# KyleHuang9/YOLO-LP

Measured on AMD Instinct MI355X. Metric: images/sec (640×640) end-to-end detect+NMS, yololps, 1/2/4/8 MI355X, higher is better.
Workload: dtype f16; 1 GPU; yololps 640x640 bs=32/GPU f16, synthetic frames resident in HBM, seeded random-init weights (sigma 0.25), conf 0.40 iou 0.45 max_det 1000; global_batch=32, parallelism=dp1: images sharded, all-gather of detections

## Files before the change

### include/lp_hip.h

```cpp
#ifndef LP_HIP_H
#define LP_HIP_H

#include <stddef.h>
#include <stdint.h>

#ifdef __cplusplus
extern "C" {
#endif

typedef enum { LP_OK = 0, LP_ERR_ARG = -1, LP_ERR_STATE = -2, LP_ERR_HIP = -3, LP_ERR_UNSUPPORTED = -4 } lp_status;
typedef enum { LP_F16 = 0, LP_BF16 = 1, LP_F32 = 2 } lp_dtype;
typedef enum { LP_ACT_NONE = 0, LP_ACT_RELU = 1, LP_ACT_SILU = 2 } lp_act;

#define LP_PRED_COLS 290
#define LP_DET_COLS 28
#define LP_MAX_SRC 4

typedef struct lp_engine lp_engine;

const char* lp_version(void);
const char* lp_last_error(void);

int lp_engine_create(lp_engine** out, int act_dtype );
void lp_engine_destroy(lp_engine* e);

int lp_engine_tensor(lp_engine* e, int channels, int stride_log2);

int lp_engine_set_lane(lp_engine* e, int lane);

int lp_engine_add_input(lp_engine* e, int dst);

typedef struct lp_conv_desc {
    int n_src;
    int src[LP_MAX_SRC];
    int dst;
    int ksize;
    int stride;
    int act;
    int res;
    float res_alpha;
    const float* weight;
    const float* bias;
    int dst2;
} lp_conv_desc;

int lp_engine_add_conv(lp_engine* e, const lp_conv_desc* d);

int lp_engine_add_deconv2x2(lp_engine* e, int src, int dst, const float* weight, const float* bias);

int lp_engine_add_pool5_chain(lp_engine* e, int src, int dst1, int dst2, int dst3);

int lp_engine_add_head_cls(lp_engine* e, int src, int level, int n_cls, const float* weight, const float* bias);

int lp_engine_add_head_box(lp_engine* e, int src, int level, int reg_bins, const float* weight, const float* bias,
                           const float* proj);

int lp_engine_finalize(lp_engine* e, int n_levels);
size_t lp_engine_weight_bytes(const lp_engine* e);
int lp_engine_upload(lp_engine* e, void* dev_weights, void* stream);

size_t lp_engine_arena_bytes(const lp_engine* e, int B, int H, int W);
int lp_engine_bind(lp_engine* e, void* dev_arena, size_t bytes, int B, int H, int W);
int lp_engine_tensor_info(const lp_engine* e, int id, size_t* offset, int* c, int* c_stored, int* h, int* w);
int lp_engine_num_anchors(const lp_engine* e);

int lp_engine_forward(lp_engine* e, const void* x, int x_dtype, float* pred, void* stream);

int lp_engine_forward_det(lp_engine* e, const void* x, int x_dtype, double conf_thres, void* workspace, size_t workspace_bytes,
                          void* stream);

int lp_engine_set_graph(lp_engine* e, int enable);

int lp_engine_set_single_lane(lp_engine* e, int enable);

int lp_engine_set_mfma16(lp_engine* e, int enable);

int lp_engine_num_ops(const lp_engine* e);
int lp_engine_op_info(const lp_engine* e, int op, int* kind, int* ksize, int* cin, int* cout, double* flops,
                      double* bytes);
int lp_engine_profile(lp_engine* e, const void* x, int x_dtype, float* pred, void* stream, float* op_ms, int reps);
int lp_engine_profile_ops(lp_engine* e, const void* x, int x_dtype, float* pred, void* stream, float* op_ms, int reps, int inner);

enum { LP_VARIANT_STREAM64 = 16, LP_VARIANT_STREAM128 = 17, LP_VARIANT_ROWS = 18,
       LP_VARIANT_PIPE_D = 32, LP_VARIANT_PIPE_B = 33, LP_VARIANT_PIPE_F = 34, LP_VARIANT_PIPE_C = 35,
       LP_VARIANT_PIPE_P = 36 ,
       LP_VARIANT_PIPE16_D = 39, LP_VARIANT_PIPE16_F = 41 ,
       LP_VARIANT_PIPE16_V0 = 42, LP_VARIANT_PIPE16_V1 = 43 ,
       LP_VARIANT_FUSED_STEM2 = 37 ,
       LP_VARIANT_FUSED_PW_S2 = 38  };
enum { LP_VARIANT_FUSED_BIFUSION = 45 };
enum { LP_VARIANT_BOX_SPARSE = 46, LP_VARIANT_BOX_DENSE = 47 };
enum { LP_VARIANT_PIPE16_S2A = 48, LP_VARIANT_PIPE16_S2B = 49 };
int lp_engine_op_carrier(const lp_engine* e, int op, int frame_direct);
int lp_engine_autotune(lp_engine* e, const void* x, int x_dtype, float* pred, void* stream, int reps);
int lp_engine_op_variant(const lp_engine* e, int op, int* cfg, int* nbuf);
int lp_engine_set_op_variant(lp_engine* e, int op, int cfg, int nbuf);
int lp_engine_set_op_tile(lp_engine* e, int op, int choice);
int lp_engine_op_tile(const lp_engine* e, int op, int* choice, int* TH, int* TW);
int lp_engine_copy_tuning(lp_engine* dst, const lp_engine* src);

size_t lp_nms_workspace_bytes(int B, int N);
int lp_nms(float* pred, int B, int N, double conf_thres, double iou_thres, int max_det, float* det, int32_t* count,
           int32_t* keep, void* workspace, size_t workspace_bytes, void* stream);

int lp_nms_candidates(int B, int N, double iou_thres, int max_det, float* det, int32_t* count, int32_t* keep, void* workspace,
                      size_t workspace_bytes, void* stream);

const int32_t* lp_nms_candidate_counts(const void* workspace, int B, int N);

int lp_preprocess_letterbox(const unsigned char* img, int h0, int w0, void* out, int out_dtype, int H, int W, int rh, int rw,
                            int top, int left, void* stream);
int lp_rescale_round(float* det, int n, double ratio, double padx, double pady, int img_w, int img_h, void* stream);

#define LP_FRAMES_PER_LAUNCH 64
typedef struct lp_frame_desc {
    const unsigned char* img;
    int h0, w0, rh, rw, top, left;
} lp_frame_desc;
typedef struct lp_rescale_desc { double ratio, padx, pady; int img_w, img_h; } lp_rescale_desc;
int lp_preprocess_letterbox_batch(const lp_frame_desc* desc, int n_frames, int B, void* out, int out_dtype, int H, int W,
                                  void* stream);
int lp_rescale_round_batch(float* det, const int32_t* count, int B, int max_det, const lp_rescale_desc* desc, void* stream);

typedef struct lp_tile_desc {
    const unsigned char* img;
    int h0, w0;
    int y0, x0, th, tw;
    int rh, rw, top, left;
} lp_tile_desc;
int lp_preprocess_tiles_batch(const lp_tile_desc* desc, int n_tiles, int B, void* out, int out_dtype, int H, int W, void* stream);

#define LP_NV12_PER_LAUNCH 32
typedef struct lp_nv12_desc {
    const unsigned char* y;
    const unsigned char* uv;
    int pitch_y, pitch_uv;
    int h0, w0;
    int y0, x0, th, tw;
    int rh, rw, top, left;
    int matrix;
} lp_nv12_desc;
typedef struct lp_nv12_bgr_desc {
    const unsigned char* y;
    const unsigned char* uv;
    int pitch_y, pitch_uv;
    int h0, w0;
    int matrix;
    unsigned char* out;
} lp_nv12_bgr_desc;
int lp_preprocess_nv12_batch(const lp_nv12_desc* desc, int n, int B, void* out, int out_dtype, int H, int W, void* stream);
int lp_nv12_to_bgr_batch(const lp_nv12_bgr_desc* desc, int n, void* stream);

typedef struct lp_tile_ref { int frame, y0, x0, th, tw; } lp_tile_ref;
size_t lp_merge_tiles_workspace_bytes(int n_frames, int max_det);
int lp_merge_tiles(const float* det_t, const int32_t* count_t, const lp_tile_ref* tiles, int n_tiles, int max_det_t,
                   const int* frame_hw, int n_frames, double thres, int metric , int border, int max_det,
                   float* det, int32_t* count, int32_t* src, void* workspace, size_t workspace_bytes, void* stream);

#define LP_TRACK_MAX_TRACKS 128
#define LP_TRACK_MAX_DETS 128
#define LP_TRACK_MAX_CLS 64
typedef struct lp_track_params { double match_thres, new_thres, expand; int max_age; int ncls[8]; } lp_track_params;
size_t lp_track_state_bytes(int n_streams, int max_tracks);
size_t lp_track_dropped_offset(int max_tracks, int stream_index);
int lp_track_update(void* state, int n_streams, int max_tracks, const lp_track_params* p,
                    const float* det, const int32_t* count, int B, int max_det,
                    const int* stream_of , const unsigned char* flush ,
                    float* det_out, int32_t* tid, int32_t* ended_i, float* ended_f, int32_t* ended_count,
                    int max_ended, void* stream);
int lp_track_update_slots(void* state, int n_streams, int max_tracks, const lp_track_params* p,
                          const float* det, const int32_t* count, int B, int max_det,
                          const int* stream_of , const unsigned char* flush ,
                          float* det_out, int32_t* tid, int32_t* slot, int32_t* ended_i, float* ended_f, int32_t* ended_count,
                          int max_ended, void* stream);
typedef struct lp_track_hold_params { int min_hits, max_misses; } lp_track_hold_params;
int lp_track_update_hold(void* state, int n_streams, int max_tracks, const lp_track_params* p,
                         const float* det, const int32_t* count, int B, int max_det,
                         const int* stream_of , const unsigned char* flush ,
                         float* det_out, int32_t* tid, int32_t* slot, int32_t* ended_i, float* ended_f, int32_t* ended_count,
                         int max_ended, const lp_track_hold_params* hp, float* det_hold, int32_t* count_hold, int32_t* tid_hold,
                         void* stream);

typedef struct lp_crop_desc {
    const unsigned char* img;
    int h0, w0;
    int max_crops;
    int out_slot;
} lp_crop_desc;
int lp_plate_crops_batch(const lp_crop_desc* desc, int n_frames, const float* det, const int32_t* count, int max_det,
                         unsigned char* out, int32_t* status, int n_slots, int crop_h, int crop_w, void* stream);

int lp_crop_sharpness(const unsigned char* crops, const int32_t* status, int n_slots, int crop_h, int crop_w,
                      unsigned long long* sharp, void* stream);

size_t lp_best_shot_state_bytes(int n_streams, int max_tracks, int crop_h, int crop_w);
int lp_best_shot_update(void* state, int n_streams, int max_tracks, int crop_h, int crop_w,
                        const float* det, const int32_t* count, int B, int max_det, const int32_t* tid, const int32_t* slot,
                        const unsigned char* crops, const int32_t* status, const unsigned long long* sharp, int max_crops,
                        const int* stream_of , const int32_t* ended_i, const int32_t* ended_count, int max_ended,
                        double min_score, unsigned char* shot_crops, int32_t* shot_i, unsigned long long* shot_q, float* shot_det,
                        void* stream);

#define LP_REDACT_MAX_CELL 64
typedef struct lp_redact_desc {
    unsigned char* p0;
    unsigned char* p1;
    int pitch0, pitch1;
    int h0, w0;
    int format;
} lp_redact_desc;
typedef struct lp_redact_params {
    int mode;
    int cell;
    double margin;
    unsigned char fill[3];
} lp_redact_params;
size_t lp_redact_workspace_bytes(const lp_redact_desc* desc, int n_frames, const lp_redact_params* p);
int lp_redact_plates_batch(const lp_redact_desc* desc, int n_frames, const float* det, const int32_t* count, int max_det,
                           const lp_redact_params* p, int32_t* status ,
                           void* workspace, size_t workspace_bytes, void* stream);

#define LP_REDACT_MAX_RADIUS 48
typedef struct lp_redact_gauss_params {
    double margin;
    int radius, radius_c;
    uint16_t taps[LP_REDACT_MAX_RADIUS + 1];
    uint16_t taps_c[LP_REDACT_MAX_RADIUS + 1];
} lp_redact_gauss_params;
size_t lp_redact_gauss_workspace_bytes(const lp_redact_desc* desc, int n_frames, const lp_redact_gauss_params* p);
int lp_redact_gauss_batch(const lp_redact_desc* desc, int n_frames, const float* det, const int32_t* count, int max_det,
                          const lp_redact_gauss_params* p, int32_t* status ,
                          void* workspace, size_t workspace_bytes, void* stream);

#define LP_LOOKBACK_MAX_DEPTH 32
size_t lp_lookback_state_bytes(int n_streams, int max_tracks, int depth, int rows);
int lp_lookback_update(void* state, int n_streams, int max_tracks, int depth, int max_back, int back_cap,
                       const float* det_hold, const int32_t* count_hold, const int32_t* tid, const int32_t* slot,
                       int B, int max_det, int hold_rows,
                       const int* stream_of , const unsigned char* flush ,
                       float* rel_det, int32_t* rel_count, int32_t* rel_frame,
                       float* tail_det, int32_t* tail_count, int32_t* tail_frame, void* stream);

#define LP_WATCH_MAX_ENTRIES (1 << 24)
#define LP_WATCH_MAX_COST 32768
#define LP_WATCH_BLOCK_ENTRIES 2048
// ... 40 lines not shown
```

### yolo-lp_amd/csrc/lp_conv.hip

```cpp
#include "lp_internal.h"

#include <cstdlib>

namespace lp {

int conv_launch_f16(int cfg, int mode, int ksize, int stride, int nbuf, const ConvArgs& a, hipStream_t st);
int conv_launch_bf16(int cfg, int mode, int ksize, int stride, int nbuf, const ConvArgs& a, hipStream_t st);
int conv_launch_f32(int cfg, int mode, int ksize, int stride, int nbuf, const ConvArgs& a, hipStream_t st);

int conv_stream_launch_f16(int wc, const ConvArgs& a, int cb_pack, int lds, hipStream_t st);
int conv_stream_launch_bf16(int wc, const ConvArgs& a, int cb_pack, int lds, hipStream_t st);
int conv_stream_launch_f32(int wc, const ConvArgs& a, int cb_pack, int lds, hipStream_t st);

int conv_pipe_launch_f16(int pcfg, const ConvArgs& a, int ncu, hipStream_t st);
int conv_pipe_launch_bf16(int pcfg, const ConvArgs& a, int ncu, hipStream_t st);

int head_rows_launch_f16(const ConvArgs& a, int cb_pack, hipStream_t st);
int head_rows_launch_bf16(const ConvArgs& a, int cb_pack, hipStream_t st);
int head_rows_launch_f32(const ConvArgs& a, int cb_pack, hipStream_t st);
int head_box_det_launch_f16(const ConvArgs& a, int cb_pack, hipStream_t st);
int head_box_det_launch_bf16(const ConvArgs& a, int cb_pack, hipStream_t st);
int head_box_det_launch_f32(const ConvArgs& a, int cb_pack, hipStream_t st);

ConvShape conv_shape(int dtype, int cfg, int ksize, int stride) {
    const int sz = (int)dtype_size(dtype);
    ConvShape s;
    int wc = 2, wp = 2, wgc = 1, wgp = 4;
    switch (cfg) {
        case CFG_A: wgc = 2; wgp = 2; break;
        case CFG_B: break;
        case CFG_C: wc = 1; break;
        case CFG_D: wgc = 2; wgp = 4; break;
        case CFG_E: wc = 1; wgc = 2; wgp = 2; break;
        case CFG_F: wc = 1; wgc = 4; wgp = 2; break;
    }
    s.WP = wp;
    s.WGC = wgc;
    s.WGP = wgp;
    s.CB = 32 * wc * wgc;
    s.PB = 32 * wp * wgp;
    s.NT = 64 * wgc * wgp;
    s.KC = ksize == 1 ? 128 / sz : 32 / sz;
    s.HPMAX = ksize == 1 ? s.PB : (stride == 1 ? 2 * s.PB + 128 : 5 * s.PB + 128);
    return s;
}

static inline int swz_host(int row, int g, int gpr) { return gpr == 2 ? (g ^ ((row >> 3) & 1)) : (g ^ ((row >> 1) & 7)); }

int conv_pick_pitch(const ConvShape& s, int dtype, int ksize, int stride, int TH, int TW) {
    const int hw = (TW - 1) * stride + ksize, hh = (TH - 1) * stride + ksize;
    if (ksize == 1) return hw;
    (void)dtype;
    const int rowb = 32, gpr = 2, npix = TH * TW;
    static const int G0[16] = {0, 1, 2, 3, 12, 13, 14, 15, 20, 21, 22, 23, 24, 25, 26, 27};
    static const int G1[16] = {4, 5, 6, 7, 8, 9, 10, 11, 16, 17, 18, 19, 28, 29, 30, 31};
    long best_cost = -1;
    int best = hw;
    for (int pitch = hw; pitch < hw + 16; ++pitch) {
        if (hh * pitch > s.HPMAX) break;
        long cost = 0;
        for (int blk = 0; blk * 32 < s.PB; ++blk)
            for (int t = 0; t < ksize * ksize; ++t)
                for (int half = 0; half < 2; ++half)
                    for (int g = 0; g < 2; ++g) {
                        const int* lanes = g ? G1 : G0;
                        int addr[16], n = 0, slot_cnt[16] = {0};
                        for (int k = 0; k < 16; ++k) {
                            int pl = blk * 32 + lanes[k];
                            if (pl >= npix) pl = 0;
                            const int ty = pl / TW, tx = pl - ty * TW;
                            const int kx = t % ksize, hwe = (hw + 1) >> 1;
                            const int col = stride == 2 ? (kx & 1) * hwe + tx + (kx >> 1) : tx * stride + kx;
                            const int hp = (ty * stride + t / ksize) * pitch + col;
                            const int a = hp * rowb + swz_host(hp, half, gpr) * 16;
                            bool dup = false;
                            for (int m = 0; m < n; ++m) dup |= addr[m] == a;
                            if (!dup) { addr[n++] = a; ++slot_cnt[(a >> 4) & 15]; }
                        }
                        int mx = 1;
                        for (int k = 0; k < 16; ++k) mx = slot_cnt[k] > mx ? slot_cnt[k] : mx;
                        cost += mx;
                    }
        cost = cost * 64 + (pitch - hw);
        if (best_cost < 0 || cost < best_cost) { best_cost = cost; best = pitch; }
    }
    return best;
}

int conv_pick_pitch16(const ConvShape& s, int TH, int TW) {
    const int hw = TW + 2, hh = TH + 2, rowb = 32, npix = TH * TW;
    static const int GRP[4][16] = {{0, 1, 2, 3, 12, 13, 14, 15, 20, 21, 22, 23, 24, 25, 26, 27}, {4, 5, 6, 7, 8, 9, 10, 11, 16, 17, 18, 19, 28, 29, 30, 31},
                                   {32, 33, 34, 35, 44, 45, 46, 47, 52, 53, 54, 55, 56, 57, 58, 59}, {36, 37, 38, 39, 40, 41, 42, 43, 48, 49, 50, 51, 60, 61, 62, 63}};
    auto qo = [](int i) { return ((i >> 2) == 2 ? 12 : (i >> 2) == 3 ? 8 : (i & 12)) + (i & 3); };
    long best_cost = -1;
    int best = hw;
    for (int pitch = hw; pitch < hw + 16; ++pitch) {
        if (hh * pitch > s.HPMAX) break;
        long cost = 0;
        for (int blk = 0; blk * 16 < s.PB; ++blk)
            for (int st = 0; st < 9; ++st) {
                const int ta = st < 4 ? 2 * st : (st == 4 ? 8 : 2 * st - 9), tb = st == 4 ? 0 : ta + 1;
                for (int gq = 0; gq < 4; ++gq) {
                    int addr[16], n = 0, slot_cnt[16] = {0};
                    for (int k = 0; k < 16; ++k) {
                        const int l = GRP[gq][k], i = l & 15, g = l >> 4;
                        int pl = blk * 16 + qo(i);
                        if (pl >= npix) pl = 0;
                        const int ty = pl / TW, tx = pl - ty * TW, t = g < 2 ? ta : tb;
                        const int hp = (ty + t / 3) * pitch + tx + t % 3;
                        const int a = hp * rowb + swz_host(hp, g & 1, 2) * 16 + (g >> 1) * (1 << 20);
                        bool dup = false;
                        for (int m = 0; m < n; ++m) dup |= addr[m] == a;
                        if (!dup) { addr[n++] = a; ++slot_cnt[(a >> 4) & 15]; }
                    }
                    int mx = 1;
                    for (int k = 0; k < 16; ++k) mx = slot_cnt[k] > mx ? slot_cnt[k] : mx;
                    cost += mx;
                }
            }
        cost = cost * 64 + (pitch - hw);
        if (best_cost < 0 || cost < best_cost) { best_cost = cost; best = pitch; }
    }
    return best;
}

void conv_pick_tile16v(const ConvShape& s, int Ho, int Wo, int B, int nct, int choice, int* TH, int* TW, int stride) {
    struct Cand { double cost; int th, tw; };
    Cand best[4];
    int n = 0;
    const int ncu = device_cus();
    for (int th = 1; th <= Ho; ++th)
        for (int tw = 1; tw <= Wo; ++tw) {
            const int hh = (th - 1) * stride + 3, hw = (tw - 1) * stride + 3;
            if (th * tw > s.PB || hh * hw > s.HPMAX) continue;
            const long tiles = (long)B * ceil_div(Ho, th) * ceil_div(Wo, tw) * nct;
            const int nb = ceil_div(th * tw, 16), per_wave = ceil_div(nb, s.WGP);
            const double cost = (double)ceil_div((int)tiles, ncu) * (per_wave + 0.75) + 1e-4 * hh * hw + 1e-7 * tiles;
            int pos = n < 4 ? n : 4;
            for (int k = 0; k < (n < 4 ? n : 4); ++k)
                if (cost < best[k].cost) { pos = k; break; }
            if (pos >= 4) continue;
            for (int k = (n < 4 ? n : 3); k > pos; --k) best[k] = best[k - 1];
            best[pos] = {cost, th, tw};
            if (n < 4) ++n;
        }
    if (n == 0) { *TH = 1; *TW = 1; return; }
    if (choice < 0) choice = 0;
    if (choice >= n) choice = n - 1;
    *TH = best[choice].th;
    *TW = best[choice].tw;
}

void conv_pick_tile(const ConvShape& s, int ksize, int stride, int Ho, int Wo, int choice, int* TH, int* TW) {
    struct Cand { long cost; int th, tw; };
    Cand best[4];
    int n = 0;
    for (int th = 1; th <= s.PB && th <= Ho; ++th) {
        int tw = s.PB / th;
        if (tw > Wo) tw = Wo;
        if (tw < 1) continue;
        const int hh = (th - 1) * stride + ksize, hw = (tw - 1) * stride + ksize;
        if (hh * hw > s.HPMAX) continue;
        const long tiles = (long)ceil_div(Ho, th) * ceil_div(Wo, tw);
        Cand c = {tiles * 100000 + (long)hh * hw, th, tw};
        int pos = n < 4 ? n : 4;
        for (int k = 0; k < (n < 4 ? n : 4); ++k)
            if (c.cost < best[k].cost) { pos = k; break; }
        if (pos >= 4) continue;
        for (int k = (n < 4 ? n : 3); k > pos; --k) best[k] = best[k - 1];
        best[pos] = c;
        if (n < 4) ++n;
    }
// ... 35 lines not shown
    if (a0.nsrc < 1 || a0.nsrc > LP_MAX_SRC || a0.nphase != 1 || a0.out_scale != 1 || a0.Ho != a0.H || a0.Wo != a0.W ||
        a0.out_img_stride != (long long)a0.Ho * a0.Wo * a0.out_pix_stride)
        return fail(LP_ERR_ARG, "conv1x1 stream: not a dense 1x1 stride-1 layer");
    if (a0.out2 && (a0.out_split % (32 * wc) != 0 || a0.res || a0.out2_img_stride != (long long)a0.Ho * a0.Wo * a0.out2_pix_stride))
        return fail(LP_ERR_ARG, "conv1x1 stream: the second destination must start at a cout tile of the wave");
    const int kc = 128 / (int)dtype_size(dtype);
    for (int i = 0; i < a0.nsrc; ++i)
        if (a0.src[i].cs % (kc / 4) != 0) return fail(LP_ERR_ARG, "conv1x1 stream: source channels are not whole 32-byte K-steps");
    ConvArgs a = a0;
    a.nct = ceil_div(a.out_c, 32 * wc);
    switch (dtype) {
        case LP_F16: return conv_stream_launch_f16(wc, a, cb_pack, lds, st);
        case LP_BF16: return conv_stream_launch_bf16(wc, a, cb_pack, lds, st);
        case LP_F32: return conv_stream_launch_f32(wc, a, cb_pack, lds, st);
    }
    return fail(LP_ERR_ARG, "conv1x1 stream: dtype");
}

ConvShape conv_pipe_shape(int pcfg) {
    ConvShape s;
    s.KC = 16;
    s.NT = 512;
    s.WP = 2;
    switch (pcfg) {
        case PIPE_B: s.CB = 64; s.WGC = 1; s.WGP = 8; s.HPMAX = 704; break;
        case PIPE_F: case PIPE16_F: s.CB = 128; s.WGC = 4; s.WGP = 2; s.HPMAX = 384; break;
        case PIPE_C: s.CB = 32; s.WGC = 1; s.WGP = 8; s.HPMAX = 736; break;
        case PIPE16_V0: s.CB = 128; s.WGC = 2; s.WGP = 4; s.HPMAX = 512; s.PB = 4 * 7 * 16; return s;
        case PIPE16_V1: s.CB = 128; s.WGC = 4; s.WGP = 2; s.HPMAX = 512; s.PB = 2 * 7 * 16; return s;
        case PIPE16_S2A: s.CB = 128; s.WGC = 2; s.WGP = 4; s.HPMAX = 864; s.PB = 4 * 4 * 16; return s;
        case PIPE16_S2B: s.CB = 128; s.WGC = 4; s.WGP = 2; s.HPMAX = 864; s.PB = 2 * 7 * 16; return s;
        default: s.CB = 128; s.WGC = 2; s.WGP = 4; s.HPMAX = 384; break;
    }
    s.PB = 32 * s.WP * s.WGP;
    return s;
}

bool conv_pipe_fits(int dtype, int pcfg, int cb_pack, int ksize, int stride, int mode, int nct, int nphase, int nchunks) {
    if (pcfg == PIPE_P) return false;
    if (pipe_is_16s2(pcfg))
        return dtype != LP_F32 && ksize == 3 && stride == 2 && mode == MODE_ACT && nphase == 1 && cb_pack == 128 && nct * 128 <= 512 && nchunks >= 1 && nchunks <= 64;
    if (pipe_is_16(pcfg) && (nchunks < 4 || nchunks % 4 != 0)) return false;
    if (dtype == LP_F32 || pcfg < 0 || (pcfg >= PIPE_COUNT && !pipe_is_16(pcfg)) || ksize != 3 || stride != 1 || mode != MODE_ACT || nphase != 1) return false;
    const ConvShape s = conv_pipe_shape(pcfg);
    if (pipe_is_16v(pcfg) && (nct * s.CB > 512 || nchunks > 32)) return false;
    return s.CB == cb_pack && nct * s.CB <= 1024 && nchunks <= 64;
}

static int g_ncu[16] = {0};
int device_cus() {
    int dev = 0;
    if (hipGetDevice(&dev) != hipSuccess || dev < 0 || dev >= 16) return 256;
    if (!g_ncu[dev]) {
        int n = 0;
        if (hipDeviceGetAttribute(&n, hipDeviceAttributeMultiprocessorCount, dev) != hipSuccess || n < 8) n = 256;
        g_ncu[dev] = n / 8 * 8;
        if (const char* cap = getenv("LP_PIPE_MAXWG")) { const int c = atoi(cap) / 8 * 8; if (c >= 8 && c < g_ncu[dev]) g_ncu[dev] = c; }
    }
    return g_ncu[dev];
}

bool stem_planar_tile(int Ho, int Wo, int choice, int* TH, int* TW) {
    struct Cand { long long tiles; int th, tw; };
    std::vector<Cand> cands;
    for (int tw = 4; tw <= 512 && tw < Wo + 4; tw += 4) {
        int th = 512 / tw;
        if (th > Ho) th = Ho;
        while (th >= 1 && ((th + 2) * 6 + 2) * (tw / 4 + 2) * 16 > 20 * 1024) --th;
        if (th < 1) continue;
        cands.push_back({(long long)ceil_div(Ho, th) * ceil_div(Wo, tw), th, tw});
    }
    std::sort(cands.begin(), cands.end(), [](const Cand& x, const Cand& y) { return x.tiles != y.tiles ? x.tiles < y.tiles : x.tw > y.tw; });
    if (choice < 0 || choice >= (int)cands.size()) return false;
    *TH = cands[choice].th;
    *TW = cands[choice].tw;
    return true;
}

bool stem2_fused_tile(int Ho, int Wo, int choice, int* TH, int* TW, int* hpitch) {
    struct Cand { long long cost; int th, tw; };
    std::vector<Cand> cands;
    for (int tw = 2; tw <= 128 && tw < Wo + 2; tw += 2)
        for (int th = 1; th <= 128 / tw && th <= Ho; ++th) {
            const int hp4 = tw / 2 + 2, rin = 2 * th + 3, hps = 2 * tw + 1;
            const int ntb = (th * tw + 31) / 32;
            if ((rin * 6 + 2) * hp4 * 16 > 21 * 1024 || (rin * 6 * hp4 + 63) / 64 > 24 || (2 * th + 1) * hps > 640 || ntb * 2 > 16) continue;
            cands.push_back({(long long)ceil_div(Ho, th) * ceil_div(Wo, tw) * (2 * th + 1) * hps, th, tw});
        }
    std::sort(cands.begin(), cands.end(), [](const Cand& x, const Cand& y) { return x.cost != y.cost ? x.cost < y.cost : x.tw > y.tw; });
    if (choice < 0 || choice >= (int)cands.size()) return false;
    *TH = cands[choice].th;
    *TW = cands[choice].tw;
    *hpitch = 2 * cands[choice].tw + 1;
    return true;
}

int conv_pipe_launch(int dtype, int pcfg, const ConvArgs& a, hipStream_t st) {
    if (pcfg == PIPE_P || pcfg == PIPE_FUSED2 || pcfg == PIPE_FUSED_PW || pcfg == PIPE_FUSED_BF) {
        switch (dtype) {
            case LP_F16: return conv_pipe_launch_f16(pcfg, a, device_cus(), st);
            case LP_BF16: return conv_pipe_launch_bf16(pcfg, a, device_cus(), st);
        }
        return fail(LP_ERR_UNSUPPORTED, "planar stem: 16-bit frames only");
    }
    const ConvShape s = conv_pipe_shape(pcfg);
    if (pipe_is_16s2(pcfg)) {
        const int hh2 = 2 * a.TH + 1, hw2 = 2 * a.TW + 1, nchunks = a.chunk_begin[a.nsrc];
        if (a.TH < 1 || a.TW < 1 || a.TH * a.TW > s.PB || a.hpitch != hw2 || hh2 * a.hpitch > s.HPMAX)
            return fail(LP_ERR_ARG, "conv3x3 s2p16: tile does not fit the kernel configuration");
        if (a.tiles_x * a.TW < a.Wo || a.tiles_y * a.TH < a.Ho) return fail(LP_ERR_ARG, "conv3x3 s2p16: tiles do not cover the output");
        if (a.nsrc < 1 || a.nsrc > LP_MAX_SRC || a.nct < 1 || a.nct * s.CB > 512 || nchunks < 1 || nchunks > 64 || a.nphase != 1 || a.out_scale != 1 ||
            a.H != 2 * a.Ho || a.W != 2 * a.Wo || a.out2)
            return fail(LP_ERR_ARG, "conv3x3 s2p16: not a 3x3 stride-2 layer this kernel runs");
        const int stride = a.out_pix_stride > a.res_cs ? a.out_pix_stride : a.res_cs;
        if (((long long)a.TH * a.Wo + a.TW) * stride + 2048 >= (1ll << 31)) return fail(LP_ERR_ARG, "conv3x3 s2p16: a tile's rows span more than 2^31 elements");
        switch (dtype) {
            case LP_F16: return conv_pipe_launch_f16(pcfg, a, device_cus(), st);
            case LP_BF16: return conv_pipe_launch_bf16(pcfg, a, device_cus(), st);
        }
        return fail(LP_ERR_UNSUPPORTED, "conv3x3 s2p16: 16-bit activations only");
    }
    const int hh = a.TH + 2, hw = a.TW + 2;
    if (pcfg < 0 || (pcfg >= PIPE_COUNT && !pipe_is_16(pcfg))) return fail(LP_ERR_ARG, "conv3x3 pipe: configuration");
    if (pipe_is_16(pcfg) && (a.chunk_begin[a.nsrc] < 4 || a.chunk_begin[a.nsrc] % 4 != 0)) return fail(LP_ERR_ARG, "conv3x3 pipe16: K-chunks not a multiple of four");
    if (a.TH < 1 || a.TW < 1 || a.TH * a.TW > s.PB || a.hpitch < hw || hh * a.hpitch > s.HPMAX)
        return fail(LP_ERR_ARG, "conv3x3 pipe: tile does not fit the kernel configuration");
    if (a.tiles_x * a.TW < a.Wo || a.tiles_y * a.TH < a.Ho) return fail(LP_ERR_ARG, "conv3x3 pipe: tiles do not cover the output");
    if (pipe_is_16v(pcfg) && (a.nct * s.CB > 512 || a.chunk_begin[a.nsrc] > 32)) return fail(LP_ERR_ARG, "conv3x3 pipe16v: layer exceeds the kernel's LDS tables");
    if (pipe_is_16v(pcfg)) {
        int stride = a.out_pix_stride > a.res_cs ? a.out_pix_stride : a.res_cs;
        if (a.out2 && a.out2_pix_stride > stride) stride = a.out2_pix_stride;
        if (((long long)a.TH * a.Wo + a.TW) * stride + 2048 >= (1ll << 31)) return fail(LP_ERR_ARG, "conv3x3 pipe16v: a tile's rows span more than 2^31 elements");
    }
    if (a.chunk_begin[a.nsrc] > 64) return fail(LP_ERR_ARG, "conv3x3 pipe: more K-chunks than the kernel's LDS chunk table holds");
    if (a.nsrc < 1 || a.nsrc > LP_MAX_SRC || a.nct < 1 || a.nct * s.CB > 1024 || a.nphase != 1 || a.out_scale != 1 || a.Ho != a.H || a.Wo != a.W)
        return fail(LP_ERR_ARG, "conv3x3 pipe: not a 3x3 stride-1 layer this kernel runs");
    switch (dtype) {
        case LP_F16: return conv_pipe_launch_f16(pcfg, a, device_cus(), st);
        case LP_BF16: return conv_pipe_launch_bf16(pcfg, a, device_cus(), st);
    }
    return fail(LP_ERR_UNSUPPORTED, "conv3x3 pipe: 16-bit activations only");
}

bool head_rows_fits(int dtype, int nchunks, int cb_pack, int out_c) {
    const long lds = (long)nchunks * 9 * 32 * 128 + 9 * 32 * 4 + 32 * 8 + 32 * 1168;
    return nchunks >= 1 && nchunks <= 3 && lds <= 160 * 1024 && (cb_pack == 32 || cb_pack == 64 || cb_pack == 128) && out_c == LP_PRED_COLS - 13;
}
bool head_det_fits(int dtype, int nchunks, int cb_pack, int out_c) {
    const long lds = (long)nchunks * 9 * 32 * 128 + 9 * 32 * 4 + 32 * 8 * 4 + 16 + 6 * 32 * 8 * 4 + 6 * 1168;
    return nchunks >= 1 && nchunks <= (dtype == LP_F32 ? 3 : 4) && lds <= 160 * 1024 && (cb_pack == 32 || cb_pack == 64 || cb_pack == 128) &&
           out_c == LP_PRED_COLS - 13;
}

bool head_box_det_fits(const ConvArgs& a, int cb_pack, int ksize, int stride) {
    const int nchunks = a.chunk_begin[a.nsrc];
    return ksize == 1 && stride == 1 && a.nsrc == 1 && nchunks >= 1 && nchunks <= 4 && a.reg_bins == 1 && a.out_c == 12 && a.nct == 1 &&
           cb_pack >= 32 && a.nphase == 1 && a.out_scale == 1 && a.Ho == a.H && a.Wo == a.W && a.src[0].cs % 8 == 0;
}
int head_box_det_launch(int dtype, const ConvArgs& a, int cb_pack, hipStream_t st) {
    if (!a.det_mode || !a.out || !a.zero || !head_box_det_fits(a, cb_pack, 1, 1)) return fail(LP_ERR_ARG, "head box: op does not fit");
    if (a.out_pix_stride % 4 != 0 || a.out_img_stride % 4 != 0 || ((uintptr_t)a.out & 15)) return fail(LP_ERR_ARG, "head box: candidate rows are not 16-byte aligned");
    switch (dtype) {
        case LP_F16: return head_box_det_launch_f16(a, cb_pack, st);
        case LP_BF16: return head_box_det_launch_bf16(a, cb_pack, st);
        case LP_F32: return head_box_det_launch_f32(a, cb_pack, st);
    }
    return fail(LP_ERR_ARG, "head box: dtype");
}

int head_rows_launch(int dtype, const ConvArgs& a, int cb_pack, hipStream_t st) {
    const int nchunks = a.chunk_begin[a.nsrc];
    if (!(a.det_mode ? head_det_fits(dtype, nchunks, cb_pack, a.out_c) : head_rows_fits(dtype, nchunks, cb_pack, a.out_c)))
        return fail(LP_ERR_ARG, "head rows: op does not fit");
    const int kc = 128 / (int)dtype_size(dtype);
    for (int i = 0; i < a.nsrc; ++i)
        if (a.src[i].cs % (kc / 4) != 0)
            return fail(LP_ERR_ARG, "head rows: source channels are not whole 32-byte K-steps");
    if (a.nphase != 1 || a.out_scale != 1 || a.Ho != a.H || a.Wo != a.W || !a.out) return fail(LP_ERR_ARG, "head rows: bad geometry");
    switch (dtype) {
        case LP_F16: return head_rows_launch_f16(a, cb_pack, st);
        case LP_BF16: return head_rows_launch_bf16(a, cb_pack, st);
        case LP_F32: return head_rows_launch_f32(a, cb_pack, st);
    }
    return fail(LP_ERR_ARG, "head rows: dtype");
}

}

extern "C" int lp_plan_block_tile(int variant, int Ho, int Wo, int B, int nct, int choice, int* TH, int* TW, int* hpitch) {
    const int pcfg = variant - LP_VARIANT_PIPE_D;
    if (!TH || !TW || Ho < 1 || Wo < 1 || B < 1 || nct < 1) return lp::fail(LP_ERR_ARG, "lp_plan_block_tile: bad arguments");
    if (!lp::pipe_is_16v(pcfg) && !lp::pipe_is_16s2(pcfg)) return lp::fail(LP_ERR_UNSUPPORTED, "lp_plan_block_tile: not a block-tiled variant");
    const lp::ConvShape s = lp::conv_pipe_shape(pcfg);
    const int stride = lp::pipe_is_16s2(pcfg) ? 2 : 1;
    lp::conv_pick_tile16v(s, Ho, Wo, B, nct, choice, TH, TW, stride);
    if (hpitch) *hpitch = (*TW - 1) * stride + 3;
    return LP_OK;
}

extern "C" int lp_plan_stem_tile(int fused, int Ho, int Wo, int choice, int* TH, int* TW, int* hpitch) {
    if (!TH || !TW || Ho < 1 || Wo < 1) return lp::fail(LP_ERR_ARG, "lp_plan_stem_tile: bad arguments");
    int hp = 0;
    const bool ok = fused ? lp::stem2_fused_tile(Ho, Wo, choice, TH, TW, &hp) : lp::stem_planar_tile(Ho, Wo, choice, TH, TW);
    if (hpitch) *hpitch = hp;
    return ok ? LP_OK : LP_ERR_UNSUPPORTED;
}
```

### yolo-lp_amd/csrc/lp_conv_bf16.hip

```cpp
#include "lp_conv_kernel.inc"
#include "lp_conv1x1_stream.inc"
#include "lp_head_rows.inc"
#include "lp_head_box.inc"
#include "lp_conv3x3_pipe.inc"
#include "lp_conv3x3_pipe16.inc"
#include "lp_conv3x3_pipe16v.inc"
#include "lp_conv3x3_s2p16.inc"
#include "lp_stem_planar.inc"
#include "lp_stem2_fused.inc"
#include "lp_pw_s2_fused.inc"
#include "lp_bifusion_fused.inc"

namespace lp {
int conv_launch_bf16(int cfg, int mode, int ksize, int stride, int nbuf, const ConvArgs& a, hipStream_t st) {
    return launch_dtype<bf16>(cfg, mode, ksize, stride, nbuf, a, st);
}
int conv_stream_launch_bf16(int wc, const ConvArgs& a, int cb_pack, int lds, hipStream_t st) {
    return stream_launch_dtype<bf16>(wc, a, cb_pack, lds, st);
}
int head_rows_launch_bf16(const ConvArgs& a, int cb_pack, hipStream_t st) { return head_rows_launch_dtype<bf16>(a, cb_pack, st); }
int head_box_det_launch_bf16(const ConvArgs& a, int cb_pack, hipStream_t st) { return head_box_det_launch_dtype<bf16>(a, cb_pack, st); }
int conv_pipe_launch_bf16(int pcfg, const ConvArgs& a, int ncu, hipStream_t st) {
    if (pcfg == PIPE_FUSED2) return stem2_fused_launch<bf16>(a, ncu, st);
    if (pcfg == PIPE_FUSED_PW) return pw_s2_fused_launch<bf16>(a, ncu, st);
    if (pcfg == PIPE_FUSED_BF) return bifusion_launch_dtype<bf16>(a, ncu, st);
    if (pipe_is_16s2(pcfg)) return s2p16_launch_dtype<bf16>(pcfg, a, ncu, st);
    if (pipe_is_16v(pcfg)) return pipe16v_launch_dtype<bf16>(pcfg, a, ncu, st);
    if (pipe_is_16(pcfg)) return pipe16_launch_dtype<bf16>(pcfg, a, ncu, st);
    return pcfg == PIPE_P ? stem_planar_launch<bf16>(a, ncu, st) : pipe_launch_dtype<bf16>(pcfg, a, ncu, st);
}
}
```

### yolo-lp_amd/csrc/lp_conv_f16.hip

```cpp
#include "lp_conv_kernel.inc"
#include "lp_conv1x1_stream.inc"
#include "lp_head_rows.inc"
#include "lp_head_box.inc"
#include "lp_conv3x3_pipe.inc"
#include "lp_conv3x3_pipe16.inc"
#include "lp_conv3x3_pipe16v.inc"
#include "lp_conv3x3_s2p16.inc"
#include "lp_stem_planar.inc"
#include "lp_stem2_fused.inc"
#include "lp_pw_s2_fused.inc"
#include "lp_bifusion_fused.inc"

namespace lp {
int conv_launch_f16(int cfg, int mode, int ksize, int stride, int nbuf, const ConvArgs& a, hipStream_t st) {
    return launch_dtype<f16>(cfg, mode, ksize, stride, nbuf, a, st);
}
int conv_stream_launch_f16(int wc, const ConvArgs& a, int cb_pack, int lds, hipStream_t st) {
    return stream_launch_dtype<f16>(wc, a, cb_pack, lds, st);
}
int head_rows_launch_f16(const ConvArgs& a, int cb_pack, hipStream_t st) { return head_rows_launch_dtype<f16>(a, cb_pack, st); }
int head_box_det_launch_f16(const ConvArgs& a, int cb_pack, hipStream_t st) { return head_box_det_launch_dtype<f16>(a, cb_pack, st); }
int conv_pipe_launch_f16(int pcfg, const ConvArgs& a, int ncu, hipStream_t st) {
    if (pcfg == PIPE_FUSED2) return stem2_fused_launch<f16>(a, ncu, st);
    if (pcfg == PIPE_FUSED_PW) return pw_s2_fused_launch<f16>(a, ncu, st);
    if (pcfg == PIPE_FUSED_BF) return bifusion_launch_dtype<f16>(a, ncu, st);
    if (pipe_is_16s2(pcfg)) return s2p16_launch_dtype<f16>(pcfg, a, ncu, st);
    if (pipe_is_16v(pcfg)) return pipe16v_launch_dtype<f16>(pcfg, a, ncu, st);
    if (pipe_is_16(pcfg)) return pipe16_launch_dtype<f16>(pcfg, a, ncu, st);
    return pcfg == PIPE_P ? stem_planar_launch<f16>(a, ncu, st) : pipe_launch_dtype<f16>(pcfg, a, ncu, st);
}
}
```

### yolo-lp_amd/csrc/lp_engine.hip

```cpp
#include "lp_internal.h"

#include <cmath>
#include <cstdlib>
#include <cstring>
#include <map>
#include <utility>
#include <vector>

namespace lp {

static thread_local std::string g_err;
void set_error(const std::string& msg) { g_err = msg; }
int fail(int code, const std::string& msg) {
    g_err = msg;
    return code;
}

enum OpKind { OP_INPUT = 0, OP_CONV = 1, OP_DECONV = 2, OP_POOL = 3, OP_HEAD_CLS = 4, OP_HEAD_BOX = 5 };

struct Tensor {
    int c, cs, sl;
    bool unused = false;
    size_t offset;
    int h, w;
};

struct Op {
    int kind = OP_CONV;
    int nsrc = 0;
    int src[LP_MAX_SRC] = {-1, -1, -1, -1};
    int dst = -1, dst2 = -1, dst3 = -1;
    int ksize = 1, stride = 1, act = 0;
    int res = -1;
    float alpha = 0.f;
    int cout = 0;
    int cin = 0;
    int level = 0, reg_bins = 1;
    bool s2d = false;
    int alg_kk = 0;
    int lane = 0;
    std::vector<int> deps;
    bool signal = false;
    std::vector<float> weight, bias, proj;
    int cfg = CFG_A, mode = MODE_ACT, nct = 1, nchunks = 0, nphase = 1, nbuf = 1, tile = 0;
    int stream_wc = 0, stream_rd = 2;
    int rows = 0;
    size_t det_scratch = (size_t)-1;
    int box_sparse = 1;
    int pipe = 0;
    int fused_pw = 0;
    int fused_bf = 0;
    int bf_up = -1, bf_cv1 = -1;
    int bf_carrier = -1;
    int fused = 0;
    int planar = 0;
    int chunk_begin[LP_MAX_SRC + 1] = {0, 0, 0, 0, 0};
    size_t w_off = 0, b_off = 0, proj_off = 0;
    long long w_phase_stride = 0;
};

struct Launch {
    ConvArgs a;
    long long pred_off = 0;
    int cfg = 0, mode = 0, ks = 1, st = 1, nbuf = 1;
    int stream_wc = 0, stream_rd = 2, cb_pack = 0, rows = 0, pipe = 0;
    bool is_conv = false;
};

}

using namespace lp;
struct lp_engine;
static bool bifusion_fused_possible(const lp_engine* e, size_t i, int* up, int* cv1);
static bool op_fam16(const lp_engine* e, const lp::Op& op);
static int fam16_default_pipe(const lp_engine* e, const lp::Op& op);

#ifndef LP_MAX_LANES
#define LP_MAX_LANES 5
#endif
struct lp_engine {
    int dtype = LP_F16;
    bool finalized = false;
    int n_levels = 3;
    std::vector<Tensor> tensors;
    std::vector<Op> ops;
    std::vector<unsigned char> blob;
    char* dev_w = nullptr;
    char* arena = nullptr;
    size_t arena_bytes = 0;
    int B = 0, H = 0, W = 0, n_anchors = 0;
    std::vector<int> level_off;
    std::vector<hipEvent_t> events;
    int cur_lane = 0;
    int n_lanes = 1;
    hipStream_t lane_stream[LP_MAX_LANES] = {};
    std::vector<hipEvent_t> op_event;
    hipEvent_t fork_ev = nullptr, join_ev[LP_MAX_LANES] = {};
    bool single_lane = true;
    bool use_graph = false;
    bool s2p16 = getenv("LP_S2P16") != nullptr;
    bool mfma16 = getenv("LP_NO_MFMA16") == nullptr;
    bool box_sparse_ok = false;
    std::vector<int> box_ord;
    struct CachedGraph {
        hipGraphExec_t exec = nullptr;
        const void* x = nullptr;
        float* pred = nullptr;
        void* ws = nullptr;
        float conf = 0.f;
        int x_dtype = -1;
        unsigned long long epoch = 0, last_use = 0;
        hipStream_t stream = nullptr;
    };
    std::vector<CachedGraph> graphs;
    unsigned long long graph_clock = 0;
    hipEvent_t done_ev = nullptr;
    bool done_valid = false;
    hipStream_t cap_stream = nullptr;
    unsigned long long epoch = 1;
    std::vector<Launch> launches;
    Launch stem_planar;
    Launch stem2_fused;
    std::map<int, Launch> pw_fused;
    std::map<int, Launch> bf_fused;
    std::map<std::vector<int>, std::vector<std::vector<int>>> tuned;
};

struct lp_engine;
static int prepare_op(lp_engine* e, size_t idx);
static unsigned long long* g_stamps = nullptr;
extern "C" void lpdbg_set_stamps(void* p) { g_stamps = (unsigned long long*)p; }
static bool valid_tensor(const lp_engine* e, int id) { return id >= 0 && id < (int)e->tensors.size(); }

extern "C" const char* lp_version(void) { return "yololp-hip 0.1 (gfx950)"; }
extern "C" const char* lp_last_error(void) { return g_err.c_str(); }

extern "C" int lp_engine_create(lp_engine** out, int act_dtype) {
    if (!out) return fail(LP_ERR_ARG, "lp_engine_create: null out");
    if (act_dtype != LP_F16 && act_dtype != LP_BF16 && act_dtype != LP_F32) return fail(LP_ERR_ARG, "lp_engine_create: dtype");
    lp_engine* e = new lp_engine();
    e->dtype = act_dtype;
    *out = e;
    return LP_OK;
}

extern "C" void lp_engine_destroy(lp_engine* e) {
    if (!e) return;
    for (int l = 1; l < LP_MAX_LANES; ++l)
        if (e->lane_stream[l]) (void)hipStreamSynchronize(e->lane_stream[l]);
    if (e->done_valid) (void)hipEventSynchronize(e->done_ev);
    if (e->done_ev) (void)hipEventDestroy(e->done_ev);
    for (hipEvent_t ev : e->events) (void)hipEventDestroy(ev);
    for (auto& g : e->graphs) {
        if (g.stream) (void)hipStreamSynchronize(g.stream);
        if (g.exec) (void)hipGraphExecDestroy(g.exec);
    }
    if (e->cap_stream) (void)hipStreamDestroy(e->cap_stream);
    for (hipEvent_t ev : e->op_event) if (ev) (void)hipEventDestroy(ev);
    if (e->fork_ev) (void)hipEventDestroy(e->fork_ev);
    for (int l = 1; l < LP_MAX_LANES; ++l) { if (e->join_ev[l]) (void)hipEventDestroy(e->join_ev[l]); if (e->lane_stream[l]) (void)hipStreamDestroy(e->lane_stream[l]); }
    delete e;
}

extern "C" int lp_engine_tensor(lp_engine* e, int channels, int stride_log2) {
    if (!e || e->finalized) return fail(LP_ERR_STATE, "lp_engine_tensor: engine is null or frozen");
    if (channels < 1 || stride_log2 < 0 || stride_log2 > 6) return fail(LP_ERR_ARG, "lp_engine_tensor: bad shape");
    Tensor t;
    t.c = channels;
    t.cs = round_up(channels, 8);
    t.sl = stride_log2;
    t.offset = 0;
    t.h = t.w = 0;
    e->tensors.push_back(t);
    return (int)e->tensors.size() - 1;
}

extern "C" int lp_engine_set_lane(lp_engine* e, int lane) {
    if (!e || e->finalized) return fail(LP_ERR_STATE, "lp_engine_set_lane: engine is null or frozen");
    if (lane < 0 || lane >= LP_MAX_LANES) return fail(LP_ERR_ARG, "lp_engine_set_lane: lane must be 0..4");
    e->cur_lane = lane;
    return LP_OK;
}

extern "C" int lp_engine_add_input(lp_engine* e, int dst) {
    if (!e || e->finalized) return fail(LP_ERR_STATE, "lp_engine_add_input: engine is null or frozen");
    if (!e->ops.empty()) return fail(LP_ERR_STATE, "lp_engine_add_input: must be the first op");
    if (!valid_tensor(e, dst) || e->tensors[dst].c != 3 || e->tensors[dst].sl != 0)
        return fail(LP_ERR_ARG, "lp_engine_add_input: dst must be a 3-channel full-resolution tensor");
    Op op;
    op.kind = OP_INPUT;
    op.dst = dst;
    op.cout = 3;
    op.cin = 3;
    op.lane = e->cur_lane;
    e->ops.push_back(op);
    return LP_OK;
}

extern "C" int lp_engine_add_conv(lp_engine* e, const lp_conv_desc* d) {
    if (!e || e->finalized) return fail(LP_ERR_STATE, "lp_engine_add_conv: engine is null or frozen");
// ... 253 lines not shown
        blob.resize(blob.size() + per_phase * op.nphase * esz, 0);
        unsigned char* wp = blob.data() + op.w_off;
        for (int ph = 0; ph < op.nphase; ++ph)
            for (int ct = 0; ct < op.nct; ++ct)
                for (int i = 0; i < op.nsrc; ++i) {
                    const Tensor& t = e->tensors[op.src[i]];
                    for (int q = op.chunk_begin[i]; q < op.chunk_begin[i + 1]; ++q) {
                        const int c0 = (q - op.chunk_begin[i]) * s.KC;
                        for (int tp = 0; tp < taps; ++tp)
                            for (int cl = 0; cl < s.CB; ++cl) {
                                const int co = ct * s.CB + cl;
                                if (co >= op.cout) continue;
                                const size_t row = ((((size_t)ph * op.nct + ct) * op.nchunks + q) * taps + tp) * s.CB + cl;
                                const int srow = tp * s.CB + cl;
                                for (int kc = 0; kc < s.KC; ++kc) {
                                    const int c = c0 + kc;
                                    if (c >= t.c) break;
                                    const int ci = cin_off[i] + c;
                                    float v;
                                    if (op.kind == OP_DECONV)
                                        v = op.weight[((size_t)ci * op.cout + co) * 4 + ph];
                                    else
                                        v = op.weight[((size_t)co * op.cin + ci) * taps + tp];
                                    const int epg = 16 / (int)esz, gpr = s.KC / epg;
                                    const int pos = gpr == 2 ? ((kc / epg) ^ ((srow >> 3) & 1)) : ((kc / epg) ^ ((srow >> 1) & 7));
                                    put_elem(wp, row * s.KC + (size_t)pos * epg + kc % epg, v, dt);
                                }
                            }
                    }
                }
        align();
        op.b_off = blob.size();
        blob.resize(blob.size() + (size_t)op.nct * s.CB * 4, 0);
        memcpy(blob.data() + op.b_off, op.bias.data(), (size_t)op.cout * 4);
        if (!op.proj.empty()) {
            align();
            op.proj_off = blob.size();
            blob.resize(blob.size() + op.proj.size() * 4, 0);
            memcpy(blob.data() + op.proj_off, op.proj.data(), op.proj.size() * 4);
        }
        std::vector<float>().swap(op.weight);
    }
    align();
    for (size_t i = 0; i < e->ops.size(); ++i) {
        int up = -1, c1 = -1;
        if (!bifusion_fused_possible(e, i, &up, &c1)) continue;
        e->ops[i].bf_up = up;
        e->ops[i].bf_cv1 = c1;
        e->ops[(size_t)up].bf_carrier = e->ops[(size_t)c1].bf_carrier = (int)i;
    }
    {
        e->box_ord.assign(e->ops.size(), -1);
        bool ok = true;
        int nbox = 0, cls_seen = 0, cls_level = -1;
        for (size_t i = 0; i < e->ops.size(); ++i) {
            const Op& o = e->ops[i];
            if (o.kind == OP_HEAD_CLS) { ++cls_seen; cls_level = o.level; }
            if (o.kind == OP_HEAD_BOX) {
                ok = ok && cls_seen == 1 && cls_level == o.level;
                e->box_ord[i] = nbox++;
                cls_seen = 0;
            }
        }
        e->box_sparse_ok = ok && nbox >= 1 && nbox <= 4 && cls_seen == 0;
    }
    e->finalized = true;
    return LP_OK;
}

extern "C" size_t lp_engine_weight_bytes(const lp_engine* e) { return e && e->finalized ? e->blob.size() : 0; }

extern "C" int lp_engine_upload(lp_engine* e, void* dev_weights, void* stream) {
    if (!e || !e->finalized) return fail(LP_ERR_STATE, "lp_engine_upload: finalize first");
    if (!dev_weights || ((uintptr_t)dev_weights & 255)) return fail(LP_ERR_ARG, "lp_engine_upload: need a 256-byte aligned device pointer");
    LP_HIP_CHECK(hipMemcpyAsync(dev_weights, e->blob.data(), e->blob.size(), hipMemcpyHostToDevice, (hipStream_t)stream));
    LP_HIP_CHECK(hipStreamSynchronize((hipStream_t)stream));
    e->dev_w = (char*)dev_weights;
    return LP_OK;
}

static bool rows_fits(const lp_engine* e, const Op& op);
static bool det_fits(const lp_engine* e, const Op& op);

static size_t place(const lp_engine* e, int B, int H, int W, std::vector<Tensor>* out, std::vector<size_t>* scratch = nullptr) {
    size_t off = 0;
    const size_t esz = dtype_size(e->dtype);
    for (size_t i = 0; i < e->tensors.size(); ++i) {
        Tensor t = e->tensors[i];
        t.h = H >> t.sl;
        t.w = W >> t.sl;
        t.offset = off;
        if (!t.unused) off += ((size_t)B * t.h * t.w * t.cs * esz + 255) / 256 * 256;
        if (out) (*out)[i] = t;
    }
    if (scratch) scratch->assign(e->ops.size(), (size_t)-1);
    for (size_t i = 0; i < e->ops.size(); ++i) {
        const Op& op = e->ops[i];
        if (op.kind != OP_HEAD_CLS || det_fits(e, op)) continue;
        if (scratch) (*scratch)[i] = off;
        off += ((size_t)B * (H >> (3 + op.level)) * (W >> (3 + op.level)) * LP_PRED_COLS * 4 + 255) / 256 * 256;
    }
    return off + 256;
}

static bool pool_fits(const lp_engine* e, int H, int W) {
    for (const Op& op : e->ops) {
        if (op.kind != OP_POOL) continue;
        const Tensor& t = e->tensors[op.src[0]];
        const int h = H >> t.sl, w = W >> t.sl;
        if (pool_min_lds_bytes(e->dtype, h, w) > POOL_MAX_LDS || h * w >= 65536) return false;
    }
    return true;
}

static int size_granule(const lp_engine* e) {
    int sl = 5;
    for (const Tensor& t : e->tensors) sl = t.sl > sl ? t.sl : sl;
    return 1 << sl;
}

extern "C" size_t lp_engine_arena_bytes(const lp_engine* e, int B, int H, int W) {
    if (!e || B < 1) return 0;
    const int g = size_granule(e);
    if (H < g || W < g || H % g || W % g || !pool_fits(e, H, W)) return 0;
    return place(e, B, H, W, nullptr);
}

extern "C" int lp_engine_bind(lp_engine* e, void* dev_arena, size_t bytes, int B, int H, int W) {
    if (!e || !e->finalized) return fail(LP_ERR_STATE, "lp_engine_bind: finalize first");
    const int gran = size_granule(e);
    if (B < 1 || H < gran || W < gran || H % gran || W % gran)
        return fail(LP_ERR_ARG, "lp_engine_bind: H and W must be positive multiples of " + std::to_string(gran) + " (the coarsest stride of the graph)");
    if (!dev_arena || ((uintptr_t)dev_arena & 255)) return fail(LP_ERR_ARG, "lp_engine_bind: need a 256-byte aligned device pointer");
    if (!pool_fits(e, H, W))
        return fail(LP_ERR_UNSUPPORTED, "lp_engine_bind: the SPPF pool chain keeps a whole stride-32 map in LDS: input too large (limit ~2048x2048 px in "
                                        "f16 / bf16, ~1440x1440 in f32)");
    const size_t need = place(e, B, H, W, nullptr);
    if (bytes < need) return fail(LP_ERR_ARG, "lp_engine_bind: arena too small");
    if ((long long)B * H * W >= (1LL << 31)) return fail(LP_ERR_UNSUPPORTED, "lp_engine_bind: batch too large for 32-bit pixel indices");
    std::vector<size_t> scratch;
    place(e, B, H, W, &e->tensors, &scratch);
    for (size_t i = 0; i < e->ops.size(); ++i) e->ops[i].det_scratch = scratch[i];
    e->arena = (char*)dev_arena;
    e->arena_bytes = bytes;
    e->B = B;
    e->H = H;
    e->W = W;
    e->level_off.assign(e->n_levels + 1, 0);
    for (int l = 0; l < e->n_levels; ++l) e->level_off[l + 1] = e->level_off[l] + (H >> (3 + l)) * (W >> (3 + l));
    e->n_anchors = e->level_off[e->n_levels];
    if (!e->dev_w) return fail(LP_ERR_STATE, "lp_engine_bind: upload the weights first");
    auto it = e->tuned.find({B, H, W});
    if (it != e->tuned.end())
        for (size_t i = 0; i < e->ops.size(); ++i) { e->ops[i].cfg = it->second[i][0]; e->ops[i].nbuf = it->second[i][1]; e->ops[i].tile = it->second[i][2]; e->ops[i].stream_wc = it->second[i][3]; e->ops[i].stream_rd = it->second[i][4]; e->ops[i].rows = it->second[i][5]; e->ops[i].pipe = it->second[i][6]; e->ops[i].planar = it->second[i][7]; e->ops[i].fused = it->second[i][8]; e->ops[i].fused_pw = it->second[i][9]; e->ops[i].fused_bf = it->second[i].size() > 10 ? it->second[i][10] : 0; }
    e->launches.assign(e->ops.size(), Launch());
    for (size_t i = 0; i < e->ops.size(); ++i) {
        int rc = prepare_op(e, i);
        if (rc) return rc;
    }
    return LP_OK;
}

extern "C" int lp_engine_tensor_info(const lp_engine* e, int id, size_t* offset, int* c, int* c_stored, int* h, int* w) {
    if (!e || !valid_tensor(e, id)) return fail(LP_ERR_ARG, "lp_engine_tensor_info: tensor id");
    const Tensor& t = e->tensors[id];
    if (offset) *offset = t.offset;
    if (c) *c = t.c;
    if (c_stored) *c_stored = t.cs;
    if (h) *h = t.h;
    if (w) *w = t.w;
    return LP_OK;
}

extern "C" int lp_engine_num_anchors(const lp_engine* e) { return e ? e->n_anchors : 0; }
extern "C" int lp_engine_num_ops(const lp_engine* e) { return e ? (int)e->ops.size() : 0; }

extern "C" int lp_engine_op_info(const lp_engine* e, int i, int* kind, int* ksize, int* cin, int* cout, double* flops, double* bytes) {
    if (!e || i < 0 || i >= (int)e->ops.size()) return fail(LP_ERR_ARG, "lp_engine_op_info: op index");
    if (!e->arena) return fail(LP_ERR_STATE, "lp_engine_op_info: bind first");
    const Op& op = e->ops[i];
    const double esz = (double)dtype_size(e->dtype);
    double fl = 0, by = 0;
    auto tbytes = [&](int id) { const Tensor& t = e->tensors[id]; return (double)e->B * t.h * t.w * t.c * esz; };
    const Tensor& s0 = e->tensors[op.kind == OP_INPUT ? op.dst : op.src[0]];
    const double in_px = (double)e->B * s0.h * s0.w;
    switch (op.kind) {
        case OP_INPUT: by = (double)e->B * e->H * e->W * 3 * esz + tbytes(op.dst); break;
        case OP_CONV: {
            const Tensor& d = e->tensors[op.dst];
            fl = 2.0 * e->B * d.h * d.w * op.cout * (op.alg_kk ? op.alg_kk : op.cin * op.ksize * op.ksize);
            for (int k = 0; k < op.nsrc; ++k) by += tbytes(op.src[k]);
            by += tbytes(op.dst) + (op.dst2 >= 0 ? tbytes(op.dst2) : 0) + (op.res >= 0 ? tbytes(op.res) : 0) + (double)op.cout * op.cin * op.ksize * op.ksize * esz;
            break;
        }
        case OP_DECONV: fl = 2.0 * in_px * op.cin * op.cout * 4; by = tbytes(op.src[0]) + tbytes(op.dst) + 4.0 * op.cin * op.cout * esz; break;
        case OP_POOL: by = 4 * tbytes(op.src[0]); break;
        case OP_HEAD_CLS:
        case OP_HEAD_BOX:
            fl = 2.0 * in_px * op.cin * op.cout;
            by = tbytes(op.src[0]) + in_px * (op.kind == OP_HEAD_CLS ? op.cout : 13) * 4 + (double)op.cin * op.cout * esz;
            break;
    }
    if (kind) *kind = op.kind;
    if (ksize) *ksize = op.ksize;
    if (cin) *cin = op.cin;
    if (cout) *cout = op.cout;
    if (flops) *flops = fl;
    if (bytes) *bytes = by;
    return LP_OK;
}

static bool stream_fits(const lp_engine* e, const Op& op, int wc) {
    if (op.kind != OP_CONV || op.ksize != 1 || op.stride != 1 || op.mode != MODE_ACT) return false;
    if (op.dst2 >= 0 && e->tensors[op.dst].cs % (32 * wc) != 0) return false;
    const int kc = 128 / (int)dtype_size(e->dtype);
    for (int i = 0; i < op.nsrc; ++i)
        if (e->tensors[op.src[i]].cs % (kc / 4) != 0) return false;
    return conv_stream_lds(e->dtype, wc, op.nchunks, conv_shape(e->dtype, op.cfg, 1, 1).CB) >= 0;
}

static bool rows_fits(const lp_engine* e, const Op& op) {
    if (op.kind != OP_HEAD_CLS) return false;
    const int kc = 128 / (int)dtype_size(e->dtype);
    for (int i = 0; i < op.nsrc; ++i) {
        const int cs = e->tensors[op.src[i]].cs;
        if (cs % (kc / 4) != 0) return false;
    }
    return head_rows_fits(e->dtype, op.nchunks, conv_shape(e->dtype, op.cfg, 1, 1).CB, op.cout);
}

static bool det_fits(const lp_engine* e, const Op& op) {
    if (op.kind != OP_HEAD_CLS || getenv("LP_NO_HEAD_DET")) return false;
    const int kc = 128 / (int)dtype_size(e->dtype);
    for (int i = 0; i < op.nsrc; ++i) {
        const int cs = e->tensors[op.src[i]].cs;
        if (cs % (kc / 4) != 0) return false;
    }
    return head_det_fits(e->dtype, op.nchunks, conv_shape(e->dtype, op.cfg, 1, 1).CB, op.cout);
}

static bool op_fam16(const lp_engine* e, const Op& op) {
    if (!e->mfma16 || e->dtype == LP_F32 || op.kind != OP_CONV || op.ksize != 3 || op.mode != MODE_ACT) return false;
    if (op.stride == 2)
        return e->s2p16 && op.dst2 < 0 && conv_pipe_fits(e->dtype, PIPE16_S2A, conv_shape(e->dtype, op.cfg, 3, 2).CB, 3, 2, op.mode, op.nct, op.nphase, op.nchunks);
    if (op.stride != 1) return false;
    return conv_pipe_fits(e->dtype, PIPE16_D, conv_shape(e->dtype, op.cfg, 1, 1).CB, 3, 1, op.mode, op.nct, op.nphase, op.nchunks);
}
static int fam16_default_pipe(const lp_engine*, const Op& op) { return (op.stride == 2 ? PIPE16_S2A : PIPE16_D) + 1; }

static int prepare_op(lp_engine* e, size_t idx) {
    ++e->epoch;
    const Op& op = e->ops[idx];
    Launch& L = e->launches[idx];
    L.is_conv = !(op.kind == OP_INPUT || op.kind == OP_POOL);
    if (!L.is_conv) return LP_OK;
    const int dt = e->dtype;
    auto tptr = [&](int id) { return (void*)(e->arena + e->tensors[id].offset); };
    const int ks = op.kind == OP_CONV ? op.ksize : 1, stv = op.kind == OP_CONV ? op.stride : 1;
    const int cb_pack = conv_shape(dt, op.cfg, ks, stv).CB;
    const ConvShape s = op.pipe ? conv_pipe_shape(op.pipe - 1) : conv_shape(dt, op.cfg, ks, stv);
    ConvArgs& a = L.a;
    memset(&a, 0, sizeof(a));
    a.nsrc = op.nsrc;
    for (int i = 0; i < op.nsrc; ++i) { a.src[i].ptr = tptr(op.src[i]); a.src[i].cs = e->tensors[op.src[i]].cs; }
    for (int i = 0; i <= LP_MAX_SRC; ++i) a.chunk_begin[i] = op.chunk_begin[i];
    a.zero = e->dev_w;
    a.trash = e->dev_w + 128;
    a.w = e->dev_w + op.w_off;
    a.bias = (const float*)(e->dev_w + op.b_off);
    const Tensor& s0 = e->tensors[op.src[0]];
    a.B = e->B;
    a.H = s0.h;
    a.W = s0.w;
    a.Ho = stv == 2 ? s0.h / 2 : s0.h;
    a.Wo = stv == 2 ? s0.w / 2 : s0.w;
    if (op.pipe && pipe_is_16s2(op.pipe - 1)) {
        conv_pick_tile16v(s, a.Ho, a.Wo, e->B, op.nct, op.tile, &a.TH, &a.TW, 2);
        a.hpitch = 2 * a.TW + 1;
    } else if (op.pipe && pipe_is_16v(op.pipe - 1)) {
        conv_pick_tile16v(s, a.Ho, a.Wo, e->B, op.nct, op.tile, &a.TH, &a.TW);
        a.hpitch = a.TW + 2;
    } else {
        conv_pick_tile(s, ks, stv, a.Ho, a.Wo, op.tile, &a.TH, &a.TW);
        a.hpitch = (op.pipe && pipe_is_16(op.pipe - 1)) ? conv_pick_pitch16(s, a.TH, a.TW) : conv_pick_pitch(s, dt, ks, stv, a.TH, a.TW);
    }
    a.tw_magic = (unsigned)(((1u << 22) + a.TW - 1) / a.TW);
    a.hp_magic = (unsigned)(((1u << 22) + a.hpitch - 1) / a.hpitch);
    a.tiles_x = ceil_div(a.Wo, a.TW);
    a.tiles_y = ceil_div(a.Ho, a.TH);
    a.nct = op.nct;
    a.nphase = op.nphase;
    a.w_phase_stride = op.w_phase_stride;
    a.out_scale = op.kind == OP_DECONV ? 2 : 1;
    a.act = op.act;
    a.alpha = op.alpha;
    if (op.mode == MODE_ACT) {
        const Tensor& d = e->tensors[op.dst];
        a.out = tptr(op.dst);
        a.out_c = d.cs;
        a.out_pix_stride = d.cs;
        a.out_img_stride = (long long)d.h * d.w * d.cs;
        if (op.kind == OP_CONV && op.dst2 >= 0) {
            const Tensor& d2 = e->tensors[op.dst2];
            a.out2 = tptr(op.dst2);
            a.out_split = d.cs;
            a.out_c = d.cs + d2.cs;
            a.out2_pix_stride = d2.cs;
            a.out2_img_stride = (long long)d2.h * d2.w * d2.cs;
        }
        if (op.res >= 0) { a.res = tptr(op.res); a.res_cs = e->tensors[op.res].cs; }
    } else {
        a.out = nullptr;
        L.pred_off = (long long)e->level_off[op.level] * LP_PRED_COLS + (op.mode == MODE_PRED ? 13 : 0);
        a.out_pix_stride = LP_PRED_COLS;
        a.out_img_stride = (long long)e->n_anchors * LP_PRED_COLS;
        a.out_c = op.cout;
        if (op.mode == MODE_DECODE) {
            a.reg_bins = op.reg_bins;
            a.proj = op.proj.empty() ? nullptr : (const float*)(e->dev_w + op.proj_off);
            a.stride_px = (float)(8 << op.level);
        }
    }
    a.stamps = g_stamps;
    L.cfg = op.cfg;
    L.mode = op.mode;
    L.ks = ks;
    L.st = stv;
    L.nbuf = op.nbuf;
    L.stream_wc = op.stream_wc;
    L.stream_rd = op.stream_rd;
    L.rows = op.rows;
    L.pipe = op.pipe;
    L.cb_pack = cb_pack;
    if (op.planar) {
        Launch& P = e->stem_planar;
        P = L;
        ConvArgs& pa = P.a;
        if (pa.W % 4 != 0 || !stem_planar_tile(pa.Ho, pa.Wo, op.planar - 1, &pa.TH, &pa.TW))
            return fail(LP_ERR_UNSUPPORTED, "planar stem: no tile for this frame size");
        pa.tw_magic = (unsigned)(((1u << 22) + pa.TW - 1) / pa.TW);
        pa.tiles_x = ceil_div(pa.Wo, pa.TW);
        pa.tiles_y = ceil_div(pa.Ho, pa.TH);
        pa.src[0].ptr = nullptr;
        P.pipe = PIPE_P + 1;
    }
    if (op.fused) {
        const Op& stem = e->ops[1];
        Launch& F = e->stem2_fused;
        F = L;
        ConvArgs& fa = F.a;
        if (!stem2_fused_tile(fa.Ho, fa.Wo, op.fused - 1, &fa.TH, &fa.TW, &fa.hpitch))
            return fail(LP_ERR_UNSUPPORTED, "fused stem: no tile for this frame size");
        fa.tw_magic = (unsigned)(((1u << 22) + fa.TW - 1) / fa.TW);
        fa.hp_magic = (unsigned)(((1u << 22) + fa.hpitch - 1) / fa.hpitch);
        fa.tiles_x = ceil_div(fa.Wo, fa.TW);
        fa.tiles_y = ceil_div(fa.Ho, fa.TH);
        fa.src[0].ptr = nullptr;
        fa.fz_w1 = e->dev_w + stem.w_off;
        fa.fz_b1 = (const float*)(e->dev_w + stem.b_off);
        fa.fz_act1 = stem.act;
        fa.fz_c1 = e->tensors[stem.dst].cs;
        F.pipe = PIPE_FUSED2 + 1;
    }
    if (op.fused_bf) {
        const Op& up = e->ops[op.bf_up];
        const Op& c1 = e->ops[op.bf_cv1];
        Launch& F = e->bf_fused[(int)idx];
        F = L;
        ConvArgs& fa = F.a;
        fa.src[0].ptr = tptr(up.src[0]); fa.src[0].cs = e->tensors[up.src[0]].cs;
        fa.src[1].ptr = tptr(c1.src[0]); fa.src[1].cs = e->tensors[c1.src[0]].cs;
        fa.fz_w1 = e->dev_w + c1.w_off;
        fa.fz_b1 = (const float*)(e->dev_w + c1.b_off);
        fa.fz_act1 = c1.act;
        fa.bf_wd = e->dev_w + up.w_off;
        fa.bf_bd = (const float*)(e->dev_w + up.b_off);
        fa.bf_wd_phase_stride = up.w_phase_stride;
        F.pipe = PIPE_FUSED_BF + 1;
    }
    if (op.fused_pw) {
        const Op& pw = e->ops[idx - 1];
        Launch& F = e->pw_fused[(int)idx];
        F = L;
        ConvArgs& fa = F.a;
        int hp = 0;
        if (!stem2_fused_tile(fa.Ho, fa.Wo, op.fused_pw - 1, &fa.TH, &fa.TW, &hp))
            return fail(LP_ERR_UNSUPPORTED, "fused 1x1 + 3x3 s2: no tile for this map size");
        fa.hpitch = hp;
        fa.tw_magic = (unsigned)(((1u << 22) + fa.TW - 1) / fa.TW);
        fa.hp_magic = (unsigned)(((1u << 22) + fa.hpitch - 1) / fa.hpitch);
        fa.tiles_x = ceil_div(fa.Wo, fa.TW);
        fa.tiles_y = ceil_div(fa.Ho, fa.TH);
        fa.src[0].ptr = tptr(pw.src[0]);
        fa.src[0].cs = e->tensors[pw.src[0]].cs;
        fa.fz_w1 = e->dev_w + pw.w_off;
        fa.fz_b1 = (const float*)(e->dev_w + pw.b_off);
        fa.fz_act1 = pw.act;
        fa.fz_c1 = e->tensors[pw.dst].cs;
        F.pipe = PIPE_FUSED_PW + 1;
    }
    return LP_OK;
}

static bool stem_planar_possible(const lp_engine* e) {
    return e->dtype != LP_F32 && e->ops.size() > 1 && e->ops[0].kind == OP_INPUT && e->ops[0].s2d && e->ops[1].kind == OP_CONV &&
           e->ops[1].ksize == 3 && e->ops[1].stride == 1 && e->ops[1].mode == MODE_ACT && e->ops[1].nct == 1 && e->ops[1].nchunks == 1 &&
           (conv_shape(e->dtype, e->ops[1].cfg, 3, 1).CB == 32 || conv_shape(e->dtype, e->ops[1].cfg, 3, 1).CB == 64) && e->ops[1].res < 0 &&
           e->ops[1].dst2 < 0;
}
static bool frame_direct(const lp_engine* e, const void* x, int x_dtype) { return x_dtype == e->dtype && ((uintptr_t)x & 15) == 0; }
static bool stem_planar_now(const lp_engine* e, const void* x, int x_dtype) { return e->ops.size() > 1 && e->ops[1].planar && frame_direct(e, x, x_dtype); }
static bool stem2_fused_possible(const lp_engine* e) {
    if (!stem_planar_possible(e) || e->ops.size() < 3) return false;
    const Op& s = e->ops[1];
    const Op& c = e->ops[2];
    if (c.kind != OP_CONV || c.ksize != 3 || c.stride != 2 || c.nsrc != 1 || c.src[0] != s.dst || c.res >= 0 || c.dst2 >= 0 || c.mode != MODE_ACT ||
        c.nct != 1 || c.nphase != 1 || c.nchunks < 1 || c.nchunks > 2 || s.act != LP_ACT_RELU || c.act != LP_ACT_RELU) return false;
    const int cb = conv_shape(e->dtype, c.cfg, 3, 2).CB, cs2 = e->tensors[c.dst].cs;
    if ((cb != 32 && cb != 64) || cb != 32 * ((cs2 + 31) / 32) || e->tensors[s.dst].cs > 16 * c.nchunks) return false;
    for (size_t i = 3; i < e->ops.size(); ++i) {
        const Op& o = e->ops[i];
        for (int k = 0; k < o.nsrc; ++k) if (o.src[k] == s.dst) return false;
        if (o.res == s.dst) return false;
    }
    return true;
}
static bool pw_fused_possible(const lp_engine* e, size_t i) {
    if (e->dtype == LP_F32 || i < 2 || i >= e->ops.size()) return false;
    const Op& p = e->ops[i - 1];
    const Op& c = e->ops[i];
    if (c.kind != OP_CONV || c.ksize != 3 || c.stride != 2 || c.nsrc != 1 || c.res >= 0 || c.dst2 >= 0 || c.mode != MODE_ACT || c.nct != 1 || c.nphase != 1) return false;
    if (p.kind != OP_CONV || p.ksize != 1 || p.stride != 1 || p.nsrc != 1 || p.res >= 0 || p.dst2 >= 0 || p.mode != MODE_ACT || p.nct != 1 || p.nphase != 1 ||
        p.nchunks != 1 || p.dst != c.src[0] || p.lane != c.lane || p.signal) return false;
    const int cs0 = e->tensors[p.src[0]].cs, cs1 = e->tensors[p.dst].cs, cs2 = e->tensors[c.dst].cs;
    if (cs0 != 64 || (cs1 != 32 && cs1 != 64) || (cs2 != 32 && cs2 != 64)) return false;
    if (conv_shape(e->dtype, p.cfg, 1, 1).CB != cs1 || conv_shape(e->dtype, c.cfg, 3, 2).CB != cs2 || c.nchunks != cs1 / 16) return false;
    for (size_t k = 0; k < e->ops.size(); ++k) {
        if (k == i) continue;
        const Op& o = e->ops[k];
        for (int q = 0; q < o.nsrc; ++q) if (o.src[q] == p.dst) return false;
        if (o.res == p.dst) return false;
    }
    return true;
}
static bool bifusion_fused_possible(const lp_engine* e, size_t i, int* up, int* cv1) {
    if (e->dtype == LP_F32 || i >= e->ops.size()) return false;
    const Op& c = e->ops[i];
    if (c.kind != OP_CONV || c.ksize != 1 || c.stride != 1 || c.nsrc != 3 || c.res >= 0 || c.dst2 >= 0 || c.mode != MODE_ACT || c.nct != 1 || c.nphase != 1 ||
        c.nchunks != 3 || c.act != LP_ACT_RELU || conv_shape(e->dtype, c.cfg, 1, 1).CB != 64 || e->tensors[c.dst].cs != 64) return false;
    int ju = -1, ja = -1;
    for (size_t k = 0; k < i; ++k) {
        if (e->ops[k].kind == OP_DECONV && e->ops[k].dst == c.src[0]) ju = (int)k;
        if (e->ops[k].kind == OP_CONV && e->ops[k].dst == c.src[1]) ja = (int)k;
    }
    if (ju < 0 || ja < 0) return false;
    const Op& u = e->ops[ju];
    const Op& p = e->ops[ja];
    if (u.nsrc != 1 || u.nct != 1 || u.nphase != 4 || u.nchunks != 1 || u.act != LP_ACT_NONE ||
        conv_shape(e->dtype, u.cfg, 1, 1).CB != 64 || e->tensors[u.src[0]].cs != 64 || e->tensors[u.dst].cs != 64) return false;
    if (p.ksize != 1 || p.stride != 1 || p.nsrc != 1 || p.res >= 0 || p.dst2 >= 0 || p.mode != MODE_ACT || p.nct != 1 || p.nphase != 1 || p.nchunks != 2 ||
        p.act != LP_ACT_RELU || conv_shape(e->dtype, p.cfg, 1, 1).CB != 64 || e->tensors[p.src[0]].cs != 128 ||
        e->tensors[p.dst].cs != 64 || e->tensors[c.src[2]].cs != 64) return false;
    const Tensor& tf = e->tensors[c.dst];
    const Tensor& tc = e->tensors[u.src[0]];
    if (tf.h != 2 * tc.h || tf.w != 2 * tc.w) return false;
    for (size_t k = 0; k < e->ops.size(); ++k) {
        if (k == i) continue;
        const Op& o = e->ops[k];
        for (int q = 0; q < o.nsrc; ++q) if (o.src[q] == u.dst || o.src[q] == p.dst) return false;
        if (o.res == u.dst || o.res == p.dst) return false;
    }
    if (up) *up = ju;
    if (cv1) *cv1 = ja;
    return true;
}
static bool stem2_fused_now(const lp_engine* e, const void* x, int x_dtype) { return e->ops.size() > 2 && e->ops[2].fused && frame_direct(e, x, x_dtype); }

struct DetCtx {
    NmsWs w;
    float conf;
};

static int run_head_det(lp_engine* e, size_t idx, const DetCtx& dc, hipStream_t st) {
    const Op& op = e->ops[idx];
    const Launch& L = e->launches[idx];
    const int dt = e->dtype;
    ConvArgs a = L.a;
    const int anchor0 = e->level_off[op.level], N = e->n_anchors;
    if (L.mode == MODE_DECODE) {
        a.det_mode = 1;
        a.out = dc.w.rows + (long long)anchor0 * LP_DET_COLS;
        a.out_pix_stride = LP_DET_COLS;
        a.out_img_stride = (long long)N * LP_DET_COLS;
        static const bool no_box_stream = getenv("LP_NO_BOX_STREAM") != nullptr;
        static const bool no_box_sparse = getenv("LP_NO_BOX_SPARSE") != nullptr;
        const bool snap_ok = !no_box_sparse && e->box_sparse_ok && (e->n_lanes <= 1 || e->single_lane) && e->box_ord[idx] >= 0 && N >= 8;
        auto streams = [&](size_t j) { const Launch& Lj = e->launches[j]; return !no_box_stream && head_box_det_fits(Lj.a, Lj.cb_pack, Lj.ks, Lj.st); };
        if (streams(idx)) {
            if (snap_ok) {
                const int k = e->box_ord[idx];
                int* const snaps = dc.w.kept;
                a.det_cnt = dc.w.cnt;
                a.det_np = dc.w.NP;
                a.det_snap = snaps + (size_t)k * e->B;
                bool prev_snap = k == 0;
                for (size_t j = 0; j < idx && !prev_snap; ++j) prev_snap = e->box_ord[j] == k - 1 && streams(j);
                if (op.box_sparse && prev_snap) {
                    a.det_keys = dc.w.keys;
                    a.det_n = N;
                    a.det_anchor0 = anchor0;
                    a.det_prev = k > 0 ? snaps + (size_t)(k - 1) * e->B : nullptr;
                }
            }
            return head_box_det_launch(dt, a, L.cb_pack, st);
        }
        return conv_launch(dt, L.cfg, L.mode, L.ks, L.st, L.nbuf, a, st);
    }
    if (op.det_scratch == (size_t)-1) {
        a.det_mode = 1;
        a.out = dc.w.rows;
        a.det_keys = dc.w.keys;
        a.det_cnt = dc.w.cnt;
        a.det_np = dc.w.NP;
        a.det_n = N;
        a.det_anchor0 = anchor0;
        a.det_conf = dc.conf;
        return head_rows_launch(dt, a, L.cb_pack, st);
    }
    float* const scratch = (float*)(e->arena + op.det_scratch);
    const int rpi = a.Ho * a.Wo;
    a.out = scratch + 13;
    a.out_img_stride = (long long)rpi * LP_PRED_COLS;
    int rc = conv_launch(dt, L.cfg, L.mode, L.ks, L.st, L.nbuf, a, st);
    if (rc) return rc;
    return nms_score_launch(scratch, e->B, rpi, anchor0, N, dc.conf, dc.w, false, st);
}

static int run_op(lp_engine* e, size_t idx, const void* x, int x_dtype, float* pred, hipStream_t st, const DetCtx* det = nullptr) {
    const Op& op = e->ops[idx];
    const int dt = e->dtype;
    auto tptr = [&](int id) { return (void*)(e->arena + e->tensors[id].offset); };
    if (op.kind == OP_INPUT) {
        if (op.s2d && (stem_planar_now(e, x, x_dtype) || stem2_fused_now(e, x, x_dtype))) return LP_OK;
        return op.s2d ? input_s2d_launch(x, x_dtype, tptr(op.dst), dt, e->B, e->H, e->W, st)
                      : input_launch(x, x_dtype, tptr(op.dst), dt, e->B, e->H, e->W, st);
    }
    if (op.kind == OP_POOL) {
        const Tensor& t = e->tensors[op.src[0]];
        return pool_launch(tptr(op.src[0]), tptr(op.dst), tptr(op.dst2), tptr(op.dst3), dt, e->B, t.h, t.w, t.cs, st);
    }
    const Launch& L = e->launches[idx];
    if (idx + 1 < e->ops.size() && e->ops[idx + 1].fused_pw) return LP_OK;
    if (op.bf_carrier >= 0 && e->ops[op.bf_carrier].fused_bf) return LP_OK;
    if (op.fused_bf) return conv_pipe_launch(dt, PIPE_FUSED_BF, e->bf_fused[(int)idx].a, st);
    if (op.fused_pw) return conv_pipe_launch(dt, PIPE_FUSED_PW, e->pw_fused[(int)idx].a, st);
    if (idx == 1 && stem2_fused_now(e, x, x_dtype)) return LP_OK;
    if (idx == 2 && stem2_fused_now(e, x, x_dtype)) {
        ConvArgs a = e->stem2_fused.a;
        a.src[0].ptr = x;
        return conv_pipe_launch(dt, PIPE_FUSED2, a, st);
    }
    if (idx == 1 && op.planar && stem_planar_now(e, x, x_dtype)) {
        ConvArgs a = e->stem_planar.a;
        a.src[0].ptr = x;
        return conv_pipe_launch(dt, PIPE_P, a, st);
    }
    if (L.mode == MODE_ACT && L.pipe) return conv_pipe_launch(dt, L.pipe - 1, L.a, st);
    if (L.mode == MODE_ACT && L.stream_wc) return conv_stream_launch(dt, L.stream_wc, L.a, L.cb_pack, st);
    if (L.mode == MODE_ACT) return conv_launch(dt, L.cfg, L.mode, L.ks, L.st, L.nbuf, L.a, st);
    if (det) return run_head_det(e, idx, *det, st);
    if (!pred) return fail(LP_ERR_ARG, "forward: pred is null");
    ConvArgs a = L.a;
    a.out = pred + L.pred_off;
    if (L.mode == MODE_PRED && L.rows) return head_rows_launch(dt, a, L.cb_pack, st);
    return conv_launch(dt, L.cfg, L.mode, L.ks, L.st, L.nbuf, a, st);
}

static int check_ready(const lp_engine* e, const void* x, int x_dtype) {
    if (!e || !e->finalized) return fail(LP_ERR_STATE, "forward: engine not finalized");
    if (!e->dev_w) return fail(LP_ERR_STATE, "forward: weights not uploaded");
    if (!e->arena) return fail(LP_ERR_STATE, "forward: arena not bound");
    if (!x) return fail(LP_ERR_ARG, "forward: x is null");
    if (x_dtype != LP_F16 && x_dtype != LP_BF16 && x_dtype != LP_F32) return fail(LP_ERR_ARG, "forward: x dtype");
    return LP_OK;
}

static int ensure_lanes(lp_engine* e) {
    for (int l = 1; l < e->n_lanes; ++l)
        if (!e->lane_stream[l]) LP_HIP_CHECK(hipStreamCreateWithFlags(&e->lane_stream[l], hipStreamNonBlocking));
    if (!e->fork_ev) LP_HIP_CHECK(hipEventCreateWithFlags(&e->fork_ev, hipEventDisableTiming));
    for (int l = 1; l < e->n_lanes; ++l)
        if (!e->join_ev[l]) LP_HIP_CHECK(hipEventCreateWithFlags(&e->join_ev[l], hipEventDisableTiming));
    if (e->op_event.size() != e->ops.size()) e->op_event.assign(e->ops.size(), nullptr);
    for (size_t i = 0; i < e->ops.size(); ++i)
        if (e->ops[i].signal && !e->op_event[i]) LP_HIP_CHECK(hipEventCreateWithFlags(&e->op_event[i], hipEventDisableTiming));
    return LP_OK;
}

static int issue_forward(lp_engine* e, const void* x, int x_dtype, float* pred, hipStream_t main_st, const DetCtx* det = nullptr) {
    int rc;
    if (e->n_lanes <= 1 || e->single_lane) {
        for (size_t i = 0; i < e->ops.size(); ++i) {
            rc = run_op(e, i, x, x_dtype, pred, main_st, det);
            if (rc) return rc;
        }
        return LP_OK;
    }
    rc = ensure_lanes(e);
    if (rc) return rc;
    e->lane_stream[0] = main_st;
    LP_HIP_CHECK(hipEventRecord(e->fork_ev, main_st));
    for (int l = 1; l < e->n_lanes; ++l) LP_HIP_CHECK(hipStreamWaitEvent(e->lane_stream[l], e->fork_ev, 0));
    for (size_t i = 0; i < e->ops.size(); ++i) {
        const Op& op = e->ops[i];
        hipStream_t st = e->lane_stream[op.lane];
        for (int d : op.deps) LP_HIP_CHECK(hipStreamWaitEvent(st, e->op_event[d], 0));
        rc = run_op(e, i, x, x_dtype, pred, st, det);
        if (rc) return rc;
        if (op.signal) LP_HIP_CHECK(hipEventRecord(e->op_event[i], st));
    }
    for (int l = 1; l < e->n_lanes; ++l) {
        LP_HIP_CHECK(hipEventRecord(e->join_ev[l], e->lane_stream[l]));
        LP_HIP_CHECK(hipStreamWaitEvent(main_st, e->join_ev[l], 0));
    }
    return LP_OK;
}

extern "C" int lp_engine_set_single_lane(lp_engine* e, int enable) {
    if (!e) return fail(LP_ERR_ARG, "lp_engine_set_single_lane: null engine");
    if (e->single_lane != (enable != 0)) ++e->epoch;
    e->single_lane = enable != 0;
    return LP_OK;
}

extern "C" int lp_engine_set_mfma16(lp_engine* e, int enable) {
    if (!e) return fail(LP_ERR_ARG, "lp_engine_set_mfma16: null engine");
    if (e->finalized) return fail(LP_ERR_STATE, "lp_engine_set_mfma16: the families are fixed by lp_engine_finalize");
    e->mfma16 = enable != 0;
    return LP_OK;
}

extern "C" int lp_engine_set_graph(lp_engine* e, int enable) {
    if (!e) return fail(LP_ERR_ARG, "lp_engine_set_graph: null engine");
    e->use_graph = enable != 0;
    return LP_OK;
}

static int mark_done(lp_engine* e, hipStream_t st) {
    if (!e->done_ev) LP_HIP_CHECK(hipEventCreateWithFlags(&e->done_ev, hipEventDisableTiming | hipEventDisableSystemFence));
    LP_HIP_CHECK(hipEventRecord(e->done_ev, st));
    e->done_valid = true;
    return LP_OK;
}

static int run_forward(lp_engine* e, const void* x, int x_dtype, float* pred, const DetCtx* det, void* ws, hipStream_t main_st) {
    int rc;
    auto issue = [&](hipStream_t st) -> int {
        if (det) { if (int zr = zero_counts_launch(det->w.cnt, e->B, st)) return zr; }
        return issue_forward(e, x, x_dtype, pred, st, det);
    };
    if (!e->use_graph) {
        rc = issue(main_st);
        return rc ? rc : mark_done(e, main_st);
    }
    constexpr size_t kMaxGraphs = 8;
    const float conf = det ? det->conf : 0.f;
    lp_engine::CachedGraph* hit = nullptr;
    for (auto& g : e->graphs)
        if (g.exec && g.x == x && g.pred == pred && g.ws == ws && g.conf == conf && g.x_dtype == x_dtype && g.epoch == e->epoch) hit = &g;
    if (!hit) {
        for (size_t i = 0; i < e->graphs.size();) {
            auto& g = e->graphs[i];
            bool drop = g.epoch != e->epoch;
            if (!drop && e->graphs.size() >= kMaxGraphs) {
                drop = true;
                for (const auto& o : e->graphs) drop = drop && o.last_use >= g.last_use;
            }
            if (!drop) { ++i; continue; }
            if (g.stream) (void)hipStreamSynchronize(g.stream);
            if (g.exec) (void)hipGraphExecDestroy(g.exec);
            e->graphs.erase(e->graphs.begin() + (long)i);
        }
        rc = ensure_lanes(e);
        if (rc) return rc;
        hipGraph_t g = nullptr;
        if (!e->cap_stream) LP_HIP_CHECK(hipStreamCreateWithFlags(&e->cap_stream, hipStreamNonBlocking));
        LP_HIP_CHECK(hipStreamBeginCapture(e->cap_stream, hipStreamCaptureModeThreadLocal));
        rc = issue(e->cap_stream);
        hipError_t ce = hipStreamEndCapture(e->cap_stream, &g);
        if (rc) { if (g) (void)hipGraphDestroy(g); return rc; }
        if (ce != hipSuccess) return fail(LP_ERR_HIP, std::string("hipStreamEndCapture: ") + hipGetErrorString(ce));
        lp_engine::CachedGraph cg;
        ce = hipGraphInstantiate(&cg.exec, g, nullptr, nullptr, 0);
        (void)hipGraphDestroy(g);
        if (ce != hipSuccess) return fail(LP_ERR_HIP, std::string("hipGraphInstantiate: ") + hipGetErrorString(ce));
        cg.x = x;
        cg.pred = pred;
        cg.ws = ws;
        cg.conf = conf;
        cg.x_dtype = x_dtype;
        cg.epoch = e->epoch;
        e->graphs.push_back(cg);
        hit = &e->graphs.back();
    }
    LP_HIP_CHECK(hipGraphLaunch(hit->exec, main_st));
    hit->stream = main_st;
    hit->last_use = ++e->graph_clock;
    return mark_done(e, main_st);
}

extern "C" int lp_engine_forward(lp_engine* e, const void* x, int x_dtype, float* pred, void* stream) {
    int rc = check_ready(e, x, x_dtype);
    if (rc) return rc;
    if (!pred) return fail(LP_ERR_ARG, "forward: pred is null");
    return run_forward(e, x, x_dtype, pred, nullptr, nullptr, (hipStream_t)stream);
}

extern "C" int lp_engine_forward_det(lp_engine* e, const void* x, int x_dtype, double conf_thres, void* workspace, size_t workspace_bytes,
                                     void* stream) {
    int rc = check_ready(e, x, x_dtype);
    if (rc) return rc;
    if (!workspace || ((uintptr_t)workspace & 255)) return fail(LP_ERR_ARG, "lp_engine_forward_det: need a 256-byte aligned workspace");
    if (!(conf_thres >= 0.0 && conf_thres <= 1.0)) return fail(LP_ERR_ARG, "lp_engine_forward_det: conf_thres must be in [0, 1]");
    DetCtx dc;
    dc.w = nms_carve(workspace, e->B, e->n_anchors);
    dc.conf = (float)conf_thres;
    if (workspace_bytes < dc.w.bytes) return fail(LP_ERR_ARG, "lp_engine_forward_det: workspace too small (lp_nms_workspace_bytes)");
    return run_forward(e, x, x_dtype, nullptr, &dc, workspace, (hipStream_t)stream);
}

static int forward_single_lane(lp_engine* e, const void* x, int x_dtype, float* pred, hipStream_t st) {
    for (size_t i = 0; i < e->ops.size(); ++i) {
        int rc = run_op(e, i, x, x_dtype, pred, st);
        if (rc) return rc;
    }
    return LP_OK;
}

extern "C" int lp_engine_profile_ops(lp_engine* e, const void* x, int x_dtype, float* pred, void* stream, float* op_ms, int reps,
                                     int inner) {
    int rc = check_ready(e, x, x_dtype);
    if (rc) return rc;
    if (!op_ms || reps < 1 || inner < 1) return fail(LP_ERR_ARG, "profile: op_ms / reps / inner");
    hipStream_t st = (hipStream_t)stream;
    const size_t n = e->ops.size();
    while (e->events.size() < n + 1) {
        hipEvent_t ev;
        LP_HIP_CHECK(hipEventCreate(&ev));
        e->events.push_back(ev);
    }
    rc = forward_single_lane(e, x, x_dtype, pred, (hipStream_t)stream);
    if (rc) return rc;
    for (size_t i = 0; i < n; ++i) op_ms[i] = 0.f;
    for (int r = 0; r < reps; ++r) {
        LP_HIP_CHECK(hipEventRecord(e->events[0], st));
        for (size_t i = 0; i < n; ++i) {
            for (int k = 0; k < inner; ++k) {
                rc = run_op(e, i, x, x_dtype, pred, st);
                if (rc) return rc;
            }
            LP_HIP_CHECK(hipEventRecord(e->events[i + 1], st));
        }
        LP_HIP_CHECK(hipEventSynchronize(e->events[n]));
        for (size_t i = 0; i < n; ++i) {
            float ms = 0.f;
            LP_HIP_CHECK(hipEventElapsedTime(&ms, e->events[i], e->events[i + 1]));
            op_ms[i] += ms / reps / inner;
        }
    }
    return LP_OK;
}

extern "C" int lp_engine_profile(lp_engine* e, const void* x, int x_dtype, float* pred, void* stream, float* op_ms, int reps) {
    return lp_engine_profile_ops(e, x, x_dtype, pred, stream, op_ms, reps, 1);
}

extern "C" int lp_engine_autotune(lp_engine* e, const void* x, int x_dtype, float* pred, void* stream, int reps) {
    int rc = check_ready(e, x, x_dtype);
    if (rc) return rc;
    if (reps < 1) reps = 3;
    hipStream_t st = (hipStream_t)stream;
    for (Op& op : e->ops) { op.planar = 0; op.fused = 0; op.fused_pw = 0; op.fused_bf = 0; }
    rc = forward_single_lane(e, x, x_dtype, pred, st);
    if (rc) return rc;
    struct EventPair {
        hipEvent_t a = nullptr, b = nullptr;
        ~EventPair() { if (a) (void)hipEventDestroy(a); if (b) (void)hipEventDestroy(b); }
    } evp;
    LP_HIP_CHECK(hipEventCreate(&evp.a));
    LP_HIP_CHECK(hipEventCreate(&evp.b));
    const hipEvent_t e0 = evp.a, e1 = evp.b;
    for (size_t i = 0; i < e->ops.size(); ++i) {
        Op& op = e->ops[i];
        if (e->launches[i].is_conv && op.kind == OP_HEAD_CLS && rows_fits(e, op) && !getenv("LP_NO_HEAD_ROWS")) {
            float best = -1.f;
            int best_rows = 0;
            for (int rows = 0; rows <= 1; ++rows) {
                op.rows = rows;
                if (prepare_op(e, i) != LP_OK || run_op(e, i, x, x_dtype, pred, st) != LP_OK) continue;
                float ms_min = -1.f;
                for (int round = 0; round < 3; ++round) {
                    LP_HIP_CHECK(hipEventRecord(e0, st));
                    for (int r = 0; r < reps; ++r) run_op(e, i, x, x_dtype, pred, st);
                    LP_HIP_CHECK(hipEventRecord(e1, st));
                    LP_HIP_CHECK(hipEventSynchronize(e1));
                    float ms = 0.f;
                    LP_HIP_CHECK(hipEventElapsedTime(&ms, e0, e1));
                    if (ms_min < 0.f || ms < ms_min) ms_min = ms;
                }
                if (best < 0.f || ms_min < best) { best = ms_min; best_rows = rows; }
            }
            op.rows = best_rows;
            rc = prepare_op(e, i);
            if (rc) return rc;
            continue;
        }
        if (!e->launches[i].is_conv || op.mode != MODE_ACT) continue;
        const int cb = conv_shape(e->dtype, op.cfg, 1, 1).CB;
        int best_cfg = op.cfg, best_nb = op.nbuf, best_tile = op.tile, best_wc = 0, best_rd = 2, best_pipe = 0;
        float best_ms = -1.f;
        int trc = LP_OK;
        auto time_current = [&]() -> float {
            if (run_op(e, i, x, x_dtype, pred, st) != LP_OK) return -1.f;
            float ms_min = -1.f;
            for (int round = 0; round < 3; ++round) {
                if (hipEventRecord(e0, st) != hipSuccess) { trc = LP_ERR_HIP; return -1.f; }
                for (int r = 0; r < reps; ++r) run_op(e, i, x, x_dtype, pred, st);
                float ms = 0.f;
                if (hipEventRecord(e1, st) != hipSuccess || hipEventSynchronize(e1) != hipSuccess ||
                    hipEventElapsedTime(&ms, e0, e1) != hipSuccess) { trc = LP_ERR_HIP; return -1.f; }
                if (ms_min < 0.f || ms < ms_min) ms_min = ms;
            }
            return ms_min;
        };
        op.stream_wc = 0;
        op.pipe = 0;
        const bool fam16 = op_fam16(e, op);
        for (int cfg = 0; cfg < CFG_COUNT && !fam16; ++cfg) {
            if (conv_shape(e->dtype, cfg, 1, 1).CB != cb) continue;
            for (int nb = 1; nb <= (cfg == CFG_C ? 1 : 2); ++nb) {
                int last_th = -1, last_tw = -1;
                for (int tile = 0; tile < 3; ++tile) {
                    op.cfg = cfg;
                    op.nbuf = nb;
                    op.tile = tile;
                    if (prepare_op(e, i) != LP_OK) continue;
                    if (e->launches[i].a.TH == last_th && e->launches[i].a.TW == last_tw) break;
                    last_th = e->launches[i].a.TH;
                    last_tw = e->launches[i].a.TW;
                    const float ms = time_current();
                    if (ms >= 0.f && (best_ms < 0.f || ms < best_ms)) { best_ms = ms; best_cfg = cfg; best_nb = nb; best_tile = tile; }
                }
            }
        }
        if (!getenv("LP_NO_STREAM") && !fam16) {
            op.cfg = best_cfg; op.nbuf = best_nb; op.tile = best_tile;
            for (int wc = 2; wc <= 4; wc += 2) {
                if (!stream_fits(e, op, wc)) continue;
                for (int rd = 2; rd <= 2; ++rd) {
                    op.stream_wc = wc;
                    op.stream_rd = rd;
                    if (prepare_op(e, i) != LP_OK) continue;
                    const float ms = time_current();
                    if (ms >= 0.f && (best_ms < 0.f || ms < best_ms)) { best_ms = ms; best_wc = wc; best_rd = rd; }
                }
            }
        }
        int pipe_tile = 0;
        if ((!getenv("LP_NO_PIPE") || fam16) && op.kind == OP_CONV) {
            op.cfg = best_cfg; op.nbuf = best_nb; op.stream_wc = 0;
            for (int pc = fam16 ? PIPE16_D : 0; pc < (fam16 ? PIPE_S2_END : PIPE_COUNT); ++pc) {
                if (fam16 && !pipe_is_16(pc)) continue;
                if (!conv_pipe_fits(e->dtype, pc, cb, op.ksize, op.stride, op.mode, op.nct, op.nphase, op.nchunks)) continue;
                int last_th = -1, last_tw = -1;
                for (int tile = 0; tile < 3; ++tile) {
                    op.pipe = pc + 1;
                    op.tile = tile;
                    if (prepare_op(e, i) != LP_OK) continue;
                    if (e->launches[i].a.TH == last_th && e->launches[i].a.TW == last_tw) break;
                    last_th = e->launches[i].a.TH;
                    last_tw = e->launches[i].a.TW;
                    const float ms = time_current();
                    if (ms >= 0.f && (best_ms < 0.f || ms < best_ms)) { best_ms = ms; best_pipe = pc + 1; pipe_tile = tile; }
                }
            }
            op.pipe = 0;
            if (fam16 && !best_pipe) best_pipe = fam16_default_pipe(e, op);
        }
        if (trc) return fail(trc, "autotune: event timing failed");
        op.cfg = best_cfg;
        op.nbuf = best_nb;
        op.tile = best_pipe ? pipe_tile : best_tile;
        op.stream_wc = best_pipe ? 0 : best_wc;
        op.stream_rd = best_rd;
        op.pipe = best_pipe;
        op.planar = 0;
        op.fused = 0;
        op.fused_pw = 0;
        rc = prepare_op(e, i);
        if (rc) return rc;
        if (i == 1 && stem_planar_possible(e) && frame_direct(e, x, x_dtype) && !getenv("LP_NO_PLANAR")) {
            float t_in = -1.f;
            for (int round = 0; round < 3 && trc == LP_OK; ++round) {
                float ms = 0.f;
                if (hipEventRecord(e0, st) != hipSuccess) { trc = LP_ERR_HIP; break; }
                for (int r = 0; r < reps; ++r) run_op(e, 0, x, x_dtype, pred, st);
                if (hipEventRecord(e1, st) != hipSuccess || hipEventSynchronize(e1) != hipSuccess || hipEventElapsedTime(&ms, e0, e1) != hipSuccess) { trc = LP_ERR_HIP; break; }
                if (t_in < 0.f || ms < t_in) t_in = ms;
            }
            int best_planar = 0, last_th = -1, last_tw = -1;
            float best_pl = -1.f;
            for (int tile = 0; tile < 3 && trc == LP_OK && t_in >= 0.f; ++tile) {
                op.planar = tile + 1;
                if (prepare_op(e, i) != LP_OK) continue;
                if (e->stem_planar.a.TH == last_th && e->stem_planar.a.TW == last_tw) break;
                last_th = e->stem_planar.a.TH;
                last_tw = e->stem_planar.a.TW;
                const float ms = time_current();
                if (ms >= 0.f && (best_pl < 0.f || ms < best_pl)) { best_pl = ms; best_planar = tile + 1; }
            }
            if (trc) return fail(trc, "autotune: event timing failed");
            op.planar = (best_planar && best_pl < best_ms + t_in) ? best_planar : 0;
            rc = prepare_op(e, i);
            if (rc) return rc;
        }
        if (i == 2 && stem2_fused_possible(e) && frame_direct(e, x, x_dtype) && !getenv("LP_NO_PLANAR") && !getenv("LP_NO_FUSED_STEM")) {
            auto time_ops = [&](size_t first, size_t last) -> float {
                float ms_min = -1.f;
                for (int round = 0; round < 3 && trc == LP_OK; ++round) {
                    float ms = 0.f;
                    if (hipEventRecord(e0, st) != hipSuccess) { trc = LP_ERR_HIP; break; }
                    for (int r = 0; r < reps; ++r)
                        for (size_t k = first; k <= last; ++k) run_op(e, k, x, x_dtype, pred, st);
                    if (hipEventRecord(e1, st) != hipSuccess || hipEventSynchronize(e1) != hipSuccess || hipEventElapsedTime(&ms, e0, e1) != hipSuccess) { trc = LP_ERR_HIP; break; }
                    if (ms_min < 0.f || ms < ms_min) ms_min = ms;
                }
                return ms_min;
            };
            op.fused = 0;
            const float t_sep = time_ops(0, 2);
            int best_f = 0, last_th = -1, last_tw = -1;
            float best_fms = -1.f;
            for (int tile = 0; tile < 3 && trc == LP_OK && t_sep >= 0.f; ++tile) {
                op.fused = tile + 1;
                if (prepare_op(e, i) != LP_OK) continue;
                if (e->stem2_fused.a.TH == last_th && e->stem2_fused.a.TW == last_tw) break;
                last_th = e->stem2_fused.a.TH;
                last_tw = e->stem2_fused.a.TW;
                if (run_op(e, 2, x, x_dtype, pred, st) != LP_OK) continue;
                const float ms = time_ops(2, 2);
                if (ms >= 0.f && (best_fms < 0.f || ms < best_fms)) { best_fms = ms; best_f = tile + 1; }
            }
            if (trc) return fail(trc, "autotune: event timing failed");
            op.fused = (best_f && best_fms < t_sep) ? best_f : 0;
            rc = prepare_op(e, i);
            if (rc) return rc;
        }
        if (pw_fused_possible(e, i) && !getenv("LP_NO_FUSED_PW")) {
            auto time_pair = [&](size_t first) -> float {
                float ms_min = -1.f;
                for (int round = 0; round < 3 && trc == LP_OK; ++round) {
                    float ms = 0.f;
                    if (hipEventRecord(e0, st) != hipSuccess) { trc = LP_ERR_HIP; break; }
                    for (int r = 0; r < reps; ++r)
                        for (size_t k = first; k <= i; ++k) run_op(e, k, x, x_dtype, pred, st);
                    if (hipEventRecord(e1, st) != hipSuccess || hipEventSynchronize(e1) != hipSuccess || hipEventElapsedTime(&ms, e0, e1) != hipSuccess) { trc = LP_ERR_HIP; break; }
                    if (ms_min < 0.f || ms < ms_min) ms_min = ms;
                }
                return ms_min;
            };
            op.fused_pw = 0;
            const float t_sep = time_pair(i - 1);
            int best_f = 0, last_th = -1, last_tw = -1;
            float best_fms = -1.f;
            for (int tile = 0; tile < 3 && trc == LP_OK && t_sep >= 0.f; ++tile) {
                op.fused_pw = tile + 1;
                if (prepare_op(e, i) != LP_OK) continue;
                const ConvArgs& fa = e->pw_fused[(int)i].a;
                if (fa.TH == last_th && fa.TW == last_tw) break;
                last_th = fa.TH;
                last_tw = fa.TW;
                if (run_op(e, i, x, x_dtype, pred, st) != LP_OK) continue;
                const float ms = time_pair(i);
                if (ms >= 0.f && (best_fms < 0.f || ms < best_fms)) { best_fms = ms; best_f = tile + 1; }
            }
            if (trc) return fail(trc, "autotune: event timing failed");
            op.fused_pw = (best_f && best_fms < t_sep) ? best_f : 0;
            rc = prepare_op(e, i);
            if (rc) return rc;
        }
        if (op.bf_up >= 0 && !getenv("LP_NO_FUSED_BF")) {
            auto time_set = [&](bool fused_form) -> float {
                float ms_min = -1.f;
                for (int round = 0; round < 3 && trc == LP_OK; ++round) {
                    float ms = 0.f;
                    if (hipEventRecord(e0, st) != hipSuccess) { trc = LP_ERR_HIP; break; }
                    for (int r = 0; r < reps; ++r) {
                        if (!fused_form) { run_op(e, (size_t)op.bf_up, x, x_dtype, pred, st); run_op(e, (size_t)op.bf_cv1, x, x_dtype, pred, st); }
                        run_op(e, i, x, x_dtype, pred, st);
                    }
                    if (hipEventRecord(e1, st) != hipSuccess || hipEventSynchronize(e1) != hipSuccess || hipEventElapsedTime(&ms, e0, e1) != hipSuccess) { trc = LP_ERR_HIP; break; }
                    if (ms_min < 0.f || ms < ms_min) ms_min = ms;
                }
                return ms_min;
            };
            op.fused_bf = 0;
            const float t_sep = time_set(false);
            op.fused_bf = 1;
            float t_fused = -1.f;
            if (prepare_op(e, i) == LP_OK && run_op(e, i, x, x_dtype, pred, st) == LP_OK) t_fused = time_set(true);
            if (trc) return fail(trc, "autotune: event timing failed");
            op.fused_bf = (t_sep >= 0.f && t_fused >= 0.f && t_fused < t_sep) ? 1 : 0;
            rc = prepare_op(e, i);
            if (rc) return rc;
        }
    }
    std::vector<std::vector<int>> choice;
    for (const Op& op : e->ops) choice.push_back({op.cfg, op.nbuf, op.tile, op.stream_wc, op.stream_rd, op.rows, op.pipe, op.planar, op.fused, op.fused_pw, op.fused_bf});
    e->tuned[{e->B, e->H, e->W}] = choice;
    return LP_OK;
}

extern "C" int lp_engine_copy_tuning(lp_engine* dst, const lp_engine* src) {
    if (!dst || !src || !dst->finalized || !src->finalized) return fail(LP_ERR_STATE, "lp_engine_copy_tuning: finalize both engines first");
    if (dst->dtype != src->dtype || dst->ops.size() != src->ops.size()) return fail(LP_ERR_ARG, "lp_engine_copy_tuning: engines differ");
    for (size_t i = 0; i < src->ops.size(); ++i) {
        const Op &a = src->ops[i], &b = dst->ops[i];
        if (a.kind != b.kind || a.ksize != b.ksize || a.stride != b.stride || a.cout != b.cout || a.nchunks != b.nchunks || a.nct != b.nct)
            return fail(LP_ERR_ARG, "lp_engine_copy_tuning: engines were built from different graphs");
    }
    dst->tuned = src->tuned;
    if (dst->arena) {
        auto it = dst->tuned.find({dst->B, dst->H, dst->W});
        if (it != dst->tuned.end())
            for (size_t i = 0; i < dst->ops.size(); ++i) {
                Op& op = dst->ops[i];
                op.cfg = it->second[i][0]; op.nbuf = it->second[i][1]; op.tile = it->second[i][2];
                op.stream_wc = it->second[i][3]; op.stream_rd = it->second[i][4]; op.rows = it->second[i][5]; op.pipe = it->second[i][6]; op.planar = it->second[i][7]; op.fused = it->second[i][8]; op.fused_pw = it->second[i][9]; op.fused_bf = it->second[i].size() > 10 ? it->second[i][10] : 0;
                int rc = prepare_op(dst, i);
                if (rc) return rc;
            }
    }
    return LP_OK;
}

extern "C" int lp_engine_set_op_variant(lp_engine* e, int op_idx, int cfg, int nbuf) {
    if (!e || !e->finalized || op_idx < 0 || op_idx >= (int)e->ops.size()) return fail(LP_ERR_ARG, "lp_engine_set_op_variant: op index");
    Op& op = e->ops[op_idx];
    if (op.kind == OP_HEAD_CLS) {
        if (cfg == LP_VARIANT_ROWS && !rows_fits(e, op)) return fail(LP_ERR_UNSUPPORTED, "lp_engine_set_op_variant: the row-writer kernel does not fit this op");
        if (cfg != LP_VARIANT_ROWS && cfg != op.cfg) return fail(LP_ERR_UNSUPPORTED, "lp_engine_set_op_variant: head_cls takes LP_VARIANT_ROWS or its packing tile");
        op.rows = cfg == LP_VARIANT_ROWS;
        e->tuned.erase({e->B, e->H, e->W});
        if (e->arena && op_idx < (int)e->launches.size()) return prepare_op(e, (size_t)op_idx);
        return LP_OK;
    }
    if (op.kind == OP_HEAD_BOX && (cfg == LP_VARIANT_BOX_SPARSE || cfg == LP_VARIANT_BOX_DENSE)) {
        op.box_sparse = cfg == LP_VARIANT_BOX_SPARSE;
        ++e->epoch;
        return LP_OK;
    }
    if (op.kind == OP_INPUT || op.kind == OP_POOL || op.mode != MODE_ACT) return fail(LP_ERR_UNSUPPORTED, "lp_engine_set_op_variant: op has no variants");
    const int ks = op.kind == OP_CONV ? op.ksize : 1, stv = op.kind == OP_CONV ? op.stride : 1;
    const int cb = conv_shape(e->dtype, op.cfg, ks, stv).CB;
    if (cfg == LP_VARIANT_FUSED_BIFUSION) {
        if (op.bf_up < 0 || nbuf != 3) return fail(LP_ERR_UNSUPPORTED, "lp_engine_set_op_variant: not the cv3 of a 64-channel BiFusion level");
        op.fused_bf = 1;
        e->tuned.erase({e->B, e->H, e->W});
        if (e->arena && op_idx < (int)e->launches.size()) return prepare_op(e, (size_t)op_idx);
        return LP_OK;
    }
    op.fused_bf = 0;
    if (cfg == LP_VARIANT_FUSED_PW_S2) {
        if (!pw_fused_possible(e, (size_t)op_idx) || nbuf != 3)
            return fail(LP_ERR_UNSUPPORTED, "lp_engine_set_op_variant: no 1x1 layer of at most 64 channels feeds this 3x3 stride-2 layer alone");
        op.fused_pw = 1;
        e->tuned.erase({e->B, e->H, e->W});
        if (e->arena && op_idx < (int)e->launches.size()) return prepare_op(e, (size_t)op_idx);
        return LP_OK;
    }
    op.fused_pw = 0;
    if (cfg == LP_VARIANT_FUSED_STEM2) {
        if (op_idx != 2 || !stem2_fused_possible(e) || nbuf != 3)
            return fail(LP_ERR_UNSUPPORTED, "lp_engine_set_op_variant: only the layer behind the stem (3x3 stride 2, <= 64 channels) has the fused form");
        op.fused = 1;
        e->tuned.erase({e->B, e->H, e->W});
        if (e->arena && op_idx < (int)e->launches.size()) return prepare_op(e, (size_t)op_idx);
        return LP_OK;
    }
    op.fused = 0;
    if (cfg == LP_VARIANT_PIPE_D + PIPE_P) {
        if (op_idx != 1 || !stem_planar_possible(e) || nbuf != 3)
            return fail(LP_ERR_UNSUPPORTED, "lp_engine_set_op_variant: only the stem over the space-to-depth image has the planar form");
        op.planar = 1;
        e->tuned.erase({e->B, e->H, e->W});
        if (e->arena && op_idx < (int)e->launches.size()) return prepare_op(e, (size_t)op_idx);
        return LP_OK;
    }
    op.planar = 0;
    if ((cfg >= LP_VARIANT_PIPE_D && cfg < LP_VARIANT_PIPE_D + PIPE_COUNT) || pipe_is_16(cfg - LP_VARIANT_PIPE_D)) {
        const int pc = cfg - LP_VARIANT_PIPE_D;
        if (!conv_pipe_fits(e->dtype, pc, cb, ks, stv, op.mode, op.nct, op.nphase, op.nchunks) || op.kind != OP_CONV || nbuf != 3)
            return fail(LP_ERR_UNSUPPORTED, "lp_engine_set_op_variant: the pipelined 3x3 kernel does not fit this op");
        op.stream_wc = 0;
        op.pipe = pc + 1;
    } else if (cfg == LP_VARIANT_STREAM64 || cfg == LP_VARIANT_STREAM128) {
        const int wc = cfg == LP_VARIANT_STREAM64 ? 2 : 4;
        if (!stream_fits(e, op, wc) || nbuf != 2)
            return fail(LP_ERR_UNSUPPORTED, "lp_engine_set_op_variant: the streaming 1x1 kernel does not fit this op");
        op.stream_wc = wc;
        op.stream_rd = nbuf;
        op.pipe = 0;
    } else {
        if (cfg < 0 || cfg >= CFG_COUNT || conv_shape(e->dtype, cfg, ks, stv).CB != cb || nbuf < 1 || nbuf > (cfg == CFG_C ? 1 : 2))
            return fail(LP_ERR_UNSUPPORTED, "lp_engine_set_op_variant: variant does not share the op's weight packing");
        op.stream_wc = 0;
        op.pipe = 0;
        op.cfg = cfg;
        op.nbuf = nbuf;
    }
    e->tuned.erase({e->B, e->H, e->W});
    if (e->arena && op_idx < (int)e->launches.size()) return prepare_op(e, (size_t)op_idx);
    return LP_OK;
}

static int* op_tile_slot(lp_engine* e, int op_idx, int* bias, const Launch** L) {
    Op& op = e->ops[(size_t)op_idx];
    if (op.kind == OP_INPUT || op.kind == OP_POOL || op.mode != MODE_ACT || op.fused_bf) return nullptr;
    const bool bound = e->arena && op_idx < (int)e->launches.size();
    *bias = 1;
    if (op.fused_pw) { *L = bound ? &e->pw_fused[op_idx] : nullptr; return &op.fused_pw; }
    if (op.fused) { *L = bound ? &e->stem2_fused : nullptr; return &op.fused; }
    if (op.planar) { *L = bound ? &e->stem_planar : nullptr; return &op.planar; }
    if (op.stream_wc && !op.pipe) return nullptr;
    *bias = 0;
    *L = bound ? &e->launches[(size_t)op_idx] : nullptr;
    return &op.tile;
}

extern "C" int lp_engine_set_op_tile(lp_engine* e, int op_idx, int choice) {
    if (!e || !e->finalized || op_idx < 0 || op_idx >= (int)e->ops.size() || choice < 0) return fail(LP_ERR_ARG, "lp_engine_set_op_tile: op index or choice");
    int bias = 0;
    const Launch* L = nullptr;
    int* slot = op_tile_slot(e, op_idx, &bias, &L);
    if (!slot) return fail(LP_ERR_UNSUPPORTED, "lp_engine_set_op_tile: the op's kernel has no output tiles");
    const int before = *slot;
    *slot = choice + bias;
    e->tuned.erase({e->B, e->H, e->W});
    if (e->arena && op_idx < (int)e->launches.size()) {
        const int rc = prepare_op(e, (size_t)op_idx);
        if (rc) { *slot = before; prepare_op(e, (size_t)op_idx); }
        return rc;
    }
    return LP_OK;
}

extern "C" int lp_engine_op_tile(const lp_engine* e, int op_idx, int* choice, int* TH, int* TW) {
    if (!e || !e->finalized || op_idx < 0 || op_idx >= (int)e->ops.size()) return fail(LP_ERR_ARG, "lp_engine_op_tile: op index");
    int bias = 0;
    const Launch* L = nullptr;
    const int* slot = op_tile_slot(const_cast<lp_engine*>(e), op_idx, &bias, &L);
    if (!slot) return fail(LP_ERR_UNSUPPORTED, "lp_engine_op_tile: the op's kernel has no output tiles");
    if (!L) return fail(LP_ERR_STATE, "lp_engine_op_tile: no shape bound");
    if (choice) *choice = *slot - bias;
    if (TH) *TH = L->a.TH;
    if (TW) *TW = L->a.TW;
    return LP_OK;
}

extern "C" int lp_engine_op_carrier(const lp_engine* e, int op, int frame_direct_) {
    if (!e || op < 0 || op >= (int)e->ops.size()) return -1;
    const Op& o = e->ops[(size_t)op];
    if (o.bf_carrier >= 0 && e->ops[(size_t)o.bf_carrier].fused_bf) return o.bf_carrier;
    if ((size_t)op + 1 < e->ops.size() && e->ops[(size_t)op + 1].fused_pw) return op + 1;
    if (frame_direct_ && e->ops.size() > 2 && e->ops[0].kind == OP_INPUT && e->ops[0].s2d) {
        if (e->ops[2].fused && op <= 1) return 2;
        if (e->ops[1].planar && op == 0) return 1;
    }
    return -1;
}

extern "C" int lp_engine_op_variant(const lp_engine* e, int op, int* cfg, int* nbuf) {
    if (!e || op < 0 || op >= (int)e->ops.size()) return fail(LP_ERR_ARG, "lp_engine_op_variant: op index");
    const bool stream = e->ops[op].stream_wc != 0;
    if (e->ops[op].fused_bf) {
        if (cfg) *cfg = LP_VARIANT_FUSED_BIFUSION;
        if (nbuf) *nbuf = 3;
        return LP_OK;
    }
    if (e->ops[op].fused_pw) {
        if (cfg) *cfg = LP_VARIANT_FUSED_PW_S2;
        if (nbuf) *nbuf = 3;
        return LP_OK;
    }
    if (e->ops[op].fused) {
        if (cfg) *cfg = LP_VARIANT_FUSED_STEM2;
        if (nbuf) *nbuf = 3;
        return LP_OK;
    }
    if (e->ops[op].planar) {
        if (cfg) *cfg = LP_VARIANT_PIPE_D + PIPE_P;
        if (nbuf) *nbuf = 3;
        return LP_OK;
    }
    if (e->ops[op].pipe) {
        if (cfg) *cfg = LP_VARIANT_PIPE_D + e->ops[op].pipe - 1;
        if (nbuf) *nbuf = 3;
        return LP_OK;
    }
    if (cfg) *cfg = e->ops[op].rows ? LP_VARIANT_ROWS : stream ? (e->ops[op].stream_wc == 2 ? LP_VARIANT_STREAM64 : LP_VARIANT_STREAM128) : e->ops[op].cfg;
    if (nbuf) *nbuf = stream ? e->ops[op].stream_rd : e->ops[op].nbuf;
    return LP_OK;
}
```

### yolo-lp_amd/csrc/lp_internal.h

```cpp
#pragma once
#include <hip/hip_runtime.h>
#include <stdint.h>
#include <stddef.h>
#include <atomic>
#include <string>

#include "../../include/lp_hip.h"

#ifndef LP_PRO_ORDER
#define LP_PRO_ORDER 0
#endif

namespace lp {

typedef _Float16 f16;
typedef __bf16 bf16;

void set_error(const std::string& msg);
int fail(int code, const std::string& msg);
#define LP_HIP_CHECK(expr)                                                                       \
    do {                                                                                         \
        hipError_t _e = (expr);                                                                  \
        if (_e != hipSuccess)                                                                    \
            return ::lp::fail(LP_ERR_HIP, std::string(#expr) + ": " + hipGetErrorString(_e));    \
    } while (0)

template <typename K> inline int set_max_lds_once(K kernel, int bytes, std::atomic<unsigned long long>& done, const char* what) {
    int dev = 0;
    if (hipGetDevice(&dev) != hipSuccess || dev < 0 || dev >= 64) dev = -1;
    if (dev >= 0 && ((done.load(std::memory_order_acquire) >> dev) & 1ull)) return LP_OK;
    hipError_t e = hipFuncSetAttribute((const void*)kernel, hipFuncAttributeMaxDynamicSharedMemorySize, bytes);
    if (e != hipSuccess) return fail(LP_ERR_HIP, std::string(what) + ": LDS attribute: " + hipGetErrorString(e));
    if (dev >= 0) done.fetch_or(1ull << dev, std::memory_order_release);
    return LP_OK;
}

__device__ __forceinline__ void resize_coef(int d, double scale, int src, int* s0, int* a0, int* a1) {
    float f = (float)((d + 0.5) * scale - 0.5);
    int s = (int)floorf(f);
    f -= (float)s;
    if (s < 0) { f = 0.f; s = 0; }
    if (s >= src - 1) { f = 0.f; s = src - 1; }
    *s0 = s;
    const float c0 = (1.f - f) * 2048.f, c1 = f * 2048.f;
    *a0 = (int)rintf(c0);
    *a1 = (int)rintf(c1);
}
__device__ __forceinline__ int resize_blend(int t00, int t01, int t10, int t11, int a0, int a1, int b0, int b1) {
    const int h0v = t00 * a0 + t01 * a1;
    const int h1v = t10 * a0 + t11 * a1;
    return (((b0 * (h0v >> 4)) >> 16) + ((b1 * (h1v >> 4)) >> 16) + 2) >> 2;
}
constexpr int LETTERBOX_PAD = 114;

std::string plane_fault(const unsigned char* y, const unsigned char* uv, int pitch_y, int pitch_uv, int h0, int w0, int matrix);

inline size_t dtype_size(int dt) { return dt == LP_F32 ? 4 : 2; }
inline int round_up(int x, int m) { return (x + m - 1) / m * m; }
inline int ceil_div(int a, int b) { return (a + b - 1) / b; }

enum ConvMode { MODE_ACT = 0, MODE_PRED = 1, MODE_DECODE = 2 };
enum ConvCfg { CFG_A = 0 , CFG_B = 1 , CFG_C = 2 , CFG_D = 3 , CFG_E = 4 , CFG_F = 5 , CFG_COUNT = 6 };

enum PipeCfgId { PIPE_D = 0 , PIPE_B = 1 , PIPE_F = 2 , PIPE_C = 3 , PIPE_P = 4 , PIPE_COUNT = 5,
                 PIPE_FUSED2 = 5 ,
                 PIPE_FUSED_PW = 6 ,
                 PIPE_FUSED_BF = 13 ,
                 PIPE16_D = 7, PIPE16_F = 9 ,
                 PIPE16_V0 = 10, PIPE16_V1 = 11 , PIPE_END = 12,
                 PIPE16_S2A = 16, PIPE16_S2B = 17 , PIPE_S2_END = 18 };
inline bool pipe_is_16s2(int pcfg) { return pcfg == PIPE16_S2A || pcfg == PIPE16_S2B; }
inline bool pipe_is_16(int pcfg) { return pcfg == PIPE16_D || pcfg == PIPE16_F || pcfg == PIPE16_V0 || pcfg == PIPE16_V1 || pipe_is_16s2(pcfg); }
inline bool pipe_is_16v(int pcfg) { return pcfg == PIPE16_V0 || pcfg == PIPE16_V1; }

struct ConvSrc {
    const void* ptr;
    int cs;
};

struct ConvArgs {
    ConvSrc src[LP_MAX_SRC];
    int chunk_begin[LP_MAX_SRC + 1];
    int nsrc;
    const void* w;
    const float* bias;
    unsigned long long* stamps;
    const void* zero;
    void* trash;
    void* out;
    void* out2;
    int out_split;
    int out2_pix_stride;
    long long out2_img_stride;
    const void* res;
    int res_cs;
    float alpha;
    int B, H, W;
    int Ho, Wo;
    int TH, TW, tiles_x, tiles_y;
    unsigned tw_magic, hp_magic;
    int hpitch;
    int nct;
    int out_c;
    long long out_img_stride;
    int out_pix_stride;
    int out_scale;
    int nphase;
    long long w_phase_stride;
    int act;
    int det_mode;
    unsigned long long* det_keys;
    int* det_cnt;
    int det_np, det_n, det_anchor0;
    float det_conf;
    const int* det_prev;
    int* det_snap;
    const void* fz_w1;
    const float* fz_b1;
    int fz_act1, fz_c1;
    const void* bf_wd;
    const float* bf_bd;
    long long bf_wd_phase_stride;
    int reg_bins;
    const float* proj;
    float stride_px;
};

struct ConvShape {
    int CB, PB, KC, HPMAX, NT, WP, WGC, WGP;
};
ConvShape conv_shape(int dtype, int cfg, int ksize, int stride);
void conv_pick_tile(const ConvShape& s, int ksize, int stride, int Ho, int Wo, int choice, int* TH, int* TW);
int conv_pick_pitch(const ConvShape& s, int dtype, int ksize, int stride, int TH, int TW);
int conv_pick_pitch16(const ConvShape& s, int TH, int TW);
void conv_pick_tile16v(const ConvShape& s, int Ho, int Wo, int B, int nct, int choice, int* TH, int* TW, int stride = 1);
int device_cus();
int conv_launch(int dtype, int cfg, int mode, int ksize, int stride, int nbuf, const ConvArgs& a, hipStream_t st);
bool stem_planar_tile(int Ho, int Wo, int choice, int* TH, int* TW);
bool stem2_fused_tile(int Ho, int Wo, int choice, int* TH, int* TW, int* hpitch);

int conv_stream_lds(int dtype, int wc, int nchunks, int cb_pack);
int conv_stream_launch(int dtype, int wc, const ConvArgs& a, int cb_pack, hipStream_t st);

ConvShape conv_pipe_shape(int pcfg);
bool conv_pipe_fits(int dtype, int pcfg, int cb_pack, int ksize, int stride, int mode, int nct, int nphase, int nchunks);
int conv_pipe_launch(int dtype, int pcfg, const ConvArgs& a, hipStream_t st);

bool head_rows_fits(int dtype, int nchunks, int cb_pack, int out_c);
bool head_det_fits(int dtype, int nchunks, int cb_pack, int out_c);
bool head_box_det_fits(const ConvArgs& a, int cb_pack, int ksize, int stride);
int head_box_det_launch(int dtype, const ConvArgs& a, int cb_pack, hipStream_t st);
int head_rows_launch(int dtype, const ConvArgs& a, int cb_pack, hipStream_t st);

struct NmsWs {
    int32_t* cnt;
    unsigned long long* keys;
    float* rows;
    float4* sbox;
    int32_t* kept;
    int NP;
    size_t bytes;
};
NmsWs nms_carve(void* base, int B, int N);
int nms_score_launch(float* pred, int B, int rows_per_img, int anchor0, int N, float conf_f, const NmsWs& w, bool write_box, hipStream_t st);
int zero_counts_launch(int* p, int n, hipStream_t st);

int input_launch(const void* x, int x_dtype, void* dst, int dtype, int B, int H, int W, hipStream_t st);
int input_s2d_launch(const void* x, int x_dtype, void* dst, int dtype, int B, int H, int W, hipStream_t st);
size_t pool_min_lds_bytes(int dtype, int h, int w);
constexpr size_t POOL_MAX_LDS = 128 * 1024;
int pool_launch(const void* src, void* d1, void* d2, void* d3, int dtype, int B, int h, int w, int cs, hipStream_t st);

}
```

### yolo-lp_amd/yolov6/hip/abi.py

```python
import ctypes
import os
from ctypes import POINTER, c_char_p, c_double, c_float, c_int, c_int32, c_size_t, c_void_p

LP_F16, LP_BF16, LP_F32 = 0, 1, 2
LP_ACT_NONE, LP_ACT_RELU, LP_ACT_SILU = 0, 1, 2
LP_PRED_COLS, LP_DET_COLS, LP_MAX_SRC = 290, 28, 4
LP_VARIANT_STREAM64, LP_VARIANT_STREAM128, LP_VARIANT_ROWS = 16, 17, 18
LP_VARIANT_PIPE_D, LP_VARIANT_PIPE_B, LP_VARIANT_PIPE_F, LP_VARIANT_PIPE_C = 32, 33, 34, 35
LP_VARIANT_PIPE16_D, LP_VARIANT_PIPE16_F = 39, 41
LP_VARIANT_PIPE16_V0, LP_VARIANT_PIPE16_V1 = 42, 43
LP_VARIANT_PIPE16_S2A, LP_VARIANT_PIPE16_S2B = 48, 49
LP_VARIANT_FUSED_BIFUSION = 45
LP_VARIANT_BOX_SPARSE, LP_VARIANT_BOX_DENSE = 46, 47
LP_VARIANT_FUSED_PW_S2 = 38
LP_VARIANT_FUSED_STEM2 = 37
LP_VARIANT_PIPE_P = 36
VARIANT_SHORT = {
    LP_VARIANT_STREAM64: 'S', LP_VARIANT_STREAM128: 'W', LP_VARIANT_ROWS: 'R',
    LP_VARIANT_PIPE_D: 'Pd', LP_VARIANT_PIPE_B: 'Pb', LP_VARIANT_PIPE_F: 'Pf', LP_VARIANT_PIPE_C: 'Pc', LP_VARIANT_PIPE_P: 'Pp',
    LP_VARIANT_FUSED_STEM2: 'Fz', LP_VARIANT_FUSED_PW_S2: 'Fp', LP_VARIANT_FUSED_BIFUSION: 'Fb',
    LP_VARIANT_PIPE16_D: 'Md', LP_VARIANT_PIPE16_F: 'Mf', LP_VARIANT_PIPE16_V0: 'V0', LP_VARIANT_PIPE16_V1: 'V1',
    LP_VARIANT_PIPE16_S2A: 'Xa', LP_VARIANT_PIPE16_S2B: 'Xb',
}
LP_FRAMES_PER_LAUNCH = 64
LP_NV12_PER_LAUNCH = 32
LP_MERGE_MAX_TILES, LP_MERGE_MAX_CANDIDATES = 64, 16384
LP_TRACK_MAX_TRACKS, LP_TRACK_MAX_DETS, LP_TRACK_MAX_CLS = 128, 128, 64
LP_REDACT_MAX_CELL = 64
LP_REDACT_MAX_RADIUS = 48
LP_LOOKBACK_MAX_DEPTH = 32
LP_WATCH_MAX_ENTRIES, LP_WATCH_MAX_COST = 1 << 24, 32768
LP_WATCH_BLOCK_ENTRIES, LP_WATCH_QUERY_BLOCK = 2048, 16
LP_TILE_GATE_TILE_WORDS = 8
LP_EVAL_NCOUNTS = 43

_PKG_ROOT = os.path.dirname(os.path.dirname(os.path.dirname(os.path.abspath(__file__))))
LIB_PATH = os.environ.get('LP_HIP_LIB') or os.path.join(_PKG_ROOT, 'libyololp_hip.so')
CSRC_DIR = os.path.join(_PKG_ROOT, 'csrc')


class FrameDesc(ctypes.Structure):
    _fields_ = [('img', c_void_p), ('h0', c_int), ('w0', c_int), ('rh', c_int), ('rw', c_int), ('top', c_int), ('left', c_int)]


class RescaleDesc(ctypes.Structure):
    _fields_ = [('ratio', c_double), ('padx', c_double), ('pady', c_double), ('img_w', c_int), ('img_h', c_int)]


class CropDesc(ctypes.Structure):
    _fields_ = [('img', c_void_p), ('h0', c_int), ('w0', c_int), ('max_crops', c_int), ('out_slot', c_int)]


class TileDesc(ctypes.Structure):
    _fields_ = [('img', c_void_p), ('h0', c_int), ('w0', c_int), ('y0', c_int), ('x0', c_int), ('th', c_int), ('tw', c_int),
                ('rh', c_int), ('rw', c_int), ('top', c_int), ('left', c_int)]


class Nv12Desc(ctypes.Structure):
    _fields_ = [('y', c_void_p), ('uv', c_void_p), ('pitch_y', c_int), ('pitch_uv', c_int), ('h0', c_int), ('w0', c_int),
                ('y0', c_int), ('x0', c_int), ('th', c_int), ('tw', c_int), ('rh', c_int), ('rw', c_int), ('top', c_int),
                ('left', c_int), ('matrix', c_int)]


class Nv12BgrDesc(ctypes.Structure):
    _fields_ = [('y', c_void_p), ('uv', c_void_p), ('pitch_y', c_int), ('pitch_uv', c_int), ('h0', c_int), ('w0', c_int),
                ('matrix', c_int), ('out', c_void_p)]


class RedactDesc(ctypes.Structure):
    _fields_ = [('p0', c_void_p), ('p1', c_void_p), ('pitch0', c_int), ('pitch1', c_int), ('h0', c_int), ('w0', c_int),
                ('format', c_int)]


class RedactParams(ctypes.Structure):
    _fields_ = [('mode', c_int), ('cell', c_int), ('margin', c_double), ('fill', ctypes.c_ubyte * 3)]


class RedactGaussParams(ctypes.Structure):
    _fields_ = [('margin', c_double), ('radius', c_int), ('radius_c', c_int), ('taps', ctypes.c_uint16 * (LP_REDACT_MAX_RADIUS + 1)),
                ('taps_c', ctypes.c_uint16 * (LP_REDACT_MAX_RADIUS + 1))]


class TileGateDesc(ctypes.Structure):
    _fields_ = [('p0', c_void_p), ('pitch0', c_int), ('h0', c_int), ('w0', c_int), ('format', c_int), ('blocks', c_void_p)]


class TileRef(ctypes.Structure):
    _fields_ = [('frame', c_int), ('y0', c_int), ('x0', c_int), ('th', c_int), ('tw', c_int)]


class TrackParams(ctypes.Structure):
    _fields_ = [('match_thres', c_double), ('new_thres', c_double), ('expand', c_double), ('max_age', c_int), ('ncls', c_int * 8)]


class TrackHoldParams(ctypes.Structure):
    _fields_ = [('min_hits', c_int), ('max_misses', c_int)]


class ConvDesc(ctypes.Structure):
    _fields_ = [('n_src', c_int), ('src', c_int * LP_MAX_SRC), ('dst', c_int), ('ksize', c_int), ('stride', c_int),
                ('act', c_int), ('res', c_int), ('res_alpha', c_float), ('weight', c_void_p), ('bias', c_void_p), ('dst2', c_int)]


SYMBOLS = {
    'lp_version': (c_char_p, []),
    'lp_last_error': (c_char_p, []),
    'lp_engine_create': (c_int, [POINTER(c_void_p), c_int]),
    'lp_engine_destroy': (None, [c_void_p]),
    'lp_engine_tensor': (c_int, [c_void_p, c_int, c_int]),
    'lp_engine_set_lane': (c_int, [c_void_p, c_int]),
    'lp_engine_add_input': (c_int, [c_void_p, c_int]),
    'lp_engine_add_conv': (c_int, [c_void_p, POINTER(ConvDesc)]),
    'lp_engine_add_deconv2x2': (c_int, [c_void_p, c_int, c_int, c_void_p, c_void_p]),
    'lp_engine_add_pool5_chain': (c_int, [c_void_p, c_int, c_int, c_int, c_int]),
    'lp_engine_add_head_cls': (c_int, [c_void_p, c_int, c_int, c_int, c_void_p, c_void_p]),
    'lp_engine_add_head_box': (c_int, [c_void_p, c_int, c_int, c_int, c_void_p, c_void_p, c_void_p]),
    'lp_engine_finalize': (c_int, [c_void_p, c_int]),
    'lp_engine_weight_bytes': (c_size_t, [c_void_p]),
    'lp_engine_upload': (c_int, [c_void_p, c_void_p, c_void_p]),
    'lp_engine_arena_bytes': (c_size_t, [c_void_p, c_int, c_int, c_int]),
    'lp_engine_bind': (c_int, [c_void_p, c_void_p, c_size_t, c_int, c_int, c_int]),
    'lp_engine_tensor_info': (c_int, [c_void_p, c_int, POINTER(c_size_t), POINTER(c_int), POINTER(c_int),
                                      POINTER(c_int), POINTER(c_int)]),
    'lp_engine_num_anchors': (c_int, [c_void_p]),
    'lp_engine_forward': (c_int, [c_void_p, c_void_p, c_int, c_void_p, c_void_p]),
    'lp_engine_set_graph': (c_int, [c_void_p, c_int]),
    'lp_engine_set_single_lane': (c_int, [c_void_p, c_int]),
    'lp_engine_set_mfma16': (c_int, [c_void_p, c_int]),
    'lp_engine_op_carrier': (c_int, [c_void_p, c_int, c_int]),
    'lp_engine_num_ops': (c_int, [c_void_p]),
    'lp_engine_op_info': (c_int, [c_void_p, c_int, POINTER(c_int), POINTER(c_int), POINTER(c_int), POINTER(c_int),
                                  POINTER(c_double), POINTER(c_double)]),
    'lp_engine_forward_det': (c_int, [c_void_p, c_void_p, c_int, ctypes.c_double, c_void_p, c_size_t, c_void_p]),
    'lp_nms_candidates': (c_int, [c_int, c_int, ctypes.c_double, c_int, c_void_p, c_void_p, c_void_p, c_void_p, c_size_t, c_void_p]),
    'lp_engine_profile': (c_int, [c_void_p, c_void_p, c_int, c_void_p, c_void_p, POINTER(c_float), c_int]),
    'lp_engine_profile_ops': (c_int, [c_void_p, c_void_p, c_int, c_void_p, c_void_p, POINTER(c_float), c_int, c_int]),
    'lp_engine_autotune': (c_int, [c_void_p, c_void_p, c_int, c_void_p, c_void_p, c_int]),
    'lp_engine_op_variant': (c_int, [c_void_p, c_int, POINTER(c_int), POINTER(c_int)]),
    'lp_engine_set_op_variant': (c_int, [c_void_p, c_int, c_int, c_int]),
    'lp_engine_set_op_tile': (c_int, [c_void_p, c_int, c_int]),
    'lp_engine_op_tile': (c_int, [c_void_p, c_int, POINTER(c_int), POINTER(c_int), POINTER(c_int)]),
    'lp_engine_copy_tuning': (c_int, [c_void_p, c_void_p]),
    'lp_nms_workspace_bytes': (c_size_t, [c_int, c_int]),
    'lp_nms_candidate_counts': (c_void_p, [c_void_p, c_int, c_int]),
    'lp_preprocess_letterbox': (c_int, [c_void_p, c_int, c_int, c_void_p, c_int, c_int, c_int, c_int, c_int, c_int, c_int,
                                        c_void_p]),
    'lp_rescale_round': (c_int, [c_void_p, c_int, c_double, c_double, c_double, c_int, c_int, c_void_p]),
    'lp_preprocess_letterbox_batch': (c_int, [POINTER(FrameDesc), c_int, c_int, c_void_p, c_int, c_int, c_int, c_void_p]),
    'lp_rescale_round_batch': (c_int, [c_void_p, c_void_p, c_int, c_int, POINTER(RescaleDesc), c_void_p]),
    'lp_preprocess_tiles_batch': (c_int, [POINTER(TileDesc), c_int, c_int, c_void_p, c_int, c_int, c_int, c_void_p]),
    'lp_preprocess_nv12_batch': (c_int, [POINTER(Nv12Desc), c_int, c_int, c_void_p, c_int, c_int, c_int, c_void_p]),
    'lp_nv12_to_bgr_batch': (c_int, [POINTER(Nv12BgrDesc), c_int, c_void_p]),
    'lp_merge_tiles_workspace_bytes': (c_size_t, [c_int, c_int]),
    'lp_merge_tiles': (c_int, [c_void_p, c_void_p, POINTER(TileRef), c_int, c_int, POINTER(c_int), c_int, c_double, c_int, c_int, c_int,
                               c_void_p, c_void_p, c_void_p, c_void_p, c_size_t, c_void_p]),
    'lp_track_state_bytes': (c_size_t, [c_int, c_int]),
    'lp_track_dropped_offset': (c_size_t, [c_int, c_int]),
    'lp_track_update': (c_int, [c_void_p, c_int, c_int, POINTER(TrackParams), c_void_p, c_void_p, c_int, c_int, POINTER(c_int),
                                c_void_p, c_void_p, c_void_p, c_void_p, c_void_p, c_void_p, c_int, c_void_p]),
    'lp_track_update_slots': (c_int, [c_void_p, c_int, c_int, POINTER(TrackParams), c_void_p, c_void_p, c_int, c_int, POINTER(c_int),
                                      c_void_p, c_void_p, c_void_p, c_void_p, c_void_p, c_void_p, c_void_p, c_int, c_void_p]),
    'lp_track_update_hold': (c_int, [c_void_p, c_int, c_int, POINTER(TrackParams), c_void_p, c_void_p, c_int, c_int, POINTER(c_int),
                                     c_void_p, c_void_p, c_void_p, c_void_p, c_void_p, c_void_p, c_void_p, c_int,
                                     POINTER(TrackHoldParams), c_void_p, c_void_p, c_void_p, c_void_p]),
    'lp_plate_crops_batch': (c_int, [POINTER(CropDesc), c_int, c_void_p, c_void_p, c_int, c_void_p, c_void_p, c_int, c_int, c_int,
                                     c_void_p]),
    'lp_crop_sharpness': (c_int, [c_void_p, c_void_p, c_int, c_int, c_int, c_void_p, c_void_p]),
    'lp_best_shot_state_bytes': (c_size_t, [c_int, c_int, c_int, c_int]),
    'lp_best_shot_update': (c_int, [c_void_p, c_int, c_int, c_int, c_int, c_void_p, c_void_p, c_int, c_int, c_void_p, c_void_p, c_void_p,
                                    c_void_p, c_void_p, c_int, POINTER(c_int), c_void_p, c_void_p, c_int, c_double, c_void_p, c_void_p,
                                    c_void_p, c_void_p, c_void_p]),
    'lp_redact_workspace_bytes': (c_size_t, [POINTER(RedactDesc), c_int, POINTER(RedactParams)]),
    'lp_redact_plates_batch': (c_int, [POINTER(RedactDesc), c_int, c_void_p, c_void_p, c_int, POINTER(RedactParams), c_void_p, c_void_p,
                                       c_size_t, c_void_p]),
    'lp_redact_gauss_workspace_bytes': (c_size_t, [POINTER(RedactDesc), c_int, POINTER(RedactGaussParams)]),
    'lp_redact_gauss_batch': (c_int, [POINTER(RedactDesc), c_int, c_void_p, c_void_p, c_int, POINTER(RedactGaussParams), c_void_p, c_void_p,
                                      c_size_t, c_void_p]),
    'lp_lookback_state_bytes': (c_size_t, [c_int, c_int, c_int, c_int]),
    'lp_lookback_update': (c_int, [c_void_p, c_int, c_int, c_int, c_int, c_int, c_void_p, c_void_p, c_void_p, c_void_p, c_int, c_int, c_int,
                                   POINTER(c_int), c_void_p, c_void_p, c_void_p, c_void_p, c_void_p, c_void_p, c_void_p, c_void_p]),
    'lp_watch_workspace_bytes': (c_size_t, [c_int, c_int]),
    'lp_watch_match': (c_int, [c_void_p, c_int, c_void_p, c_void_p, c_void_p, c_void_p, c_int, c_int, c_int, c_int, c_void_p, c_void_p,
                               c_size_t, c_void_p]),
    'lp_tile_gate_luma_batch': (c_int, [POINTER(TileGateDesc), c_int, c_void_p]),
    'lp_tile_gate_update': (c_int, [POINTER(TileGateDesc), c_int, POINTER(c_int), c_int, c_void_p, POINTER(c_int), c_int, c_void_p,
                                    ctypes.c_longlong, c_void_p, c_int, c_int, c_int, c_void_p, c_void_p, c_void_p]),
    'lp_eval_counts': (c_int, [c_void_p, c_void_p, c_int, c_void_p, c_void_p, c_int, c_int, c_void_p, c_void_p]),
    'lp_check_sigmoid_monotone': (c_int, [c_void_p, c_void_p]),
    'lp_debug_poison_lds': (c_int, [c_void_p]),
    'lp_check_iou_predicate': (c_int, [c_void_p, ctypes.c_longlong, c_double, c_void_p, c_void_p]),
    'lp_plan_stem_tile': (c_int, [c_int, c_int, c_int, c_int, c_void_p, c_void_p, c_void_p]),
    'lp_plan_block_tile': (c_int, [c_int, c_int, c_int, c_int, c_int, c_int, c_void_p, c_void_p, c_void_p]),
    'lp_nms': (c_int, [c_void_p, c_int, c_int, c_double, c_double, c_int, c_void_p, c_void_p, c_void_p, c_void_p,
                       c_size_t, c_void_p]),
}

_lib = None


def load():
    global _lib
    if _lib is None:
        import torch
        if not os.path.exists(LIB_PATH):
            raise RuntimeError('HIP extension %s is missing: build it with `make -C %s` (or '
                               '`python -c "import __graft_entry__ as g; g.build()"`). The GPU path has no '
                               'eager fallback.' % (LIB_PATH, CSRC_DIR))
        lib = ctypes.CDLL(LIB_PATH)
        for name, (restype, argtypes) in SYMBOLS.items():
            fn = getattr(lib, name)
            fn.restype = restype
            fn.argtypes = argtypes
        _lib = lib
    return _lib


def check(rc, what=''):
    if rc < 0:
        msg = load().lp_last_error()
        raise RuntimeError('%s failed (%d): %s' % (what or 'libyololp_hip', rc, msg.decode() if msg else '?'))
    return rc
```

### yolo-lp_amd/yolov6/hip/runtime.py

```python
import copy
import ctypes
import os
import weakref

import numpy as np
import torch
import torch.nn as nn

from yolov6.core.frames import letterbox_placement
from yolov6.core.tiles import hw_pair, plan_frames, tiles_per_frame
from yolov6.hip import abi
from yolov6.layers import common as L
from yolov6.utils.lookback import LookbackHost
from yolov6.utils.nv12 import Nv12Frame, is_nv12_list

DET_CROSSOVER = 0.5
_DT = {torch.float16: abi.LP_F16, torch.bfloat16: abi.LP_BF16, torch.float32: abi.LP_F32}
_TORCH_DT = {v: k for k, v in _DT.items()}
CLS_HEADS = ('pro', 'alp', 'ad0', 'ad1', 'ad2', 'ad3', 'ad4', 'ad5')
OP_KINDS = ('input', 'conv', 'deconv', 'pool', 'head_cls', 'head_box', 'stem')


def _dptr(t):
    return None if t is None else ctypes.c_void_p(t.data_ptr())
# ... 361 lines not shown

    def tensor_view(self, tid):
        off, c, cs, h, w = ctypes.c_size_t(), ctypes.c_int(), ctypes.c_int(), ctypes.c_int(), ctypes.c_int()
        abi.check(self.lib.lp_engine_tensor_info(self.h, tid, ctypes.byref(off), ctypes.byref(c), ctypes.byref(cs),
                                                 ctypes.byref(h), ctypes.byref(w)), 'lp_engine_tensor_info')
        B = self.bound[0]
        esz = torch.empty(0, dtype=self.dtype).element_size()
        base = _aligned(self.arena) - self.arena.data_ptr() + off.value
        n = B * h.value * w.value * cs.value
        flat = self.arena[base:base + n * esz].view(self.dtype)
        return flat.view(B, h.value, w.value, cs.value)[..., :c.value].permute(0, 3, 1, 2)

    def prepare(self, B, H, W, x_dtype=None):
        if not self._untuned((B, H, W)):
            return
        x = torch.zeros(B, 3, H, W, dtype=x_dtype or self.dtype, device=self.device)
        graph = self.graph
        if graph:
            self.set_graph(False)
        try:
            self.forward(x)
            torch.cuda.current_stream(self.device).synchronize()
        finally:
            if graph:
                self.set_graph(True)

    @staticmethod
    def _check_input(x):
        if x.dim() != 4 or x.shape[1] != 3:
            raise ValueError('expected [B,3,H,W], got %s' % (tuple(x.shape),))
        if x.dtype not in _DT:
            raise TypeError('unsupported input dtype %s' % x.dtype)
        return x.contiguous(), (x.shape[0], x.shape[2], x.shape[3])

    def _new_pred(self, B):
        return torch.empty(B, self.n_anchors, abi.LP_PRED_COLS, dtype=torch.float32, device=self.device)

    def _untuned(self, shape):
        return self.autotune and shape not in self.tuned and len(self.tuned) < self.max_tuned_shapes

    def forward(self, x):
        x, shape = self._check_input(x)
        with torch.cuda.device(self.device):
            cur = self._stream_enter()
            self.bind(*shape)
            if self.graph:
                if self._graph_pred is None or self._graph_pred.shape != (shape[0], self.n_anchors, abi.LP_PRED_COLS):
                    self._graph_pred = self._new_pred(shape[0])
                pred = self._graph_pred
                x = self._stage_for_graph(x)
            else:
                pred = self._new_pred(shape[0])
            if self._untuned(shape):
                abi.check(self.lib.lp_engine_autotune(self.h, _dptr(x), _DT[x.dtype], _dptr(pred), _stream_ptr(self.device), 5),
                          'lp_engine_autotune')
                self.tuned.add(shape)
            abi.check(self.lib.lp_engine_forward(self.h, _dptr(x), _DT[x.dtype], _dptr(pred), _stream_ptr(self.device)),
                      'lp_engine_forward')
            self._stream_leave(cur)
        return pred

    def _stage_for_graph(self, x):
        gx = self._graph_x
        if gx is None or gx.shape != x.shape or gx.dtype != x.dtype:
            gx = self._graph_x = torch.empty_like(x)
        if gx.data_ptr() != x.data_ptr():
            gx.copy_(x)
        return gx

    def forward_det(self, x, conf_thres, ws=None):
        x, shape = self._check_input(x)
        if not 0.0 <= conf_thres <= 1.0:
            raise ValueError('conf_thres must be in [0, 1]')
        with torch.cuda.device(self.device):
            if self._untuned(shape):
                self.forward(x)
            cur = self._stream_enter()
            self.bind(*shape)
            B, N = shape[0], self.n_anchors
            need = self.lib.lp_nms_workspace_bytes(B, N)
            if ws is None:
                ws = _nms_workspace(self.device, need)
            elif ws.numel() < need + 256:
                raise ValueError('workspace too small: %d bytes needed' % (need + 256))
            if self.graph:
                x = self._stage_for_graph(x)
            abi.check(self.lib.lp_engine_forward_det(self.h, _dptr(x), _DT[x.dtype], float(conf_thres), _aligned(ws), need,
                                                     _stream_ptr(self.device)), 'lp_engine_forward_det')
            self._stream_leave(cur)
        return ws, B, N

    def det_workspace(self, B, H, W):
        with torch.cuda.device(self.device):
            self.bind(B, H, W)
            return torch.empty(self.lib.lp_nms_workspace_bytes(B, self.n_anchors) + 256, dtype=torch.uint8, device=self.device)

    def detect(self, x, conf_thres, iou_thres, max_det, want_keep=False, route=None):
        if route is None:
            self._poll_pass_rate()
            route = 'pred' if (self.pass_rate is not None and self.pass_rate > self.det_crossover) else 'det'
        self.det_routes[route] += 1
        if route == 'pred':
            pred = self.forward(x)
            out = nms_padded(pred, conf_thres, iou_thres, max_det, want_keep)
            self._probe_pass_rate(_nms_workspace(self.device, 0), pred.shape[0], pred.shape[1])
            return out
        handle = self.forward_det(x, conf_thres)
        out = nms_candidates(handle, iou_thres, max_det, want_keep)
        self._probe_pass_rate(*handle)
        return out

    def _probe_pass_rate(self, ws, B, N):
        with torch.cuda.device(self.device):
            ptr = self.lib.lp_nms_candidate_counts(_aligned(ws), B, N)
            off = ptr - ws.data_ptr()
            pr = self._pass_probe
            if pr is None or pr[0].numel() != B:
                pr = (torch.empty(B, dtype=torch.int32).pin_memory(), torch.cuda.Event(), N)
            pr[0].copy_(ws[off:off + 4 * B].view(torch.int32), non_blocking=True)
            pr[1].record(torch.cuda.current_stream(self.device))
            self._pass_probe = (pr[0], pr[1], N)

    def _poll_pass_rate(self):
        pr = self._pass_probe
        if pr is not None and pr[1].query():
            self.pass_rate = float(pr[0].float().mean()) / max(1, pr[2])

    def op_kinds(self):
        return [self._op_info(i)['kind'] for i in range(self.lib.lp_engine_num_ops(self.h))]

    def _op_info(self, i):
        kind, ks, cin, cout = ctypes.c_int(), ctypes.c_int(), ctypes.c_int(), ctypes.c_int()
        fl, by = ctypes.c_double(), ctypes.c_double()
        abi.check(self.lib.lp_engine_op_info(self.h, i, ctypes.byref(kind), ctypes.byref(ks), ctypes.byref(cin),
                                             ctypes.byref(cout), ctypes.byref(fl), ctypes.byref(by)), 'lp_engine_op_info')
        return dict(kind=OP_KINDS[kind.value], ksize=ks.value, cin=cin.value, cout=cout.value, flops=fl.value, bytes=by.value)

    def profile(self, x, reps=3, inner=1):
        x = x.contiguous()
        B, _, H, W = x.shape
        with torch.cuda.device(self.device):
            self.bind(B, H, W)
            pred = self._new_pred(B)
            n = self.lib.lp_engine_num_ops(self.h)
            ms = (ctypes.c_float * n)()
            abi.check(self.lib.lp_engine_profile_ops(self.h, _dptr(x), _DT[x.dtype], _dptr(pred), _stream_ptr(self.device), ms, reps,
                                                     inner), 'lp_engine_profile_ops')
        ops = []
        for i in range(n):
            cfg, nb = ctypes.c_int(), ctypes.c_int()
            self.lib.lp_engine_op_variant(self.h, i, ctypes.byref(cfg), ctypes.byref(nb))
            ops.append(dict(self._op_info(i), ms=float(ms[i]),
                            variant='%s%d' % (abi.VARIANT_SHORT.get(cfg.value) or 'ABCDEFGH'[cfg.value], nb.value)))
        direct = x.dtype == self.dtype
        for o in ops:
            o['flops_own'], o['bytes_own'] = o['flops'], o['bytes']
        for j, c in enumerate(ops):
            i = self.lib.lp_engine_op_carrier(self.h, j, 1 if direct else 0)
            if i < 0 or i == j:
                continue
            ops[i]['flops'] += c['flops']
            c.update(flops=0.0, bytes=0.0, ms=0.0, carried_by=i, variant=c['variant'] + '>%d' % i)
        return ops


def _weights_version(model):
    return sum(t._version for t in list(model.parameters()) + list(model.buffers()))


_engines = weakref.WeakKeyDictionary()


def drop_engine(model):
    _engines.pop(model, None)


def engine_for(model, dtype=None):
    p = next(model.parameters())
    if not p.is_cuda:
        raise RuntimeError('model is not on a GPU')
    dtype = dtype or getattr(model, 'lp_dtype', None) or p.dtype
    if dtype not in _DT:
        raise TypeError('unsupported activation dtype %s' % dtype)
    key = (dtype, p.device, _weights_version(model))
    cached = _engines.get(model)
    if cached is None or cached[0] != key:
        cached = (key, Engine.from_model(model, dtype, p.device))
        _engines[model] = cached
    return cached[1]


def _engine(model):
    eng = engine_for(model)
    if bool(getattr(model, 'lp_graph', False)) != eng.graph:
        eng.set_graph(getattr(model, 'lp_graph', False))
    return eng


def prepare_for(model, shape, x_dtype=None):
    _engine(model).prepare(int(shape[0]), int(shape[2]), int(shape[3]), x_dtype)


def model_forward(model, x):
    eng = _engine(model)
    pred = eng.forward(x)
    return [pred, [eng.tensor_view(t) for t in eng.neck_ids]]


def _det_buffers(B, max_det, device, index=True):
    return (torch.empty(B, max_det, abi.LP_DET_COLS, dtype=torch.float32, device=device),
            torch.empty(B, dtype=torch.int32, device=device),
            torch.empty(B, max_det, dtype=torch.int32, device=device) if index else None)


def nms_candidates(handle, iou_thres, max_det, want_keep=False):
    ws, B, N = handle
    if not 0.0 <= iou_thres <= 1.0:
        raise ValueError('iou_thres must be in [0, 1]')
    lib = abi.load()
    dev = ws.device
    with torch.cuda.device(dev):
        need = lib.lp_nms_workspace_bytes(B, N)
        det, count, keep = _det_buffers(B, max_det, dev, want_keep)
        abi.check(lib.lp_nms_candidates(B, N, float(iou_thres), int(max_det), _dptr(det), _dptr(count), _dptr(keep), _aligned(ws),
                                        need, _stream_ptr(dev)), 'lp_nms_candidates')
    return det, count, keep


def detect_padded(model, x, conf_thres, iou_thres, max_det, want_keep=False, route=None):
    return _engine(model).detect(x, conf_thres, iou_thres, max_det, want_keep, route)


def _unpad(det, counts, n=None):
    return [det[b, :counts[b]] for b in range(len(counts) if n is None else n)]


def detect(model, x, conf_thres, iou_thres, max_det, route=None):
    det, count, _ = detect_padded(model, x, conf_thres, iou_thres, max_det, route=route)
    return _unpad(det, count.cpu().tolist())


_nms_ws, _redact_ws = {}, {}


def _stream_workspace(cache, device, need):
    key = (device, torch.cuda.current_stream(device).cuda_stream)
    ws = cache.get(key)
    if ws is None or ws.numel() < need + 256:
        ws = cache[key] = torch.empty(need + 256, dtype=torch.uint8, device=device)
    return ws


def _nms_workspace(device, need):
    return _stream_workspace(_nms_ws, device, need)


def nms_padded(prediction, conf_thres, iou_thres, max_det, want_keep=False):
    if not (prediction.is_cuda and prediction.dtype == torch.float32 and prediction.is_contiguous()):
        raise ValueError('prediction must be a contiguous fp32 CUDA tensor')
    B, N, C = prediction.shape
    if C != abi.LP_PRED_COLS:
        raise ValueError('prediction must have %d columns, got %d' % (abi.LP_PRED_COLS, C))
    lib = abi.load()
    dev = prediction.device
    with torch.cuda.device(dev):
        need = lib.lp_nms_workspace_bytes(B, N)
        ws = _nms_workspace(dev, need)
        det, count, keep = _det_buffers(B, max_det, dev, want_keep)
        abi.check(lib.lp_nms(_dptr(prediction), B, N, float(conf_thres), float(iou_thres), int(max_det), _dptr(det), _dptr(count),
                             _dptr(keep), _aligned(ws), need, _stream_ptr(dev)), 'lp_nms')
    return det, count, keep


def non_max_suppression(prediction, conf_thres, iou_thres, max_det):
    B, N = prediction.shape[0], prediction.shape[1]
    if B == 0 or N == 0:
        return [torch.zeros((0, 28), device=prediction.device)] * B
    src = prediction
    work = prediction
    if work.dtype != torch.float32 or not work.is_contiguous():
        work = work.float().contiguous()
    det, count, _ = nms_padded(work, conf_thres, iou_thres, max_det)
    if work is not src:
        src.copy_(work)
    return _unpad(det, count.cpu().tolist())


def _frames_device(frames):
    dev = frames[0].device
    for f in frames:
        if not (f.is_cuda and f.device == dev and f.dtype == torch.uint8 and f.dim() == 3 and f.shape[2] == 3 and f.is_contiguous()):
            raise ValueError('frames must be contiguous uint8 CUDA tensors [h, w, 3] on one device')
    return dev


def _nv12_device(frames):
    dev = frames[0].device
    for f in frames:
        if not (isinstance(f, Nv12Frame) and f.is_cuda and f.device == dev):
            raise ValueError('NV12 frames must be Nv12Frame objects with CUDA planes on one device')
    return dev


def _frames_on(frames, what='frames'):
    if is_nv12_list(frames, what):
        return _nv12_device(frames), True
# ... 924 lines not shown
```

Before: 17970 images/s.

## Add wave-per-tile head detection kernel with autotuned selection

Adds a new fused classification-head + detection kernel where each wavefront independently processes 32-pixel tiles, with weights staged in LDS and cross-half reductions via permlane32 swaps. This replaces the block-level row writer for 16-bit heads with at most two K-chunks. Autotune times both variants and keeps the faster one, and an env flag can disable it. The cost is extra code paths and another tuning step.

Measured after the change: 18270 images/s, median of 6. About the same (+1.7%).

```diff
diff --git a/include/lp_hip.h b/include/lp_hip.h
--- a/include/lp_hip.h
+++ b/include/lp_hip.h
@@ -91,6 +91,8 @@
 enum { LP_VARIANT_FUSED_BIFUSION = 45 };
 enum { LP_VARIANT_BOX_SPARSE = 46, LP_VARIANT_BOX_DENSE = 47 };
 enum { LP_VARIANT_PIPE16_S2A = 48, LP_VARIANT_PIPE16_S2B = 49 };
+enum { LP_VARIANT_HEAD_DET_WAVE = 50, LP_VARIANT_HEAD_DET = 51 };
+int lp_engine_op_det_variant(const lp_engine* e, int op, int* cfg);
 int lp_engine_op_carrier(const lp_engine* e, int op, int frame_direct);
 int lp_engine_autotune(lp_engine* e, const void* x, int x_dtype, float* pred, void* stream, int reps);
 int lp_engine_op_variant(const lp_engine* e, int op, int* cfg, int* nbuf);
diff --git a/yolo-lp_amd/csrc/lp_conv.hip b/yolo-lp_amd/csrc/lp_conv.hip
--- a/yolo-lp_amd/csrc/lp_conv.hip
+++ b/yolo-lp_amd/csrc/lp_conv.hip
@@ -18,6 +18,8 @@
 int head_rows_launch_f16(const ConvArgs& a, int cb_pack, hipStream_t st);
 int head_rows_launch_bf16(const ConvArgs& a, int cb_pack, hipStream_t st);
 int head_rows_launch_f32(const ConvArgs& a, int cb_pack, hipStream_t st);
+int head_det_wave_launch_f16(const ConvArgs& a, int cb_pack, hipStream_t st);
+int head_det_wave_launch_bf16(const ConvArgs& a, int cb_pack, hipStream_t st);
 int head_box_det_launch_f16(const ConvArgs& a, int cb_pack, hipStream_t st);
 int head_box_det_launch_bf16(const ConvArgs& a, int cb_pack, hipStream_t st);
 int head_box_det_launch_f32(const ConvArgs& a, int cb_pack, hipStream_t st);
@@ -359,6 +361,17 @@
            out_c == LP_PRED_COLS - 13;
 }
 
+bool head_det_wave_fits(int dtype, int nchunks, int cb_pack, int out_c) {
+    return head_det_fits(dtype, nchunks, cb_pack, out_c) && dtype != LP_F32 && nchunks <= 2;
+}
+int head_det_wave_launch(int dtype, const ConvArgs& a, int cb_pack, hipStream_t st) {
+    if (!a.det_mode || !head_det_wave_fits(dtype, a.chunk_begin[a.nsrc], cb_pack, a.out_c)) return fail(LP_ERR_ARG, "head det wave: op does not fit");
+    for (int i = 0; i < a.nsrc; ++i)
+        if (a.src[i].cs % 16 != 0) return fail(LP_ERR_ARG, "head det wave: source channels are not whole 32-byte K-steps");
+    if (a.nphase != 1 || a.out_scale != 1 || a.Ho != a.H || a.Wo != a.W || !a.out) return fail(LP_ERR_ARG, "head det wave: bad geometry");
+    return dtype == LP_F16 ? head_det_wave_launch_f16(a, cb_pack, st) : head_det_wave_launch_bf16(a, cb_pack, st);
+}
+
 bool head_box_det_fits(const ConvArgs& a, int cb_pack, int ksize, int stride) {
     const int nchunks = a.chunk_begin[a.nsrc];
     return ksize == 1 && stride == 1 && a.nsrc == 1 && nchunks >= 1 && nchunks <= 4 && a.reg_bins == 1 && a.out_c == 12 && a.nct == 1 &&
diff --git a/yolo-lp_amd/csrc/lp_conv_bf16.hip b/yolo-lp_amd/csrc/lp_conv_bf16.hip
--- a/yolo-lp_amd/csrc/lp_conv_bf16.hip
+++ b/yolo-lp_amd/csrc/lp_conv_bf16.hip
@@ -1,6 +1,7 @@
 #include "lp_conv_kernel.inc"
 #include "lp_conv1x1_stream.inc"
 #include "lp_head_rows.inc"
+#include "lp_head_det_wave.inc"
 #include "lp_head_box.inc"
 #include "lp_conv3x3_pipe.inc"
 #include "lp_conv3x3_pipe16.inc"
@@ -19,6 +20,7 @@
     return stream_launch_dtype<bf16>(wc, a, cb_pack, lds, st);
 }
 int head_rows_launch_bf16(const ConvArgs& a, int cb_pack, hipStream_t st) { return head_rows_launch_dtype<bf16>(a, cb_pack, st); }
+int head_det_wave_launch_bf16(const ConvArgs& a, int cb_pack, hipStream_t st) { return head_det_wave_launch_dtype<bf16>(a, cb_pack, st); }
 int head_box_det_launch_bf16(const ConvArgs& a, int cb_pack, hipStream_t st) { return head_box_det_launch_dtype<bf16>(a, cb_pack, st); }
 int conv_pipe_launch_bf16(int pcfg, const ConvArgs& a, int ncu, hipStream_t st) {
     if (pcfg == PIPE_FUSED2) return stem2_fused_launch<bf16>(a, ncu, st);
diff --git a/yolo-lp_amd/csrc/lp_conv_f16.hip b/yolo-lp_amd/csrc/lp_conv_f16.hip
--- a/yolo-lp_amd/csrc/lp_conv_f16.hip
+++ b/yolo-lp_amd/csrc/lp_conv_f16.hip
@@ -1,6 +1,7 @@
 #include "lp_conv_kernel.inc"
 #include "lp_conv1x1_stream.inc"
 #include "lp_head_rows.inc"
+#include "lp_head_det_wave.inc"
 #include "lp_head_box.inc"
 #include "lp_conv3x3_pipe.inc"
 #include "lp_conv3x3_pipe16.inc"
@@ -19,6 +20,7 @@
     return stream_launch_dtype<f16>(wc, a, cb_pack, lds, st);
 }
 int head_rows_launch_f16(const ConvArgs& a, int cb_pack, hipStream_t st) { return head_rows_launch_dtype<f16>(a, cb_pack, st); }
+int head_det_wave_launch_f16(const ConvArgs& a, int cb_pack, hipStream_t st) { return head_det_wave_launch_dtype<f16>(a, cb_pack, st); }
 int head_box_det_launch_f16(const ConvArgs& a, int cb_pack, hipStream_t st) { return head_box_det_launch_dtype<f16>(a, cb_pack, st); }
 int conv_pipe_launch_f16(int pcfg, const ConvArgs& a, int ncu, hipStream_t st) {
     if (pcfg == PIPE_FUSED2) return stem2_fused_launch<f16>(a, ncu, st);
diff --git a/yolo-lp_amd/csrc/lp_engine.hip b/yolo-lp_amd/csrc/lp_engine.hip
--- a/yolo-lp_amd/csrc/lp_engine.hip
+++ b/yolo-lp_amd/csrc/lp_engine.hip
@@ -1,5 +1,6 @@
 #include "lp_internal.h"
 
+#include <cctype>
 #include <cmath>
 #include <cstdlib>
 #include <cstring>
@@ -46,6 +47,7 @@
     int stream_wc = 0, stream_rd = 2;
     int rows = 0;
     size_t det_scratch = (size_t)-1;
+    int det_wave = -1;
     int box_sparse = 1;
     int pipe = 0;
     int fused_pw = 0;
@@ -605,7 +607,7 @@
     if (!e->dev_w) return fail(LP_ERR_STATE, "lp_engine_bind: upload the weights first");
     auto it = e->tuned.find({B, H, W});
     if (it != e->tuned.end())
-        for (size_t i = 0; i < e->ops.size(); ++i) { e->ops[i].cfg = it->second[i][0]; e->ops[i].nbuf = it->second[i][1]; e->ops[i].tile = it->second[i][2]; e->ops[i].stream_wc = it->second[i][3]; e->ops[i].stream_rd = it->second[i][4]; e->ops[i].rows = it->second[i][5]; e->ops[i].pipe = it->second[i][6]; e->ops[i].planar = it->second[i][7]; e->ops[i].fused = it->second[i][8]; e->ops[i].fused_pw = it->second[i][9]; e->ops[i].fused_bf = it->second[i].size() > 10 ? it->second[i][10] : 0; }
+        for (size_t i = 0; i < e->ops.size(); ++i) { e->ops[i].cfg = it->second[i][0]; e->ops[i].nbuf = it->second[i][1]; e->ops[i].tile = it->second[i][2]; e->ops[i].stream_wc = it->second[i][3]; e->ops[i].stream_rd = it->second[i][4]; e->ops[i].rows = it->second[i][5]; e->ops[i].pipe = it->second[i][6]; e->ops[i].planar = it->second[i][7]; e->ops[i].fused = it->second[i][8]; e->ops[i].fused_pw = it->second[i][9]; e->ops[i].fused_bf = it->second[i].size() > 10 ? it->second[i][10] : 0; e->ops[i].det_wave = it->second[i].size() > 11 ? it->second[i][11] : -1; }
     e->launches.assign(e->ops.size(), Launch());
     for (size_t i = 0; i < e->ops.size(); ++i) {
         int rc = prepare_op(e, i);
@@ -691,6 +693,20 @@
     }
     return head_det_fits(e->dtype, op.nchunks, conv_shape(e->dtype, op.cfg, 1, 1).CB, op.cout);
 }
+
+static bool env_flag(const char* name) {
+    const char* v = getenv(name);
+    if (!v || !*v) return false;
+    std::string s(v);
+    for (char& c : s) c = (char)tolower((unsigned char)c);
+    return !(s == "0" || s == "false" || s == "no" || s == "off");
+}
+
+static bool det_wave_fits(const lp_engine* e, const Op& op) {
+    static const bool no_wave = env_flag("LP_NO_HEAD_DET_WAVE");
+    return !no_wave && det_fits(e, op) && head_det_wave_fits(e->dtype, op.nchunks, conv_shape(e->dtype, op.cfg, 1, 1).CB, op.cout);
+}
+static bool det_wave_now(const lp_engine* e, const Op& op) { return op.det_wave != 0 && det_wave_fits(e, op); }
 
 static bool op_fam16(const lp_engine* e, const Op& op) {
     if (!e->mfma16 || e->dtype == LP_F32 || op.kind != OP_CONV || op.ksize != 3 || op.mode != MODE_ACT) return false;
@@ -978,7 +994,7 @@
         a.det_n = N;
         a.det_anchor0 = anchor0;
         a.det_conf = dc.conf;
-        return head_rows_launch(dt, a, L.cb_pack, st);
+        return det_wave_now(e, op) ? head_det_wave_launch(dt, a, L.cb_pack, st) : head_rows_launch(dt, a, L.cb_pack, st);
     }
     float* const scratch = (float*)(e->arena + op.det_scratch);
     const int rpi = a.Ho * a.Wo;
@@ -1243,8 +1259,40 @@
     LP_HIP_CHECK(hipEventCreate(&evp.a));
     LP_HIP_CHECK(hipEventCreate(&evp.b));
     const hipEvent_t e0 = evp.a, e1 = evp.b;
+    struct DetWs {
+        void* p = nullptr;
+        ~DetWs() { if (p) (void)hipFree(p); }
+    } det_ws;
     for (size_t i = 0; i < e->ops.size(); ++i) {
         Op& op = e->ops[i];
+        if (e->launches[i].is_conv && op.kind == OP_HEAD_CLS && op.det_scratch == (size_t)-1 && det_wave_fits(e, op)) {
+            DetCtx dc;
+            dc.w = nms_carve(nullptr, e->B, e->n_anchors);
+            if (!det_ws.p) LP_HIP_CHECK(hipMalloc(&det_ws.p, dc.w.bytes));
+            dc.w = nms_carve(det_ws.p, e->B, e->n_anchors);
+            dc.conf = 0.25f;
+            float best = -1.f;
+            int best_wave = 0;
+            for (int wv = 0; wv <= 1; ++wv) {
+                op.det_wave = wv;
+                float ms_min = -1.f;
+                for (int round = 0; round < 4; ++round) {
+                    LP_HIP_CHECK(hipEventRecord(e0, st));
+                    for (int r = 0; r < reps; ++r) {
+                        LP_HIP_CHECK(hipMemsetAsync(dc.w.cnt, 0, (size_t)e->B * 4, st));
+                        rc = run_head_det(e, i, dc, st);
+                        if (rc) return rc;
+                    }
+                    LP_HIP_CHECK(hipEventRecord(e1, st));
+                    LP_HIP_CHECK(hipEventSynchronize(e1));
+                    float ms = 0.f;
+                    LP_HIP_CHECK(hipEventElapsedTime(&ms, e0, e1));
+                    if (round > 0 && (ms_min < 0.f || ms < ms_min)) ms_min = ms;
+                }
+                if (best < 0.f || ms_min < best) { best = ms_min; best_wave = wv; }
+            }
+            op.det_wave = best_wave;
+        }
         if (e->launches[i].is_conv && op.kind == OP_HEAD_CLS && rows_fits(e, op) && !getenv("LP_NO_HEAD_ROWS")) {
             float best = -1.f;
             int best_rows = 0;
@@ -1469,7 +1517,7 @@
         }
     }
     std::vector<std::vector<int>> choice;
-    for (const Op& op : e->ops) choice.push_back({op.cfg, op.nbuf, op.tile, op.stream_wc, op.stream_rd, op.rows, op.pipe, op.planar, op.fused, op.fused_pw, op.fused_bf});
+    for (const Op& op : e->ops) choice.push_back({op.cfg, op.nbuf, op.tile, op.stream_wc, op.stream_rd, op.rows, op.pipe, op.planar, op.fused, op.fused_pw, op.fused_bf, op.det_wave});
     e->tuned[{e->B, e->H, e->W}] = choice;
     return LP_OK;
 }
@@ -1489,7 +1537,7 @@
             for (size_t i = 0; i < dst->ops.size(); ++i) {
                 Op& op = dst->ops[i];
                 op.cfg = it->second[i][0]; op.nbuf = it->second[i][1]; op.tile = it->second[i][2];
-                op.stream_wc = it->second[i][3]; op.stream_rd = it->second[i][4]; op.rows = it->second[i][5]; op.pipe = it->second[i][6]; op.planar = it->second[i][7]; op.fused = it->second[i][8]; op.fused_pw = it->second[i][9]; op.fused_bf = it->second[i].size() > 10 ? it->second[i][10] : 0;
+                op.stream_wc = it->second[i][3]; op.stream_rd = it->second[i][4]; op.rows = it->second[i][5]; op.pipe = it->second[i][6]; op.planar = it->second[i][7]; op.fused = it->second[i][8]; op.fused_pw = it->second[i][9]; op.fused_bf = it->second[i].size() > 10 ? it->second[i][10] : 0; op.det_wave = it->second[i].size() > 11 ? it->second[i][11] : -1;
                 int rc = prepare_op(dst, i);
                 if (rc) return rc;
             }
@@ -1500,6 +1548,15 @@
 extern "C" int lp_engine_set_op_variant(lp_engine* e, int op_idx, int cfg, int nbuf) {
     if (!e || !e->finalized || op_idx < 0 || op_idx >= (int)e->ops.size()) return fail(LP_ERR_ARG, "lp_engine_set_op_variant: op index");
     Op& op = e->ops[op_idx];
+    if (op.kind == OP_HEAD_CLS && (cfg == LP_VARIANT_HEAD_DET_WAVE || cfg == LP_VARIANT_HEAD_DET)) {
+        if (cfg == LP_VARIANT_HEAD_DET_WAVE ? !det_wave_fits(e, op) : !det_fits(e, op))
+            return fail(LP_ERR_UNSUPPORTED, cfg == LP_VARIANT_HEAD_DET_WAVE ? "lp_engine_set_op_variant: head_det_wave_kernel does not fit this op (16-bit, at most two K-chunks)"
+                                                                            : "lp_engine_set_op_variant: head_det_kernel does not fit this op");
+        op.det_wave = cfg == LP_VARIANT_HEAD_DET_WAVE;
+        e->tuned.erase({e->B, e->H, e->W});
+        ++e->epoch;
+        return LP_OK;
+    }
     if (op.kind == OP_HEAD_CLS) {
         if (cfg == LP_VARIANT_ROWS && !rows_fits(e, op)) return fail(LP_ERR_UNSUPPORTED, "lp_engine_set_op_variant: the row-writer kernel does not fit this op");
         if (cfg != LP_VARIANT_ROWS && cfg != op.cfg) return fail(LP_ERR_UNSUPPORTED, "lp_engine_set_op_variant: head_cls takes LP_VARIANT_ROWS or its packing tile");
@@ -1633,6 +1690,16 @@
     return -1;
 }
 
+extern "C" int lp_engine_op_det_variant(const lp_engine* e, int op, int* cfg) {
+    if (!e || !e->finalized || op < 0 || op >= (int)e->ops.size()) return fail(LP_ERR_ARG, "lp_engine_op_det_variant: op index");
+    const Op& o = e->ops[(size_t)op];
+    int v = 0;
+    if (o.kind == OP_HEAD_CLS && det_fits(e, o)) v = det_wave_now(e, o) ? LP_VARIANT_HEAD_DET_WAVE : LP_VARIANT_HEAD_DET;
+    if (o.kind == OP_HEAD_BOX) v = o.box_sparse ? LP_VARIANT_BOX_SPARSE : LP_VARIANT_BOX_DENSE;
+    if (cfg) *cfg = v;
+    return LP_OK;
+}
+
 extern "C" int lp_engine_op_variant(const lp_engine* e, int op, int* cfg, int* nbuf) {
     if (!e || op < 0 || op >= (int)e->ops.size()) return fail(LP_ERR_ARG, "lp_engine_op_variant: op index");
     const bool stream = e->ops[op].stream_wc != 0;
diff --git a/yolo-lp_amd/csrc/lp_head_det_wave.inc b/yolo-lp_amd/csrc/lp_head_det_wave.inc
--- /dev/null
+++ b/yolo-lp_amd/csrc/lp_head_det_wave.inc
@@ -0,0 +1,325 @@
+#pragma once
+#include "lp_head_rows.inc"
+
+namespace lp {
+
+constexpr int HEAD_WAVE_STG = HEAD_ROWS_PITCH + 32;
+constexpr int HEAD_WAVE_DENSE = 4;
+
+static inline int head_det_wave_lds_bytes(int nch, int nw) {
+    return nch * HEAD_ROWS_NT * 32 * 128 + HEAD_ROWS_NT * 32 * 4 + nw * HEAD_WAVE_STG;
+}
+
+__device__ __forceinline__ float hw_pair_max(float v) {
+    const auto s = __builtin_amdgcn_permlane32_swap(__float_as_uint(v), __float_as_uint(v), false, false);
+    return __builtin_fmaxf(__uint_as_float(s[0]), __uint_as_float(s[1]));
+}
+__device__ __forceinline__ int hw_pair_min(int v) {
+    const auto s = __builtin_amdgcn_permlane32_swap((unsigned)v, (unsigned)v, false, false);
+    const int x = (int)s[0], y = (int)s[1];
+    return x < y ? x : y;
+}
+__device__ __forceinline__ unsigned hw_pair_or(unsigned v) {
+    const auto s = __builtin_amdgcn_permlane32_swap(v, v, false, false);
+    return s[0] | s[1];
+}
+
+template <typename T, int NCH, int NW>
+__global__ __launch_bounds__(NW * 64, 8 / NW) void head_det_wave_kernel(const ConvArgs a, const int cb_pack, const int nwaves) {
+    typedef typename Mma<T>::V V;
+    constexpr int SZ = sizeof(T), EPG = 16 / SZ, KC = 128 / SZ, ROWB = 128, NKB = 4, GPR = 8;
+    constexpr int NT = HEAD_ROWS_NT, PXT = 32, PITCH = HEAD_ROWS_PITCH, NTHR = NW * 64;
+    extern __shared__ __attribute__((aligned(1024))) char smem[];
+    char* const wres = smem;
+    float* const bias_lds = (float*)(smem + NCH * NT * 32 * ROWB);
+
+    const int tid = threadIdx.x, lane = tid & 63, wave = __builtin_amdgcn_readfirstlane(tid >> 6);
+    const int r = lane & 31, h = lane >> 5;
+    char* const stg = (char*)(bias_lds + NT * 32) + wave * HEAD_WAVE_STG;
+    const unsigned uHW = (unsigned)(a.Ho * a.Wo);
+    const unsigned uM = (unsigned)a.B * uHW;
+    constexpr int SEGS[9] = {0, 31, 55, 92, 129, 166, 203, 240, 277};
+
+    for (int i = tid; i < NT * 32; i += NTHR) bias_lds[i] = i < a.out_c ? a.bias[i] : 0.f;
+    for (int i = wave; i < NCH * NT * 4; i += NW) {
+        const int q = i / (NT * 4), rem = i - q * (NT * 4), t = rem >> 2, part = rem & 3;
+        const int ctp = (t * 32) / cb_pack, row0 = (t * 32) % cb_pack;
+        const char* src = (const char*)((const T*)a.w + (((long long)ctp * NCH + q) * cb_pack + row0) * KC) + part * 1024 + lane * 16;
+        __builtin_amdgcn_global_load_lds((gbl_ptr_t)src, (lds_ptr_t)(wres + (q * NT + t) * (32 * ROWB) + part * 1024), 16, 0, 0);
+    }
+    asm volatile("s_waitcnt vmcnt(0)" ::: "memory");
+    __syncthreads();
+
+    const unsigned ntiles = (uM + PXT - 1) / PXT;
+    const unsigned gw = blockIdx.x * NW + wave;
+    if (gw >= ntiles) return;
+    const int my_tiles = (int)((ntiles - gw + nwaves - 1) / nwaves);
+    const unsigned mstride = (unsigned)nwaves * PXT;
+
+    const char* cbase[NCH];
+    int ccs[NCH], crem[NCH];
+#pragma unroll
+    for (int q = 0; q < NCH; ++q) {
+        int s = 0;
+#pragma unroll
+        for (int k = 1; k < LP_MAX_SRC; ++k)
+            if (k < a.nsrc && q >= a.chunk_begin[k]) s = k;
+        ccs[q] = a.src[s].cs;
+        crem[q] = a.src[s].cs - (q - a.chunk_begin[s]) * KC;
+        cbase[q] = (const char*)((const T*)a.src[s].ptr + (q - a.chunk_begin[s]) * KC);
+    }
+    auto issue = [&](V(&dst)[NKB], int q, unsigned m0, bool live) {
+        const int cs = ccs[q];
+        const char* const base = live ? cbase[q] + (long long)m0 * cs * SZ : (const char*)a.zero;
+        const unsigned remu = uM - m0;
+        const int rem = remu < (unsigned)PXT ? (int)remu : PXT;
+        const int row = r < rem ? r : rem - 1;
+        const unsigned voff = live ? (unsigned)((row * cs + h * EPG) * SZ) : 0u;
+#pragma unroll
+        for (int kb = 0; kb < NKB; ++kb) {
+            V v = {};
+            if (kb * (32 / SZ) + h * EPG < crem[q] || !live) v = *(const V*)(base + voff + kb * 32);
+            dst[kb] = v;
+        }
+    };
+    int aoff[NKB];
+#pragma unroll
+    for (int kb = 0; kb < NKB; ++kb) aoff[kb] = r * ROWB + swz(r, 2 * kb + h, GPR) * 16;
+
+    f32x16 acc[NT];
+    V cur[NCH][NKB], nx[NCH][NKB];
+    unsigned m0 = gw * PXT;
+    unsigned b_first = m0 / uHW, off0 = m0 - b_first * uHW;
+    const unsigned step_b = mstride / uHW, step_off = mstride - step_b * uHW;
+    bool p_pass = false;
+    unsigned long long p_key = 0;
+    long long p_pos = 0;
+    int p_base = 0, p_leader = 0;
+#pragma unroll
+    for (int q = 0; q < NCH; ++q) issue(cur[q], q, m0, true);
+#pragma unroll
+    for (int q = 0; q < NCH; ++q)
+#pragma unroll
+        for (int kb = 0; kb < NKB; ++kb) asm volatile("" : "+v"(cur[q][kb]));
+    for (int t = 0; t < my_tiles; ++t) {
+#pragma unroll
+        for (int j = 0; j < NT; ++j) {
+            const float* bp = bias_lds + j * 32 + 4 * h;
+#pragma unroll
+            for (int rg = 0; rg < 4; ++rg) {
+                const f32x4 bv = *(const f32x4*)(bp + 8 * rg);
+                acc[j][4 * rg + 0] = bv[0]; acc[j][4 * rg + 1] = bv[1]; acc[j][4 * rg + 2] = bv[2]; acc[j][4 * rg + 3] = bv[3];
+            }
+        }
+#pragma unroll
+        for (int q = 0; q < NCH; ++q) {
+            const char* const wl = wres + q * NT * (32 * ROWB);
+#pragma unroll
+            for (int kb = 0; kb < NKB; ++kb)
+#pragma unroll
+                for (int j0 = 0; j0 < NT; j0 += 3) {
+                    V fa[3];
+#pragma unroll
+                    for (int j = 0; j < 3; ++j) fa[j] = *(const V*)(wl + aoff[kb] + (j0 + j) * 32 * ROWB);
+#pragma unroll
+                    for (int j = 0; j < 3; ++j) acc[j0 + j] = Mma<T>::mma(fa[j], cur[q][kb], acc[j0 + j]);
+                }
+        }
+        __builtin_amdgcn_sched_barrier(0);
+#pragma unroll
+        for (int q = 0; q < NCH; ++q) issue(nx[q], q, m0 + mstride, t + 1 < my_tiles);
+        __builtin_amdgcn_sched_barrier(0);
+        float pm[8];
+        unsigned nanbits = 0;
+        {
+            bool anyn = false;
+#pragma unroll
+            for (int k = 0; k < 8; ++k) pm[k] = -INFINITY;
+            hd_static_for<NT * 16>([&](auto itag) {
+                constexpr int I = decltype(itag)::value, j = I / 16, rg = (I % 16) / 4, e = I % 4;
+                constexpr int c0 = j * 32 + 8 * rg + e, c1 = c0 + 4;
+                constexpr int k0 = head_of_col(c0), k1 = head_of_col(c1);
+                const float v = acc[j][4 * rg + e];
+                if constexpr (k0 == k1) {
+                    if constexpr (k0 < 8) { pm[k0] = __builtin_fmaxf(pm[k0], v); anyn |= v != v; }
+                } else {
+                    if constexpr (k0 < 8) { pm[k0] = __builtin_fmaxf(pm[k0], h == 0 ? v : -INFINITY); anyn |= h == 0 && v != v; }
+                    if constexpr (k1 < 8) { pm[k1] = __builtin_fmaxf(pm[k1], h == 1 ? v : -INFINITY); anyn |= h == 1 && v != v; }
+                }
+            });
+            if (__ballot(anyn)) {
+                hd_static_for<NT * 16>([&](auto itag) {
+                    constexpr int I = decltype(itag)::value, j = I / 16, rg = (I % 16) / 4, e = I % 4;
+                    constexpr int c0 = j * 32 + 8 * rg + e, c1 = c0 + 4;
+                    constexpr int k0 = head_of_col(c0), k1 = head_of_col(c1);
+                    const float v = acc[j][4 * rg + e];
+                    if constexpr (k0 < 8) nanbits |= (v != v && (k0 == k1 || h == 0)) ? 1u << k0 : 0u;
+                    if constexpr (k1 < 8 && k1 != k0) nanbits |= (v != v && h == 1) ? 1u << k1 : 0u;
+                    if constexpr (e == 3) asm volatile("" : "+v"(nanbits));
+                });
+                nanbits = hw_pair_or(nanbits);
+            }
+#pragma unroll
+            for (int k = 0; k < 8; ++k) {
+                const float m = hw_pair_max(pm[k]);
+                pm[k] = ((nanbits >> k) & 1u) ? __builtin_nanf("") : m;
+            }
+        }
+        float cf[8];
+#pragma unroll
+        for (int k = 0; k < 8; ++k) cf[k] = act_c<ACT_SIGMOID>(pm[k]);
+        const bool one_image = off0 + PXT <= uHW || b_first + 1 == (unsigned)a.B;
+        const bool pass = m0 + (unsigned)r < uM && score_mask_value(cf) >= a.det_conf;
+        const unsigned pmask = (unsigned)__ballot(pass);
+        {
+            const int base = __shfl(p_base, p_leader);
+            if (p_pass && h == 0) a.det_keys[p_pos + base] = p_key;
+        }
+        unsigned b = b_first, offs = off0 + (unsigned)r;
+        if (!one_image) { const unsigned w = offs / uHW; b += w; offs -= w * uHW; }
+        p_pass = pass;
+        p_key = score_key(score_value(cf), a.det_anchor0 + (int)offs);
+        if (one_image) {
+            p_leader = pmask ? __ffs((int)pmask) - 1 : 0;
+            p_pos = (long long)b_first * a.det_np + __popc(pmask & ((1u << r) - 1u));
+            if (pmask && lane == p_leader) p_base = atomicAdd(&a.det_cnt[b_first], __popc(pmask));
+        } else {
+            p_leader = r;
+            p_pos = (long long)b * a.det_np;
+            if (pass && h == 0) p_base = atomicAdd(&a.det_cnt[b], 1);
+        }
+#pragma unroll
+        for (int q = 0; q < NCH; ++q)
+#pragma unroll
+            for (int kb = 0; kb < NKB; ++kb) {
+                asm volatile("" : "+v"(nx[q][kb]));
+                cur[q][kb] = nx[q][kb];
+            }
+        if (pmask) {
+            if (__popc(pmask) > HEAD_WAVE_DENSE) {
+                int fi[8];
+#pragma unroll
+                for (int k = 0; k < 8; ++k) fi[k] = 0x7fffffff;
+                hd_static_for<NT * 16>([&](auto itag) {
+                    constexpr int I = NT * 16 - 1 - decltype(itag)::value, j = I / 16, rg = (I % 16) / 4, e = I % 4;
+                    constexpr int c0 = j * 32 + 8 * rg + e, c1 = c0 + 4;
+                    constexpr int k0 = head_of_col(c0), k1 = head_of_col(c1);
+                    if constexpr (k0 < 8 || k1 < 8) {
+                        const float sg = act_c<ACT_SIGMOID>(acc[j][4 * rg + e]);
+                        if constexpr (k0 == k1) {
+                            fi[k0] = sg == cf[k0] ? c0 - SEGS[k0] : fi[k0];
+                        } else {
+                            if constexpr (k0 < 8) fi[k0] = ((h == 0) & (sg == cf[k0])) ? c0 - SEGS[k0] : fi[k0];
+                            if constexpr (k1 < 8) fi[k1] = ((h == 1) & (sg == cf[k1])) ? c0 - SEGS[k1] : fi[k1];
+                        }
+                    }
+                });
+                if (__ballot(nanbits != 0)) {
+                    hd_static_for<NT * 16>([&](auto itag) {
+                        constexpr int I = NT * 16 - 1 - decltype(itag)::value, j = I / 16, rg = (I % 16) / 4, e = I % 4;
+                        constexpr int c0 = j * 32 + 8 * rg + e, c1 = c0 + 4;
+                        constexpr int k0 = head_of_col(c0), k1 = head_of_col(c1);
+                        const float v = acc[j][4 * rg + e];
+                        if constexpr (k0 < 8) fi[k0] = (v != v && (k0 == k1 || h == 0)) ? c0 - SEGS[k0] : fi[k0];
+                        if constexpr (k1 < 8 && k1 != k0) fi[k1] = (v != v && h == 1) ? c0 - SEGS[k1] : fi[k1];
+                    });
+                }
+#pragma unroll
+                for (int k = 0; k < 8; ++k) fi[k] = hw_pair_min(fi[k] == 0x7fffffff ? fi[k] : fi[k] + 4 * h);
+                if (pass && h == 0) {
+                    float* const o = (float*)a.out + ((long long)b * a.det_n + a.det_anchor0 + (int)offs) * LP_DET_COLS + 12;
+                    typedef float f4u __attribute__((ext_vector_type(4), aligned(4)));
+                    *(f4u*)o = f4u{cf[0], cf[1], cf[2], cf[3]};
+                    *(f4u*)(o + 4) = f4u{cf[4], cf[5], cf[6], cf[7]};
+                    *(f4u*)(o + 8) = f4u{(float)fi[0], (float)fi[1], (float)fi[2], (float)fi[3]};
+                    *(f4u*)(o + 12) = f4u{(float)fi[4], (float)fi[5], (float)fi[6], (float)fi[7]};
+                }
+            } else {
+                const float* const sr = (const float*)stg;
+                const float* const smx = (const float*)(stg + PITCH);
+                for (unsigned mm = pmask; mm; mm &= mm - 1u) {
+                    const int arow = __ffs((int)mm) - 1;
+                    if (r == arow) {
+                        hd_static_for<NT * 4>([&](auto itag) {
+                            constexpr int I = decltype(itag)::value, j = I / 4, rg = I % 4;
+                            *(f32x4*)(stg + (j * 32 + 8 * rg + 4 * h) * 4) = f32x4{acc[j][4 * rg], acc[j][4 * rg + 1], acc[j][4 * rg + 2], acc[j][4 * rg + 3]};
+                        });
+                        if (h == 0) {
+                            *(f32x4*)(stg + PITCH) = f32x4{cf[0], cf[1], cf[2], cf[3]};
+                            *(f32x4*)(stg + PITCH + 16) = f32x4{cf[4], cf[5], cf[6], cf[7]};
+                        }
+                    }
+                    asm volatile("s_waitcnt lgkmcnt(0)" ::: "memory");
+                    unsigned long long bal[5];
+                    hd_static_for<5>([&](auto jtag) {
+                        constexpr int j = decltype(jtag)::value;
+                        const int c = 64 * j + lane;
+                        int hk = 8;
+#pragma unroll
+                        for (int q = 7; q >= 0; --q) if (c < SEGS[q + 1]) hk = q;
+                        const bool valid = hk < 8;
+                        const float v = valid ? sr[c] : 0.f;
+                        const float mx = smx[valid ? hk : 0];
+                        bal[j] = __ballot(valid && (act_c<ACT_SIGMOID>(v) == mx || (mx != mx && v != v)));
+                    });
+                    float myv = 0.f;
+                    hd_static_for<8>([&](auto ktag) {
+                        constexpr int k = decltype(ktag)::value;
+                        int idx = SEGS[k + 1] - SEGS[k] - 1;
+                        bool found = false;
+                        hd_static_for<5>([&](auto jtag) {
+                            constexpr int j = decltype(jtag)::value;
+                            constexpr int lo = SEGS[k] > 64 * j ? SEGS[k] - 64 * j : 0;
+                            constexpr int hi = SEGS[k + 1] < 64 * j + 64 ? SEGS[k + 1] - 64 * j : 64;
+                            if constexpr (lo < hi) {
+                                constexpr unsigned long long msk = (hi - lo == 64 ? ~0ull : ((1ull << (hi - lo)) - 1ull)) << lo;
+                                const unsigned long long hit = bal[j] & msk;
+                                if (!found && hit) { idx = 64 * j + __ffsll((long long)hit) - 1 - SEGS[k]; found = true; }
+                            }
+                        });
+                        if (lane == 8 + k) myv = (float)idx;
+                    });
+                    if (lane < 8) myv = smx[lane];
+                    unsigned ab = b_first, aoffs = off0 + (unsigned)arow;
+                    if (!one_image) { const unsigned w = aoffs / uHW; ab += w; aoffs -= w * uHW; }
+                    float* const o = (float*)a.out + ((long long)ab * a.det_n + a.det_anchor0 + (int)aoffs) * LP_DET_COLS + 12;
+                    if (lane < 16) o[lane] = myv;
+                    asm volatile("s_waitcnt lgkmcnt(0)" ::: "memory");
+                }
+            }
+        }
+        m0 += mstride;
+        b_first += step_b;
+        off0 += step_off;
+        if (off0 >= uHW) { off0 -= uHW; ++b_first; }
+    }
+    {
+        const int base = __shfl(p_base, p_leader);
+        if (p_pass && h == 0) a.det_keys[p_pos + base] = p_key;
+    }
+}
+
+template <typename T, int NCH, int NW>
+static inline int head_det_wave_launch_one(const ConvArgs& a, int cb_pack, hipStream_t st) {
+    static std::atomic<unsigned long long> attr_done{0};
+    if (int rc = set_max_lds_once(head_det_wave_kernel<T, NCH, NW>, 160 * 1024, attr_done, "head det wave")) return rc;
+    const long long ntiles = ((long long)a.B * a.Ho * a.Wo + 31) / 32;
+    const int lds = head_det_wave_lds_bytes(NCH, NW);
+    const int per_cu = NW == 8 ? 1 : (160 * 1024) / lds >= 2 ? 2 : 1;
+    const long long want = (ntiles + NW - 1) / NW, cap = 256LL * per_cu;
+    const long long nblk = want < cap ? want : cap;
+    hipLaunchKernelGGL((head_det_wave_kernel<T, NCH, NW>), dim3((unsigned)nblk), dim3(NW * 64), (size_t)lds, st, a, cb_pack, (int)(nblk * NW));
+    hipError_t e = hipGetLastError();
+    if (e != hipSuccess) return fail(LP_ERR_HIP, std::string("head det wave launch: ") + hipGetErrorString(e));
+    return LP_OK;
+}
+
+template <typename T>
+static inline int head_det_wave_launch_dtype(const ConvArgs& a, int cb_pack, hipStream_t st) {
+    const int nch = a.chunk_begin[a.nsrc];
+    if (nch == 1) return head_det_wave_launch_one<T, 1, 4>(a, cb_pack, st);
+    if (nch == 2) return head_det_wave_launch_one<T, 2, 4>(a, cb_pack, st);
+    return fail(LP_ERR_UNSUPPORTED, "head det wave: K-chunks");
+}
+
+}
diff --git a/yolo-lp_amd/csrc/lp_internal.h b/yolo-lp_amd/csrc/lp_internal.h
--- a/yolo-lp_amd/csrc/lp_internal.h
+++ b/yolo-lp_amd/csrc/lp_internal.h
@@ -148,6 +148,8 @@
 
 bool head_rows_fits(int dtype, int nchunks, int cb_pack, int out_c);
 bool head_det_fits(int dtype, int nchunks, int cb_pack, int out_c);
+bool head_det_wave_fits(int dtype, int nchunks, int cb_pack, int out_c);
+int head_det_wave_launch(int dtype, const ConvArgs& a, int cb_pack, hipStream_t st);
 bool head_box_det_fits(const ConvArgs& a, int cb_pack, int ksize, int stride);
 int head_box_det_launch(int dtype, const ConvArgs& a, int cb_pack, hipStream_t st);
 int head_rows_launch(int dtype, const ConvArgs& a, int cb_pack, hipStream_t st);
diff --git a/yolo-lp_amd/yolov6/hip/abi.py b/yolo-lp_amd/yolov6/hip/abi.py
--- a/yolo-lp_amd/yolov6/hip/abi.py
+++ b/yolo-lp_amd/yolov6/hip/abi.py
@@ -12,6 +12,7 @@
 LP_VARIANT_PIPE16_S2A, LP_VARIANT_PIPE16_S2B = 48, 49
 LP_VARIANT_FUSED_BIFUSION = 45
 LP_VARIANT_BOX_SPARSE, LP_VARIANT_BOX_DENSE = 46, 47
+LP_VARIANT_HEAD_DET_WAVE, LP_VARIANT_HEAD_DET = 50, 51
 LP_VARIANT_FUSED_PW_S2 = 38
 LP_VARIANT_FUSED_STEM2 = 37
 LP_VARIANT_PIPE_P = 36
@@ -21,6 +22,7 @@
     LP_VARIANT_FUSED_STEM2: 'Fz', LP_VARIANT_FUSED_PW_S2: 'Fp', LP_VARIANT_FUSED_BIFUSION: 'Fb',
     LP_VARIANT_PIPE16_D: 'Md', LP_VARIANT_PIPE16_F: 'Mf', LP_VARIANT_PIPE16_V0: 'V0', LP_VARIANT_PIPE16_V1: 'V1',
     LP_VARIANT_PIPE16_S2A: 'Xa', LP_VARIANT_PIPE16_S2B: 'Xb',
+    LP_VARIANT_HEAD_DET_WAVE: 'Dw', LP_VARIANT_HEAD_DET: 'Dt',
 }
 LP_FRAMES_PER_LAUNCH = 64
 LP_NV12_PER_LAUNCH = 32
@@ -128,6 +130,7 @@
     'lp_engine_set_single_lane': (c_int, [c_void_p, c_int]),
     'lp_engine_set_mfma16': (c_int, [c_void_p, c_int]),
     'lp_engine_op_carrier': (c_int, [c_void_p, c_int, c_int]),
+    'lp_engine_op_det_variant': (c_int, [c_void_p, c_int, POINTER(c_int)]),
     'lp_engine_num_ops': (c_int, [c_void_p]),
     'lp_engine_op_info': (c_int, [c_void_p, c_int, POINTER(c_int), POINTER(c_int), POINTER(c_int), POINTER(c_int),
                                   POINTER(c_double), POINTER(c_double)]),
diff --git a/yolo-lp_amd/yolov6/hip/runtime.py b/yolo-lp_amd/yolov6/hip/runtime.py
--- a/yolo-lp_amd/yolov6/hip/runtime.py
+++ b/yolo-lp_amd/yolov6/hip/runtime.py
@@ -537,6 +537,10 @@
             self.lib.lp_engine_op_variant(self.h, i, ctypes.byref(cfg), ctypes.byref(nb))
             ops.append(dict(self._op_info(i), ms=float(ms[i]),
                             variant='%s%d' % (abi.VARIANT_SHORT.get(cfg.value) or 'ABCDEFGH'[cfg.value], nb.value)))
+            det = ctypes.c_int()
+            abi.check(self.lib.lp_engine_op_det_variant(self.h, i, ctypes.byref(det)), 'lp_engine_op_det_variant')
+            if ops[-1]['kind'] == 'head_cls' and det.value:
+                ops[-1]['variant'] += '+' + abi.VARIANT_SHORT[det.value]
         direct = x.dtype == self.dtype
         for o in ops:
             o['flops_own'], o['bytes_own'] = o['flops'], o['bytes']
```
